# mayataka/idocp

Hardware: AMD Instinct MI355X
Metric: SQP iterations/sec (whole node) (higher is better)
Workload: dtype f64; 1 GPU; ANYmal OCPSolver N=100 T=5.05 FP64, trotting contact sequence (1 lift + 9 impulse events, 120 stages incl. impulse / aux / lift stages, switching constraints; BASELINE.json configs[2]); batch=1024 independent OCP instances per GPU, replicas across GPUs; horizon=100, batch_per_gpu=1024, parallelism=replicas x1

## Files before the change

### idocp_amd/csrc/ocp_capi.hip

```cpp
#include <hip/hip_runtime.h>

#include <cmath>
#include <cstdlib>
#include <cstring>
#include <limits>
#include <string>
#include <vector>

#include "dev_lie.hpp"
#include "host_util.hpp"
#include "idocp_hip.h"
#include "model_shapes.hpp"
#include "ocp_launch.hpp"

using namespace idocp_dev;
using idocp_host::set_last_error;
using idocp_host::isQuadruped;

#define HIP_TRY(expr)                                                                         \
  do {                                                                                        \
    hipError_t e_ = (expr);                                                                   \
    if (e_ != hipSuccess) {                                                                   \
      set_last_error(std::string(#expr) + ": " + hipGetErrorString(e_));                      \
      (void)hipGetLastError();  \
// ... 1532 lines not shown
    }
    const int ck = nd.kind == 1 ? P.impulse_cone_kind : P.cone_kind;
    for (int c = 0; c < DQ::NC; ++c) {
      if (!nd.active[c]) continue;
      double J[3];
      for (int r = 0; r < coneRows(ck); ++r) if (coneRow(ck, P.mu, r, s + LQ::S_F + 3 * c, J) > 0) return false;
    }
    return true;
  };
  for (int b = 0; b < h->batch; ++b) {
    int bad = -1;
    for (int kind = 0; kind < 4 && bad < 0; ++kind)
      for (int p = 0; p < M && bad < 0; ++p) {
        const OcpNode& nd = h->chain[p];
        if (nd.kind != kind) continue;
        if (!stageOk(nd, &sol[((size_t)b * h->NS + nd.slot) * LQ::SOL])) bad = p;
      }
    feasible[b] = bad < 0 ? 1 : 0;
    if (where) where[b] = bad;
  }
  return IDOCP_OK;
}

int idocp_ocp_dimc(const idocp_ocp_t* h) {
  if (!h) return 0;
  const idocp_constraints_t& c = h->cons;
  return 2 * DQ::NU * ((c.joint_position_limits ? 1 : 0) + (c.joint_velocity_limits ? 1 : 0) + (c.joint_torque_limits ? 1 : 0)) +
         (c.linearized_friction_cone ? 5 * DQ::NC : 0) + (c.friction_cone ? 2 * DQ::NC : 0) +
         DQ::NU * ((c.joint_acceleration_lower_limit ? 1 : 0) + (c.joint_acceleration_upper_limit ? 1 : 0)) + (c.contact_distance ? DQ::NC : 0);
}

int idocp_ocp_get_constraint_data(idocp_ocp_t* h, int instance, double* slack, double* dual) {
  if (!h || instance < 0 || instance >= h->batch) return IDOCP_E_ARG;
  int rc = setDev(h); if (rc) return rc;
  const int N = h->Ngrid, dimc = idocp_ocp_dimc(h);
  std::vector<double> sl((size_t)N * LQ::CON), du((size_t)N * LQ::CON);
  HIP_TRY(hipMemcpyAsync(sl.data(), h->B.slack + (size_t)instance * h->NS * LQ::CON, sl.size() * sizeof(double), hipMemcpyDeviceToHost, h->stream));
  HIP_TRY(hipMemcpyAsync(du.data(), h->B.dual + (size_t)instance * h->NS * LQ::CON, du.size() * sizeof(double), hipMemcpyDeviceToHost, h->stream));
  HIP_TRY(hipStreamSynchronize(h->stream));
  const idocp_constraints_t& c = h->cons;
  const int use[11] = {c.joint_position_limits, c.joint_position_limits, c.joint_velocity_limits, c.joint_velocity_limits, c.joint_torque_limits,
                       c.joint_torque_limits, c.linearized_friction_cone || c.friction_cone, 0, c.joint_acceleration_lower_limit, c.joint_acceleration_upper_limit,
                       c.contact_distance};
  const int cr = coneRows(h->prob.cone_kind);
  for (int i = 0; i < N; ++i) {
    int off = 0;
    for (int comp = 0; comp < 11; ++comp) {
      if (!use[comp]) continue;
      const int n = comp == 10 ? DQ::NC : (comp != 6 ? DQ::NU : cr * DQ::NC);
      const bool valid = (comp < 2 || comp == 10) ? i >= 2 : (comp < 4 ? i >= 1 : true);
      for (int r = 0; r < n; ++r) {
        const int src = comp == 10 ? LQ::C_CD + r : (comp != 6 ? ipmCompRow<LQ>(comp) + r : LQ::C_FRIC + 5 * (r / cr) + r % cr);
        if (slack) slack[(size_t)i * dimc + off + r] = valid ? sl[(size_t)i * LQ::CON + src] : 0.0;
        if (dual) dual[(size_t)i * dimc + off + r] = valid ? du[(size_t)i * LQ::CON + src] : 0.0;
      }
      off += n;
    }
  }
  return IDOCP_OK;
}

int idocp_ocp_get_profile(idocp_ocp_t* h, long long* out, int n) {
  if (!h || !out || n <= 0 || n > 64) return IDOCP_E_ARG;
  int rc = setDev(h); if (rc) return rc;
  HIP_TRY(hipMemcpy(out, h->B.prof, sizeof(long long) * n, hipMemcpyDeviceToHost));
  return IDOCP_OK;
}

int idocp_ocp_set_lqr_stage(idocp_ocp_t* h, int stage, int terminal, const double* Qxx, const double* Qxu, const double* Quu, const double* Fqq6,
                            const double* Fqv6, const double* Fvq, const double* Fvv, const double* Fvu, const double* lx, const double* lu,
                            const double* Fx) {
  if (!h || !Qxx || !lx || stage < 0 || stage > h->Ngrid) return IDOCP_E_ARG;
  if (!terminal && (!Qxu || !Quu || !Fqq6 || !Fqv6 || !Fvq || !Fvv || !Fvu || !lu || !Fx)) return IDOCP_E_ARG;
  int rc = setDev(h); if (rc) return rc;
  const int nv = DQ::NV, nx = DQ::NX, nu = DQ::NU;
  std::vector<double> k(LQ::KKT, 0.0);
  for (int c = 0; c < nx; ++c) for (int r = 0; r <= c; ++r) k[LQ::K_QXX + LQ::xsym(r, c)] = Qxx[c * nx + r];
  std::memcpy(&k[LQ::K_LX], lx, sizeof(double) * nx);
  if (!terminal) {
    std::memcpy(&k[LQ::K_QXU], Qxu, sizeof(double) * nx * nu);
    std::memcpy(&k[LQ::K_QUU], Quu, sizeof(double) * nu * nu);
    std::memcpy(&k[LQ::K_FQQ], Fqq6, sizeof(double) * 36);
    std::memcpy(&k[LQ::K_FQV], Fqv6, sizeof(double) * 36);
    std::memcpy(&k[LQ::K_FVQ], Fvq, sizeof(double) * nv * nv);
    std::memcpy(&k[LQ::K_FVV], Fvv, sizeof(double) * nv * nv);
    std::memcpy(&k[LQ::K_FVU], Fvu, sizeof(double) * nv * nu);
    std::memcpy(&k[LQ::K_LU], lu, sizeof(double) * nu);
    std::memcpy(&k[LQ::K_FX], Fx, sizeof(double) * nx);
  }
  HIP_TRY(hipStreamSynchronize(h->stream));
  for (long b = 0; b < h->batch; ++b)
    HIP_TRY(hipMemcpy(h->B.kkt + ((size_t)b * h->NS + stage) * LQ::KKT, k.data(), k.size() * sizeof(double), hipMemcpyHostToDevice));
  return IDOCP_OK;
}

static int getContactDynamics(idocp_ocp_t* h, int instance, int stage, int dimf, double* MJtJinv, double* MJtJinv_dIDCdqv, double* MJtJinv_IDC);
int idocp_ocp_get_contact_dynamics(idocp_ocp_t* h, int instance, int stage, double* MJtJinv, double* MJtJinv_dIDCdqv, double* MJtJinv_IDC) {
  if (!h || !MJtJinv || !MJtJinv_dIDCdqv || !MJtJinv_IDC || instance < 0 || instance >= h->batch) return IDOCP_E_ARG;
  int dimf = -1;
  for (const OcpNode& nd : h->chain) if (nd.kind == 0 && nd.slot == stage) dimf = nd.dimf;
  if (dimf < 0) { set_last_error("idocp_ocp_get_contact_dynamics: stage " + std::to_string(stage) + " is not a grid stage of the current discretisation"); return IDOCP_E_ARG; }
  return getContactDynamics(h, instance, stage, dimf, MJtJinv, MJtJinv_dIDCdqv, MJtJinv_IDC);
}
int idocp_ocp_get_contact_dynamics_chain(idocp_ocp_t* h, int instance, int position, double* MJtJinv, double* MJtJinv_dIDCdqv, double* MJtJinv_IDC) {
  if (!h || !MJtJinv || !MJtJinv_dIDCdqv || !MJtJinv_IDC || instance < 0 || instance >= h->batch || position < 0 || position >= h->M()) return IDOCP_E_ARG;
  const OcpNode& nd = h->chain[position];
  if (nd.kind == 4) { set_last_error("idocp_ocp_get_contact_dynamics_chain: the terminal stage has no dynamics"); return IDOCP_E_ARG; }
  return getContactDynamics(h, instance, nd.slot, nd.dimf, MJtJinv, MJtJinv_dIDCdqv, MJtJinv_IDC);
}
static int getContactDynamics(idocp_ocp_t* h, int instance, int stage, int dimf, double* MJtJinv, double* MJtJinv_dIDCdqv, double* MJtJinv_IDC) {
  int rc = setDev(h); if (rc) return rc;
  std::vector<double> e(LQ::EXP);
  HIP_TRY(hipMemcpyAsync(e.data(), h->B.exp + ((size_t)instance * h->NS + stage) * LQ::EXP, e.size() * sizeof(double), hipMemcpyDeviceToHost, h->stream));
  HIP_TRY(hipStreamSynchronize(h->stream));
  const int n = DQ::NV + dimf;
  for (int c = 0; c < n; ++c) for (int r = 0; r < n; ++r) MJtJinv[r + n * c] = r >= c ? e[LQ::E_MJ + r * (r + 1) / 2 + c] : e[LQ::E_MJ + c * (c + 1) / 2 + r];
  for (int c = 0; c < DQ::NX; ++c) for (int r = 0; r < n; ++r) MJtJinv_dIDCdqv[r + n * c] = e[LQ::E_MJD + r + DQ::NVF * c];
  for (int r = 0; r < n; ++r) MJtJinv_IDC[r] = e[LQ::E_MJIDC + r];
  return dimf;
}

int idocp_ocp_get_lqr_stage(idocp_ocp_t* h, int instance, int stage, double* Qxx, double* Qxu, double* Quu, double* A, double* Bm,
                            double* lx, double* lu, double* Fx) {
  if (!h || instance < 0 || instance >= h->batch || stage < 0 || stage >= h->Ngrid) return IDOCP_E_ARG;
  int rc = setDev(h); if (rc) return rc;
  const int nv = DQ::NV, nx = DQ::NX, nu = DQ::NU;
  std::vector<double> k(LQ::KKT);
  HIP_TRY(hipMemcpyAsync(k.data(), h->B.kkt + ((size_t)instance * h->NS + stage) * LQ::KKT, k.size() * sizeof(double), hipMemcpyDeviceToHost, h->stream));
  HIP_TRY(hipStreamSynchronize(h->stream));
  for (int c = 0; c < nx; ++c) for (int r = 0; r < nx; ++r) Qxx[c * nx + r] = k[LQ::K_QXX + LQ::xsym(r, c)];
  std::memcpy(Qxu, &k[LQ::K_QXU], sizeof(double) * nx * nu);
  std::memcpy(Quu, &k[LQ::K_QUU], sizeof(double) * nu * nu);
  std::memset(A, 0, sizeof(double) * nx * nx);
  std::memset(Bm, 0, sizeof(double) * nx * nu);
  double dt = h->T / h->N;
  for (const OcpNode& nd : h->chain) if (nd.slot == stage) dt = nd.dtq;
  for (int c = 0; c < nv; ++c) for (int r = 0; r < nv; ++r) {
    double fqq = (r == c) ? 1.0 : 0.0, fqv = (r == c) ? dt : 0.0;
    if (r < 6 && c < 6) { fqq = k[LQ::K_FQQ + r + 6 * c]; fqv = k[LQ::K_FQV + r + 6 * c]; }
    else if (r < 6 || c < 6) { fqq = 0.0; fqv = 0.0; }
    A[r + nx * c] = fqq; A[r + nx * (nv + c)] = fqv;
    A[(nv + r) + nx * c] = k[LQ::K_FVQ + r + nv * c]; A[(nv + r) + nx * (nv + c)] = k[LQ::K_FVV + r + nv * c];
  }
  for (int j = 0; j < nu; ++j) for (int r = 0; r < nv; ++r) Bm[(nv + r) + nx * j] = k[LQ::K_FVU + r + nv * j];
  std::memcpy(lx, &k[LQ::K_LX], sizeof(double) * nx);
  std::memcpy(lu, &k[LQ::K_LU], sizeof(double) * nu);
  std::memcpy(Fx, &k[LQ::K_FX], sizeof(double) * nx);
  return IDOCP_OK;
}

int idocp_parnmpc_create(const idocp_model_t* model, const idocp_cost_t* cost, const idocp_constraints_t* constraints, double T,
                         int N, int batch, int device, idocp_ocp_t** out) {
  return createOcpImpl(model, cost, constraints, T, N, 0, batch, device, true, out);
}

int idocp_parnmpc_create_hybrid(const idocp_model_t* model, const idocp_cost_t* cost, const idocp_constraints_t* constraints, double T,
                                int N, int max_num_impulse, int batch, int device, idocp_ocp_t** out) {
  return createOcpImpl(model, cost, constraints, T, N, max_num_impulse, batch, device, true, out);
}

int idocp_parnmpc_init_backward_correction(idocp_ocp_t* h, double t) {
  if (!h || !h->parnmpc) return IDOCP_E_ARG;
  int rc = setDev(h); if (rc) return rc;
  if ((rc = discretize(h, t))) return rc;
  OcpLaunch<DQ>::parnmpcPhase(4, h->B, h->batch, h->M(), h->has_terminal, h->d_q0, h->d_v0, h->stream);
  HIP_TRY(hipGetLastError());
  HIP_TRY(hipStreamSynchronize(h->stream));
  return IDOCP_OK;
}

int idocp_parnmpc_launch_phase(idocp_ocp_t* h, int phase, const double* d_q, const double* d_v) {
  if (!h || !h->parnmpc || phase < 0 || phase > 9 || !d_q || !d_v) return IDOCP_E_ARG;
  int rc = setDev(h); if (rc) return rc;
  if (h->seq_dirty || h->disc_time != h->disc_time) { if ((rc = discretize(h, h->disc_time == h->disc_time ? h->disc_time : 0.0))) return rc; }
  const int M = h->M();
  switch (phase) {
    case 0: OcpLaunch<DQ>::rnea(h->B, h->batch, M, h->n_impulse, h->stream); break;
    case 1:
      if (h->has_switch) OcpLaunch<DQ>::switching(h->B, h->batch, M, h->stream);
      OcpLaunch<DQ>::condenseBackwardEuler(h->B, h->batch, M, d_q, d_v, false, h->stream);
      OcpLaunch<DQ>::parnmpcImpulseCondense(h->B, h->batch, h->n_impulse, false, d_q, d_v, h->stream);
      break;
    case 2:
      OcpLaunch<DQ>::parnmpcInverse(h->B, h->batch, M, h->stream);
      OcpLaunch<DQ>::parnmpcEventInverse(h->B, h->batch, h->n_general, h->stream);
      break;
    case 3: case 4: case 5: case 6: OcpLaunch<DQ>::parnmpcPhase(phase - 3, h->B, h->batch, M, h->has_terminal, d_q, d_v, h->stream); break;
    case 7: OcpLaunch<DQ>::single(4, h->B, h->batch, M, h->stream); break;
    case 8: OcpLaunch<DQ>::single(5, h->B, h->batch, M, h->stream); break;
    default: OcpLaunch<DQ>::single(6, h->B, h->batch, M, h->stream); break;
  }
  HIP_TRY(hipGetLastError());
  return IDOCP_OK;
}

int idocp_parnmpc_update_solution_device(idocp_ocp_t* h, double t, const double* d_q, const double* d_v) {
  if (!h || !h->parnmpc || !d_q || !d_v) return IDOCP_E_ARG;
  if (!h->contact_status_set) { set_last_error("idocp_parnmpc_update_solution: call setContactStatusUniformly first"); return IDOCP_E_ARG; }
  int rc = setDev(h); if (rc) return rc;
  if ((rc = discretize(h, t))) return rc;
  HIP_TRY(hipMemsetAsync(h->B.status, 0, sizeof(int) * h->batch, h->stream));
  for (int phase = 0; phase <= 9; ++phase) if ((rc = idocp_parnmpc_launch_phase(h, phase, d_q, d_v))) return rc;
  return IDOCP_OK;
}

int idocp_parnmpc_compute_direction(idocp_ocp_t* h, double t, const double* q, const double* v) {
  if (!h || !h->parnmpc || !q || !v) return IDOCP_E_ARG;
  if (!h->contact_status_set) { set_last_error("idocp_parnmpc_update_solution: call setContactStatusUniformly first"); return IDOCP_E_ARG; }
  int rc = setDev(h); if (rc) return rc;
  HIP_TRY(hipMemcpyAsync(h->d_q0, q, sizeof(double) * h->batch * DQ::NQ, hipMemcpyHostToDevice, h->stream));
  HIP_TRY(hipMemcpyAsync(h->d_v0, v, sizeof(double) * h->batch * DQ::NV, hipMemcpyHostToDevice, h->stream));
  if ((rc = discretize(h, t))) return rc;
  HIP_TRY(hipMemsetAsync(h->B.status, 0, sizeof(int) * h->batch, h->stream));
  for (int phase = 0; phase <= 8; ++phase) if ((rc = idocp_parnmpc_launch_phase(h, phase, h->d_q0, h->d_v0))) return rc;
  HIP_TRY(hipStreamSynchronize(h->stream));
  return IDOCP_OK;
}

int idocp_parnmpc_update_solution(idocp_ocp_t* h, double t, const double* q, const double* v, int line_search) {
  if (!h || !h->parnmpc || !q || !v) return IDOCP_E_ARG;
  int rc = setDev(h); if (rc) return rc;
  if (line_search) {
    if (!h->contact_status_set) { set_last_error("idocp_parnmpc_update_solution: call setContactStatusUniformly first"); return IDOCP_E_ARG; }
    if ((rc = discretize(h, t))) return rc;
    if ((rc = parnmpcLineSearchSupported(h))) return rc;
// ... 233 lines not shown
```

### idocp_amd/csrc/ocp_condense_kernel.hip

```cpp
#include <hip/hip_runtime.h>

#include <cstdlib>

#include "dev_dense.hpp"
#include "dev_lie.hpp"
#include "dev_rnea_tangent.hpp"
#include "ocp_device.hpp"
#include "ocp_launch.hpp"

namespace idocp_dev {

#ifdef IDOCP_K5_TILES16
#define K5_TILE_PAIR mfmaTilePairTN
#else
#define K5_TILE_PAIR mfmaTilePairTN4
#endif

__device__ __forceinline__ double ocpLimit(const OcpProblem* __restrict__ P, int comp, int r) {
  switch (comp) {
    case 0: return P->q_min[r];
    case 1: return P->q_max[r];
    case 2: return -P->v_max[r];
    case 3: return P->v_max[r];
    case 4: return -P->u_max[r];
// ... 673 lines not shown
        X = &sm[S::MJD + SVF * 16 * ib]; xr = NX - 16 * ib; Y = &sm[S::QAFU + SVF * 16 * jb]; yc = NV - 16 * jb; r0 = 16 * ib; c0 = 16 * jb;
      } else {
        const int ib = j - 12;
        X = &sm[S::MJ + SVF * 16 * ib]; xr = NV - 16 * ib; Y = &sm[S::QAFU + SVF * 6]; yc = NU; r0 = 16 * ib; c0 = 0;
      }
    };
    auto finish = [&](int j, const mfma_d4& acc, int r0, int c0) {
      const int r = r0 + (lane & 15), g4 = lane >> 4;
      if (j < 6) {
        double b6[4];
        const double dg = sm[S::HQD + (r < NX ? r : NX - 1)];
        static_assert(S::HVD == S::HQD + NV, "one diagonal vector");
#pragma unroll
        for (int q = 0; q < 4; ++q) { const int c = c0 + g4 + 4 * q; b6[q] = sm[S::QB6 + (r < 6 ? r : 5) + 6 * (c < 6 ? c : 5)]; }
#pragma unroll
        for (int q = 0; q < 4; ++q) {
          const int c = c0 + g4 + 4 * q;
          const double base = (r < 6 && c < 6) ? b6[q] : (r == c ? dg : 0.0);
          if (r <= c && c < NX) kk[L::K_QXX + L::xsym(r, c)] = base - acc[q];
        }
      } else if (j < 12) {
#pragma unroll
        for (int q = 0; q < 4; ++q) {
          const int c = c0 + g4 + 4 * q;
          double* dst = c < 6 ? ee + (L::E_QXUP + r + NX * c) : kk + (L::K_QXU + r + NX * (c - 6));
          if (r < NX && c < NV) *dst = -acc[q];
        }
      } else {
        double hd[4];
#pragma unroll
        for (int q = 0; q < 4; ++q) { const int c = c0 + g4 + 4 * q; hd[q] = sm[S::HUD + (c < NU ? c : NU - 1)]; }
#pragma unroll
        for (int q = 0; q < 4; ++q) {
          const int c = c0 + g4 + 4 * q;
          double* dst = r < 6 ? ee + (L::E_QUUP + r + 6 * c) : kk + (L::K_QUU + (r - 6) + NU * c);
          const double v = acc[q] + ((r >= 6 && r - 6 == c) ? hd[q] : 0.0);
          if (r < NV && c < NU) *dst = v;
        }
      }
    };
    auto pair = [&](auto jc) {
      constexpr int j = decltype(jc)::value;
      const double *X0, *Y0, *X1, *Y1;
      int xr0, yc0, r00, c00, xr1, yc1, r01, c01;
      operands(j, X0, xr0, Y0, yc0, r00, c00);
      operands(j + 1, X1, xr1, Y1, yc1, r01, c01);
      mfma_d4 a0, a1;
      K5_TILE_PAIR<RVF>(X0, xr0, Y0, yc0, X1, xr1, Y1, yc1, SVF, SVF, dimvf, lane, a0, a1);
      finish(j, a0, r00, c00);
      finish(j + 1, a1, r01, c01);
    };
    static_assert(nt == 256 && NJOB == 14, "four wavefronts: jobs 2 w, 2 w + 1 and 2 w + 8, 2 w + 9");
    switch (__builtin_amdgcn_readfirstlane(wave)) {
      case 0: pair(std::integral_constant<int, 0>{}); pair(std::integral_constant<int, 8>{}); break;
      case 1: pair(std::integral_constant<int, 2>{}); pair(std::integral_constant<int, 10>{}); break;
      case 2: pair(std::integral_constant<int, 4>{}); pair(std::integral_constant<int, 12>{}); break;
      default: pair(std::integral_constant<int, 6>{}); break;
    }
  }
  STAMP(14);
  {
    const int part = tid & 3, g = tid >> 2;
    const int q4 = (dimvf + 3) >> 2, k0 = part * q4, k1 = (k0 + q4 < dimvf) ? k0 + q4 : dimvf;
    double acc = 0.0;
    if (g < NX) { const double* col = &sm[S::MJD + SVF * g]; for (int k = k0; k < k1; ++k) acc += col[k] * sm[S::LAF + k]; }
    else if (g < NX + NV) { const double* row = &sm[S::MJ + (g - NX)]; for (int k = k0; k < k1; ++k) acc += row[SVF * k] * sm[S::LAF + k]; }
    acc += __shfl_xor(acc, 1);
    acc += __shfl_xor(acc, 2);
    if (part == 0) {
      if (g < NV) sm[S::LQ + g] -= acc;
      else if (g < NX) sm[S::LV + g - NV] -= acc;
      else if (g < NX + NV) {
        const int r = g - NX;
        if (r < 6) sm[S::LUP + r] += hu * acc; else sm[S::LU + r - 6] += hu * acc;
        sm[S::FV + r] -= dt * mjidc[r];
      }
    }
  }
  static_assert(4 * (NX + NV) <= nt, "a quad per row of the vector updates");
  blockLdsBarrier();

  STAMP(9);
  typedef double wd2 __attribute__((ext_vector_type(2)));
  static_assert(NV % 2 == 0 && SVF % 2 == 0 && S::MJD % 2 == 0 && L::K_FVQ % 2 == 0 && L::K_FVV % 2 == 0 && L::KKT % 2 == 0, "16-byte stores of Fvq / Fvv");
  for (int e = tid; e < NV * NV / 2; e += nt) {
    const int c = e / (NV / 2), r = 2 * (e - c * (NV / 2));
    const wd2 mq = *reinterpret_cast<const wd2*>(&sm[S::MJD + r + SVF * c]), mvv = *reinterpret_cast<const wd2*>(&sm[S::MJD + r + SVF * (NV + c)]);
    const double one = BWD ? -1.0 : 1.0;
    wd2 fq, fv;
    fq.x = -dt * mq.x; fq.y = -dt * mq.y;
    fv.x = -dt * mvv.x + (r == c ? one : 0.0); fv.y = -dt * mvv.y + (r + 1 == c ? one : 0.0);
    *reinterpret_cast<wd2*>(&kk[L::K_FVQ + r + NV * c]) = fq;
    *reinterpret_cast<wd2*>(&kk[L::K_FVV + r + NV * c]) = fv;
  }
  for (int e = tid; e < NV * NU; e += nt) { const int c = e / NV, r = e - c * NV; kk[L::K_FVU + e] = hu * dt * sm[S::MJ + r + SVF * (6 + c)]; }
  if (tid < NV) {
    kk[L::K_LX + tid] = sm[S::LQ + tid]; kk[L::K_LX + NV + tid] = sm[S::LV + tid];
    kk[L::K_FX + tid] = sm[S::FQ + tid]; kk[L::K_FX + NV + tid] = sm[S::FV + tid];
  }
  if (tid < NU) kk[L::K_LU + tid] = sm[S::LU + tid];
  for (int t = tid; t < RVF * (RVF + 1) / 2; t += nt) {
    const int pr = t / (RVF + 1), idx = t - pr * (RVF + 1);
    const bool lo = idx <= pr;
    const int r = lo ? pr : RVF - 1 - pr, c = lo ? idx : idx - pr - 1;
    ee[L::E_MJ + r * (r + 1) / 2 + c] = sm[S::MJ + r + SVF * c];
  }
  static_assert(RVF % 2 == 0 && NVF % 2 == 0 && L::E_MJD % 2 == 0 && L::EXP % 2 == 0, "16-byte stores of MJtJinv_dIDCdqv");
  for (int e = tid; e < (RVF / 2) * NX; e += nt) {
    const int c = e / (RVF / 2), r = 2 * (e - c * (RVF / 2));
    *reinterpret_cast<wd2*>(&ee[L::E_MJD + r + NVF * c]) = *reinterpret_cast<const wd2*>(&sm[S::MJD + r + SVF * c]);
  }
  if (tid < NV) ee[L::E_QAA + tid] = sm[S::QAA + tid];
  for (int e = tid; e < SF * SF; e += nt) { const int c = e / SF, r = e - c * SF; ee[L::E_QFF + r + NF * c] = sm[S::QFF + e]; }
  if (tid < RVF) { ee[L::E_MJIDC + tid] = mjidc[tid]; ee[L::E_LAF + tid] = sm[S::LAF + tid]; }
  if (tid < 6) ee[L::E_LUP + tid] = sm[S::LUP + tid];
  if (sw_dimi > 0) {
    const int dimi = sw_dimi;
    double* __restrict__ W = B.swc + rec * L::SWC;
    for (int e = tid; e < dimi * NX; e += nt) {
      const int c = e / dimi, j = e - c * dimi;
      double acc = 0.0;
      for (int m2 = 0; m2 < NV; ++m2) acc += W[L::W_PHIA + j + NF * m2] * sm[S::MJD + m2 + SVF * c];
      W[L::W_PHIX + j + NF * c] -= acc;
    }
    for (int e = tid; e < dimi * NU; e += nt) {
      const int c = e / dimi, j = e - c * dimi;
      double acc = 0.0;
      for (int m2 = 0; m2 < NV; ++m2) acc += W[L::W_PHIA + j + NF * m2] * sm[S::MJ + m2 + SVF * (6 + c)];
      W[L::W_PHIU + j + NF * c] = acc;
    }
    if (tid < dimi) {
      double acc = 0.0;
      for (int m2 = 0; m2 < NV; ++m2) acc += W[L::W_PHIA + tid + NF * m2] * mjidc[m2];
      W[L::W_P + tid] -= acc;
    }
  }
  STAMP(10);
  if (tid == 0 && !s_ok && B.status[b] == 0) B.status[b] = 1 + pos;
  };
  stage((long)blockIdx.x);
#undef STAMP
#undef STAMPW
}


template <typename D>
__global__ __launch_bounds__(64) void parnmpc_lie_kernel(OcpBuffers B, const double* __restrict__ q0) {
  using L = OcpLayout<D>;
  constexpr int NQ = D::NQ;
  const OcpProblem* __restrict__ P = B.prob;
  const int M = B.M;
  const long unit = (long)blockIdx.x * 64 + threadIdx.x;
  if (unit >= (long)P->batch * (M - 1)) return;
  const long b = unit / (M - 1);
  const int pos = (int)(unit - b * (M - 1));
  const OcpNode* __restrict__ nd = B.nodes + pos;
  const int task = blockIdx.y;
  const long rec = b * B.NS + nd->slot;
  const double* __restrict__ s = B.sol + rec * L::SOL;
  const double* __restrict__ q = s + L::S_Q;
  double* __restrict__ zz = B.lie + rec * L::LIE;
  double R[9], p[3], Ja[36], Jb[36], d6[6];
  if (task == 0) {
    lieRelative(B.q_ref + (long)pos * NQ, q, R, p);
    lieLog6(R, p, d6);
    lieJlog6(R, p, Ja);
    for (int k = 0; k < 36; ++k) zz[L::Z_JQ + k] = Ja[k];
    for (int k = 0; k < 6; ++k) zz[L::Z_QDIFF + k] = d6[k];
  } else if (task == 1) {
    lieRelative(B.sol + (b * B.NS + nd->next) * L::SOL + L::S_Q, q, R, p);
    lieJlog6(R, p, Ja);
    for (int k = 0; k < 36; ++k) zz[L::Z_FQQ + k] = Ja[k];
  } else {
    const double* __restrict__ q_prev = (nd->prev < 0) ? (q0 + b * NQ) : (B.sol + (b * B.NS + nd->prev) * L::SOL + L::S_Q);
    lieRelative(q, q_prev, R, p);
    lieLog6(R, p, d6);
    for (int k = 0; k < 6; ++k) zz[L::Z_FQ6 + k] = d6[k];
    lieJlog6(R, p, Ja);
    lieDDiffArg0(R, p, Ja, Jb);
    for (int k = 0; k < 36; ++k) zz[L::Z_FQQP + k] = Jb[k];
    lieBlockInverse(Ja, Jb);
    for (int k = 0; k < 36; ++k) zz[L::Z_FQQI + k] = Jb[k];
  }
}

template <typename D>
static void launchCondense(const OcpBuffers& B, long batch, int M, int dimf, const double* q0, hipStream_t st, bool residual, int part = 0) {
  const size_t smem = CondenseSmem<D>::TOTAL * sizeof(double);
  static bool configured = false;
  if (!configured) {
    (void)hipFuncSetAttribute((const void*)ocp_condense_kernel<D, false, -1>, hipFuncAttributeMaxDynamicSharedMemorySize, (int)smem);
    (void)hipFuncSetAttribute((const void*)ocp_condense_kernel<D, false, -1, false, false, true>, hipFuncAttributeMaxDynamicSharedMemorySize, (int)smem);
    (void)hipFuncSetAttribute((const void*)ocp_condense_kernel<D, false, D::NF>, hipFuncAttributeMaxDynamicSharedMemorySize, (int)smem);
// ... 113 lines not shown
```

### idocp_amd/csrc/ocp_device.hpp

```cpp
#ifndef IDOCP_OCP_DEVICE_HPP_
#define IDOCP_OCP_DEVICE_HPP_

#include "unocp_device.hpp"

namespace idocp_dev {

template <int NL_, int LJ_>
struct LeggedDims {
  static constexpr int NL = NL_, LJ = LJ_;
  static constexpr int NJ = 1 + NL * LJ, NV = 6 + NL * LJ, NQ = NV + 1, NU = NL * LJ, NC = NL, NF = 3 * NC;
  static constexpr int NX = 2 * NV, NVF = NV + NF;
};

template <typename D>
struct OcpLayout {
  static constexpr int NV = D::NV, NQ = D::NQ, NU = D::NU, NF = D::NF, NX = D::NX, NVF = D::NVF, NC = D::NC;
  static constexpr int S_LMD = 0, S_GMM = NV, S_Q = 2 * NV, S_V = S_Q + NQ, S_A = S_V + NV, S_U = S_A + NV, S_BETA = S_U + NU,
                       S_F = S_BETA + NV, S_MU = S_F + NF, S_NUP = S_MU + NF, S_XI = S_NUP + 6;
  static constexpr int SOL = roundUp16(S_XI + NF);
  static constexpr int D_LMD = 0, D_GMM = NV, D_Q = 2 * NV, D_V = 3 * NV, D_A = 4 * NV, D_U = 5 * NV, D_BETA = D_U + NU,
                       D_F = D_BETA + NV, D_MU = D_F + NF, D_NUP = D_MU + NF, D_XI = D_NUP + 6,
                       D_T = D_XI + NF, D_W = D_T + NVF;
  static constexpr int DIR = roundUp16(D_W + NVF);
  static constexpr int C_FRIC = 6 * NU, C_ACC = C_FRIC + 5 * NC, C_CD = C_ACC + 2 * NU, NCON = C_CD + NC;
  static constexpr int CON = roundUp16(NCON);
  static constexpr int L_DIDC = 0, L_M = NVF * NX, L_J = L_M + NV * NV, L_IDC = L_J + NF * NV;
  static constexpr int LIN = roundUp16(L_IDC + NVF);
  static constexpr int X_TRI = (NX * (NX + 1) / 2 + 1) / 2 * 2;
  __host__ __device__ static constexpr int xsym(int r, int c) { return r <= c ? c * (c + 1) / 2 + r : r * (r + 1) / 2 + c; }
  static constexpr int K_QXX = 0, K_QXU = X_TRI, K_QUU = K_QXU + NX * NU, K_FQQ = K_QUU + NU * NU, K_FQV = K_FQQ + 36,
                       K_FVQ = K_FQV + 36, K_FVV = K_FVQ + NV * NV, K_FVU = K_FVV + NV * NV, K_LX = K_FVU + NV * NU,
                       K_LU = K_LX + NX, K_FX = K_LU + NU;
  static constexpr int KKT = roundUp16(K_FX + NX);
  static constexpr int MJ_TRI = (NVF * (NVF + 1) / 2 + 1) / 2 * 2;
  static constexpr int E_MJ = 0, E_MJD = MJ_TRI, E_QAA = E_MJD + NVF * NX, E_QFF = E_QAA + NV,
                       E_MJIDC = E_QFF + NF * NF, E_LAF = E_MJIDC + NVF, E_LUP = E_LAF + NVF, E_QUUP = E_LUP + 6,
                       E_QXUP = E_QUUP + 6 * NU, E_FQQPI = E_QXUP + NX * 6;
  static constexpr int EXP = roundUp16(E_FQQPI + 36);
  static constexpr int P_TRI = (NV * (NV + 1) / 2 + 1) / 2 * 2;
  __host__ __device__ static constexpr int psym(int r, int c) { return r <= c ? c * (c + 1) / 2 + r : r * (r + 1) / 2 + c; }
  static constexpr int R_PQQ = 0, R_PQV = P_TRI, R_PVV = R_PQV + NV * NV, R_SQ = R_PVV + P_TRI, R_SV = R_SQ + NV;
  static constexpr int RIC = roundUp16(R_SV + NV);
  static constexpr int Z_JQ = 0, Z_QDIFF = 36, Z_FQQ = 44, Z_FQ6 = 80, Z_FQQI = 88, Z_FQQP = 124, Z_FQQPI = 160;
  static constexpr int LIE = roundUp16(196);
  static constexpr int NJL = NV - 6, NJ_DYN = 42, NF_DYN = 18, NB_DYN = 16;
  static constexpr int O_JOINT = 0, O_FEET = NJL * NJ_DYN, O_BASE = O_FEET + NC * NF_DYN, O_BN = O_BASE + NB_DYN,
                       O_IDC = O_BN + (NC + 1) * 6;
  static constexpr int NOM = roundUp16(O_IDC + NVF);
  static_assert(NVF % 2 == 0, "the nominal record is copied in 16-byte pieces");
  static constexpr int X_CDJ = 0, X_Z = NC * NV, X_LQ = X_Z + NC, X_W = X_LQ + NV, X_ERR = X_W + NC, X_VIOL = X_ERR + 1;
  static constexpr int NT = 1 + IDOCP_MAX_EXTRA_TASKS;
  static constexpr int X_TJ = X_VIOL + 1, X_TW = X_TJ + NT * 6 * NV, X_COST = X_TW + NT * 6;
  static constexpr int EXT = roundUp16(X_COST + 1);
  static constexpr int G_K = 0, G_k = NU * NX;
  static constexpr int GAIN = roundUp16(G_k + NU);
  static constexpr int W_P = 0, W_PHIX = NF, W_PHIA = W_PHIX + NF * NX, W_PHIU = W_PHIA + NF * NV, W_M = W_PHIU + NF * NU,
                       W_m = W_M + NF * NX;
  static constexpr int SWC = roundUp16(W_m + NF);
  static constexpr int N_LMD = 0, N_GMM = NV, N_U = 2 * NV, N_Q = N_U + NU, N_V = N_Q + NQ, N_XI = N_V + NV;
  static constexpr int SNEW = roundUp16(N_XI + NF);
  static constexpr int NK = 2 * NX + NU, I_C0 = 0, I_C1 = NK * NX;
  static constexpr int NKG = 2 * NX + NU + NF, I_C1G = NKG * NX;
  static constexpr int KINV = roundUp16(2 * NKG * NX);
  static constexpr int AUX = roundUp16(NX * NX);
  static constexpr int XRES = roundUp16(NX);
};

struct OcpNode {
  int slot, next, prev;
  int kind;
  int level;
  int has_u;
  int dimf, active[IDOCP_MAX_CONTACTS], row_of[IDOCP_MAX_CONTACTS];
  double dt;
  double dtq;
  double vref_on;
  double contact_point[IDOCP_MAX_CONTACTS][3];
  int sw_dimi, sw_active[IDOCP_MAX_CONTACTS], sw_row[IDOCP_MAX_CONTACTS];
  double sw_dt1, sw_dt2, sw_point[IDOCP_MAX_CONTACTS][3];
};

struct ParnmpcShape {
  bool general, impulse;
  int ni, nw, nk, ld, c1;
};
template <typename L>
__host__ __device__ inline ParnmpcShape parnmpcShape(const OcpNode& nd) {
  ParnmpcShape s;
  s.impulse = nd.kind == 1;
  const bool aux = nd.kind == 2 && nd.sw_dimi > 0;
  s.general = s.impulse || aux;
  s.ni = s.impulse ? nd.dimf : (aux ? nd.sw_dimi : 0);
  s.nw = s.impulse ? nd.dimf : L::NU;
  s.nk = 2 * L::NX + s.ni + s.nw;
  s.ld = s.general ? L::NKG : L::NK;
  s.c1 = s.general ? L::I_C1G : L::I_C1;
  return s;
}

__host__ __device__ inline int coneRows(int kind) { return kind == 1 ? 2 : 5; }
__host__ __device__ inline double coneRow(int kind, double mu, int r, const double* f, double* J) {
  if (kind == 1) {
    if (r == 0) { J[0] = 0.0; J[1] = 0.0; J[2] = -1.0; return -f[2]; }
    J[0] = 2.0 * f[0]; J[1] = 2.0 * f[1]; J[2] = -2.0 * mu * mu * f[2];
    return f[0] * f[0] + f[1] * f[1] - mu * mu * f[2] * f[2];
  }
  const double m2 = mu * 0.70710678118654752440;
  J[0] = (r == 1) ? 1.0 : (r == 2 ? -1.0 : 0.0);
  J[1] = (r == 3) ? 1.0 : (r == 4 ? -1.0 : 0.0);
  J[2] = (r == 0) ? -1.0 : -m2;
  return J[0] * f[0] + J[1] * f[1] + J[2] * f[2];
}

struct OcpProblem;
template <typename L>
__host__ __device__ inline int ipmCompRow(int comp) { return comp < 6 ? comp * L::NU : L::C_ACC + (comp - 8) * L::NU; }

struct OcpProblem {
  int N, batch;
  int M, NS, E;
  int stage_offset;
// ... 74 lines not shown
```

### idocp_amd/csrc/ocp_expand_kernel.hip

```cpp
#include <hip/hip_runtime.h>

#include <cstdlib>

#include "dev_lie.hpp"
#include "dev_dense.hpp"
#include "ocp_device.hpp"
#include "ocp_launch.hpp"

namespace idocp_dev {

__device__ __forceinline__ double ocpLimit2(const OcpProblem* __restrict__ P, int comp, int r) {
  switch (comp) {
    case 0: return P->q_min[r];
    case 1: return P->q_max[r];
    case 2: return -P->v_max[r];
    case 3: return P->v_max[r];
    case 4: return -P->u_max[r];
    case 8: return P->a_min[r];
    case 9: return P->a_max[r];
    default: return P->u_max[r];
  }
}
__device__ __forceinline__ bool ocpRowValid2(const OcpProblem* __restrict__ P, int comp, int level, bool impulse) {
  if (impulse) return comp == 6 && P->use_impulse_friction_cone != 0;
// ... 13 lines not shown
__device__ __forceinline__ bool ipmRow(const OcpProblem* __restrict__ P, const OcpNode* __restrict__ nd, int row, const double* __restrict__ s,
                                       const double* dq, const double* dv, const double* du, const double* df_slot, const double* da,
                                       const double* __restrict__ xx, double* g, double* dg) {
  using L = OcpLayout<D>;
  constexpr int NU = D::NU;
  if (row >= L::C_CD) {
    const int c = row - L::C_CD;
    if (!xx || !P->use_contact_distance || nd->kind == 1 || nd->level < 2 || nd->active[c]) return false;
    *g = -xx[L::X_Z + c];
    double acc = 0.0;
    for (int t = 0; t < D::NV; ++t) acc += xx[L::X_CDJ + c * D::NV + t] * dq[t];
    *dg = -acc;
    return true;
  }
  if (row >= L::C_ACC) {
    const int c = 8 + (row - L::C_ACC) / NU, j = (row - L::C_ACC) % NU;
    if (!ocpRowValid2(P, c, nd->level, nd->kind == 1)) return false;
    const double sgn = (c & 1) ? 1.0 : -1.0;
    *g = sgn * (s[L::S_A + 6 + j] - ocpLimit2(P, c, j));
    *dg = sgn * da[6 + j];
    return true;
  }
  if (row < L::C_FRIC) {
    const int c = row / NU, j = row - c * NU;
    if (!ocpRowValid2(P, c, nd->level, nd->kind == 1)) return false;
    const double sgn = (c & 1) ? 1.0 : -1.0;
    const double x = (c < 2) ? s[L::S_Q + 7 + j] : ((c < 4) ? s[L::S_V + 6 + j] : s[L::S_U + j]);
    const double dx = (c < 2) ? dq[6 + j] : ((c < 4) ? dv[6 + j] : du[j]);
    *g = sgn * (x - ocpLimit2(P, c, j));
    *dg = sgn * dx;
    return true;
  }
  const int fr = row - L::C_FRIC, c = fr / 5, r = fr - 5 * c;
  const int ck = nd->kind == 1 ? P->impulse_cone_kind : P->cone_kind;
  if (r >= coneRows(ck) || !ocpRowValid2(P, 6, nd->level, nd->kind == 1) || !nd->active[c]) return false;
  double J[3];
  const double f[3] = {s[L::S_F + 3 * c], s[L::S_F + 3 * c + 1], s[L::S_F + 3 * c + 2]};
  *g = coneRow(ck, P->mu, r, f, J);
  *dg = J[0] * df_slot[3 * c] + J[1] * df_slot[3 * c + 1] + J[2] * df_slot[3 * c + 2];
  return true;
}
template <typename D>
__device__ __forceinline__ bool ipmIdleConeRow(const OcpProblem* __restrict__ P, const OcpNode* __restrict__ nd, int row) {
  using L = OcpLayout<D>;
  if (row >= L::C_CD) return P->use_contact_distance && nd->kind != 1 && nd->level >= 2 && nd->active[row - L::C_CD];
  if (row < L::C_FRIC || row >= L::C_ACC || !ocpRowValid2(P, 6, nd->level, nd->kind == 1)) return false;
  const int r = (row - L::C_FRIC) % 5;
  return r < coneRows(nd->kind == 1 ? P->impulse_cone_kind : P->cone_kind);
}

typedef double ex_d2 __attribute__((ext_vector_type(2)));
template <int N2>
__device__ __forceinline__ void wideLoad(ex_d2 (&r)[(N2 + 63) / 64], const double* __restrict__ src, int lane) {
  const ex_d2* __restrict__ p = reinterpret_cast<const ex_d2*>(src);
#pragma unroll
  for (int t = 0; t < (N2 + 63) / 64; ++t) { const int e = lane + 64 * t; r[t] = p[e < N2 ? e : N2 - 1]; }
}
template <int N2>
__device__ __forceinline__ void wideLoadN(ex_d2 (&r)[(N2 + 63) / 64], const double* __restrict__ src, int lane, int n2) {
  const ex_d2* __restrict__ p = reinterpret_cast<const ex_d2*>(src);
#pragma unroll
  for (int t = 0; t < (N2 + 63) / 64; ++t) { const int e = lane + 64 * t; r[t] = p[e < n2 ? e : n2 - 1]; }
}
template <int N2, int LD2>
__device__ __forceinline__ void wideLoadRows(ex_d2 (&r)[(N2 + 63) / 64], const double* __restrict__ src, int lane, int h, int inv, int n2) {
  const ex_d2* __restrict__ p = reinterpret_cast<const ex_d2*>(src);
#pragma unroll
  for (int t = 0; t < (N2 + 63) / 64; ++t) {
    int e = lane + 64 * t;
    e = e < n2 ? e : n2 - 1;
    const int c = (e * inv) >> 16;
    r[t] = p[c * LD2 + (e - c * h)];
  }
}
template <int N2, int LD2>
__device__ __forceinline__ void wideStoreLdsRows(double* dst, const ex_d2 (&r)[(N2 + 63) / 64], int lane, int h, int inv, int n2) {
#pragma unroll
  for (int t = 0; t < (N2 + 63) / 64; ++t) {
    const int e = lane + 64 * t;
    const int c = (e * inv) >> 16;
    if (e < n2) reinterpret_cast<ex_d2*>(dst)[c * LD2 + (e - c * h)] = r[t];
  }
}
template <int N2>
__device__ __forceinline__ void wideStoreLds(double* dst, const ex_d2 (&r)[(N2 + 63) / 64], int lane) {
#pragma unroll
  for (int t = 0; t < (N2 + 63) / 64; ++t) { const int e = lane + 64 * t; if (e < N2) reinterpret_cast<ex_d2*>(dst)[e] = r[t]; }
}

template <typename D>
__global__ __launch_bounds__(64) void ocp_expand_primal_kernel(OcpBuffers B) {
  using L = OcpLayout<D>;
  constexpr int NV = D::NV, NX = D::NX, NU = D::NU, NF = D::NF, NVF = D::NVF, NC = D::NC;
  constexpr int RL = L::R_SV + NV, MJDL = NVF * NX, MJUL = L::MJ_TRI;
  static_assert(RL % 2 == 0 && MJDL % 2 == 0 && MJUL % 2 == 0 && L::E_MJD % 2 == 0 && L::EXP % 2 == 0 && L::RIC % 2 == 0, "16-byte loads");
  constexpr int PML = RL > MJDL ? RL : MJDL;
  __shared__ __attribute__((aligned(16))) double pm[PML], mju[MJUL], sr[L::SOL];
  double* pb = pm;
  double* mjd = pm;
  __shared__ double dx[NX], du[NU], dfs[NF], das[NV];
  const OcpProblem* __restrict__ P = B.prob;
  const int M = B.M;
  const int lane = threadIdx.x;
  const long unit = blockIdx.x;
  const long b = unit / M;
  const int pos = (int)(unit - b * M);
  const OcpNode* __restrict__ nd = B.nodes + pos;
  const bool terminal = (pos == M - 1);
  const long rec = b * B.NS + nd->slot;
  double* __restrict__ dd = B.dir + rec * L::DIR;
  if (P->backward_euler && terminal) return;
  const bool costate = !P->backward_euler;
  const bool bimp = P->backward_euler && nd->kind == 1;
  const bool expand = !terminal && !bimp;
  ex_d2 pw[(RL / 2 + 63) / 64], mw[(MJDL / 2 + 63) / 64], uw[(MJUL / 2 + 63) / 64];
  if (costate) wideLoad<RL / 2>(pw, B.ric + rec * L::RIC, lane);
  const int rows_ld = NV + nd->dimf, h_ld = (rows_ld + 1) >> 1, inv_ld = 65535 / h_ld + 1, nmjd2 = h_ld * NX, ntri2 = (rows_ld * (rows_ld + 1) / 2 + 1) >> 1;
  static_assert(NVF % 2 == 0 && (NVF / 2) * NX == MJDL / 2, "pieces per column of MJtJinv_dIDCdqv");
  if (expand) {
    wideLoadRows<MJDL / 2, NVF / 2>(mw, B.exp + rec * L::EXP + L::E_MJD, lane, h_ld, inv_ld, nmjd2);
    wideLoadN<MJUL / 2>(uw, B.exp + rec * L::EXP + L::E_MJ, lane, ntri2);
  }
  static_assert(L::SOL % 2 == 0 && L::NCON <= 128, "two IPM rows per lane");
  ex_d2 sw[(L::SOL / 2 + 63) / 64];
  double sl_r[2] = {1.0, 1.0}, dl_r[2] = {1.0, 1.0}, mjidc_r = 0.0;
  if (!terminal) {
    wideLoad<L::SOL / 2>(sw, B.sol + rec * L::SOL, lane);
#pragma unroll
    for (int t = 0; t < 2; ++t) {
      const int row = lane + 64 * t;
      if (row < L::NCON) { sl_r[t] = B.slack[rec * L::CON + row]; dl_r[t] = B.dual[rec * L::CON + row]; }
    }
    if (lane < NVF) mjidc_r = B.exp[rec * L::EXP + L::E_MJIDC + lane];
  }
  if (lane < NV) { dx[lane] = dd[L::D_Q + lane]; dx[NV + lane] = dd[L::D_V + lane]; }
  if (lane < NU && !terminal) du[lane] = dd[L::D_U + lane];
  if (lane < NF) dfs[lane] = 0.0;
  if (costate) wideStoreLds<RL / 2>(pb, pw, lane);
  if (expand) wideStoreLds<MJUL / 2>(mju, uw, lane);
  if (!terminal) wideStoreLds<L::SOL / 2>(sr, sw, lane);
  waveLdsSync();
  if (lane < NX && costate) {
    const bool isv = lane >= NV;
    const int r = isv ? lane - NV : lane;
    double acc = -pb[(isv ? L::R_SV : L::R_SQ) + r];
    if (!isv) {
#pragma unroll
      for (int c = 0; c < NV; ++c) acc += pb[L::R_PQQ + L::psym(r, c)] * dx[c] + pb[L::R_PQV + r + NV * c] * dx[NV + c];
    } else {
#pragma unroll
      for (int c = 0; c < NV; ++c) acc += pb[L::R_PQV + c + NV * r] * dx[c] + pb[L::R_PVV + L::psym(r, c)] * dx[NV + c];
    }
    dd[(isv ? L::D_GMM : L::D_LMD) + r] = acc;
  }
  if (terminal) return;
  waveLdsSync();
  if (expand) wideStoreLdsRows<MJDL / 2, NVF / 2>(mjd, mw, lane, h_ld, inv_ld, nmjd2);
  waveLdsSync();
  const long su = rec;
  const double* s = sr;
  const int dimf = nd->dimf, dimvf = NV + dimf;
  if (bimp) {
    const double* __restrict__ kk = B.kkt + rec * L::KKT;
    if (lane < NF) dfs[lane] = dd[L::D_F + lane];
    if (lane < NV) {
      double acc = -mjidc_r;
      double t1 = 0.0;
      for (int c = 0; c < NV; ++c) t1 += kk[L::K_FVQ + lane + NV * c] * dx[c];
      acc += t1;
      double t2 = 0.0;
      for (int j = 0; j < dimf; ++j) t2 += kk[L::K_FVU + lane + NV * j] * du[j];
      acc += t2;
      dd[L::D_A + lane] = acc; das[lane] = acc;
    }
  }
  if (!P->backward_euler && nd->sw_dimi > 0 && lane >= 32 && lane < 32 + nd->sw_dimi) {
    const int l = lane - 32;
    const double* __restrict__ W = B.swc + rec * L::SWC;
    double acc = W[L::W_m + l];
    for (int c = 0; c < NX; ++c) acc += W[L::W_M + l + NF * c] * dx[c];
    dd[L::D_XI + l] = acc;
  }
  if (!bimp && lane < dimvf) {
    const int r = lane;
    double acc = -mjidc_r, tt = 0.0, ww = 0.0;
#pragma unroll
    for (int c = 0; c < NX; ++c) tt += mjd[r + NVF * c] * dx[c];
#pragma unroll
    for (int j = 0; j < NU; ++j) { const int c = 6 + j; ww += (r >= c ? mju[r * (r + 1) / 2 + c] : mju[c * (c + 1) / 2 + r]) * du[j]; }
    acc += ww - tt;
    dd[L::D_T + r] = tt; dd[L::D_W + r] = ww;
    if (r < NV) { dd[L::D_A + r] = acc; das[r] = acc; }
    else {
      const int pr = r - NV;
      for (int c = 0; c < NC; ++c) if (nd->active[c] && pr >= nd->row_of[c] && pr < nd->row_of[c] + 3) {
        const int slot = 3 * c + (pr - nd->row_of[c]);
        dfs[slot] = -acc; dd[L::D_F + slot] = -acc;
      }
    }
  }
  waveLdsSync();
  double ps = 1.0, ds = 1.0;
#pragma unroll
  for (int t = 0; t < 2; ++t) {
    const int row = lane + 64 * t;
    double g, dg;
    if (row >= L::NCON || !ipmRow<D>(P, nd, row, s, dx, dx + NV, du, dfs, das, B.ext ? B.ext + rec * L::EXT : nullptr, &g, &dg)) continue;
    const double sl = sl_r[t], dl = dl_r[t];
    const double res = g + sl, duality = sl * dl - P->barrier;
    const double dslack = -dg - res;
    const double ddual = -(dl * dslack + duality) / sl;
    ps = f2b(P->fraction_rate, sl, dslack, ps);
    ds = f2b(P->fraction_rate, dl, ddual, ds);
  }
#pragma unroll
  for (int off = 32; off >= 1; off >>= 1) { ps = fmin(ps, __shfl_xor(ps, off)); ds = fmin(ds, __shfl_xor(ds, off)); }
  if (lane == 0) { B.step_stage[su * 2] = ps; B.step_stage[su * 2 + 1] = ds; }
}

template <typename D>
__global__ __launch_bounds__(128, 1) void ocp_forward_expand_kernel(OcpBuffers B, const double* __restrict__ q0, const double* __restrict__ v0) {
  using L = OcpLayout<D>;
  constexpr int NV = D::NV, NQ = D::NQ, NX = D::NX, NU = D::NU, NF = D::NF, NVF = D::NVF, NC = D::NC;
  constexpr int GL = L::GAIN, RL = L::R_SV + NV, MJDL = NVF * NX, MJUL = L::MJ_TRI;
  static_assert(GL % 2 == 0 && RL % 2 == 0 && MJDL % 2 == 0 && MJUL % 2 == 0 && L::SOL % 2 == 0 && L::GAIN % 2 == 0 && L::RIC % 2 == 0 && L::EXP % 2 == 0 &&
                L::E_MJD % 2 == 0 && L::KKT % 2 == 0 && L::K_FQQ % 2 == 0 && L::K_FX % 2 == 0 && NVF % 2 == 0, "16-byte loads");
  static_assert(L::K_FQV == L::K_FQQ + 36 && L::NCON <= 128 && NX <= 36 && 36 + NX / 2 <= 64, "Fqq6 | Fqv6 and Fx on one load; two IPM rows per lane");
  static_assert(NC <= 4 && NF <= 15 && NVF + NV <= 64 && L::R_PQQ == 0 && L::R_SV == L::R_SQ + NV, "node word: four contacts; lane maps");
  static_assert(L::C_FRIC >= 64 && L::C_CD >= 64 && L::NCON <= 128, "cone / contact-distance rows are mapped to lane + 64 only");
  constexpr int NG2 = (GL / 2 + 63) / 64, NP2 = (RL / 2 + 63) / 64, NM2 = (MJDL / 2 + 63) / 64, NT2 = (MJUL / 2 + 63) / 64, NS2 = (L::SOL / 2 + 63) / 64;
  constexpr int MAXM = OcpForwardExpandMaxChain;
  constexpr int PF = NX * NX, PSV = PF, PPAD = PF + NX;
  constexpr int DV = NX + NU + NV + NF + 2;
  __shared__ __attribute__((aligned(16))) double gb[GL], pfull[PF + NX + 2], mjd[MJDL], mju[MJUL], sr[L::SOL], fb[72 + NX];
  __shared__ double ring[3][DV];
  __shared__ int n_slot[MAXM], n_word[MAXM];
  __shared__ double n_dt[MAXM], n_dtq[MAXM];
  const int M = B.M;
  const int tid = threadIdx.x, lane = tid & 63;
  const int wave = __builtin_amdgcn_readfirstlane(tid >> 6);
  const long b = blockIdx.x;
  const long base = b * B.NS;
  int use_cone, use_icone, use_cd, ck_stage, ck_imp;
  double cmu, barrier, frate;
  int r_xoff[2], r_doff[2], r_thr[2];
  double r_sgn[2], r_bound[2];
  {
    const OcpProblem* __restrict__ P = B.prob;
    use_cone = P->use_friction_cone; use_icone = P->use_impulse_friction_cone;
    use_cd = P->use_contact_distance; ck_stage = P->cone_kind; ck_imp = P->impulse_cone_kind;
    cmu = P->mu; barrier = P->barrier; frate = P->fraction_rate;
#pragma unroll
    for (int t = 0; t < 2; ++t) {
      const int row = lane + 64 * t;
      r_xoff[t] = 0; r_doff[t] = 0; r_thr[t] = 4; r_sgn[t] = 1.0; r_bound[t] = 0.0;
      if (row < L::C_FRIC) {
        const int c = row / NU, j = row - c * NU;
        r_sgn[t] = (c & 1) ? 1.0 : -1.0;
        r_xoff[t] = (c < 2) ? L::S_Q + 7 + j : ((c < 4) ? L::S_V + 6 + j : L::S_U + j);
        r_doff[t] = (c < 2) ? 6 + j : ((c < 4) ? NV + 6 + j : NX + j);
        r_bound[t] = ocpLimit2(P, c, j);
        r_thr[t] = (c < 2) ? (P->use_q_limits ? 2 : 4) : ((c < 4) ? (P->use_v_limits ? 1 : 4) : (P->use_u_limits ? 0 : 4));
      } else if (row >= L::C_ACC && row < L::C_CD) {
        const int c = 8 + (row - L::C_ACC) / NU, j = (row - L::C_ACC) % NU;
        r_sgn[t] = (c & 1) ? 1.0 : -1.0;
        r_xoff[t] = L::S_A + 6 + j; r_doff[t] = NX + NU + 6 + j;
        r_bound[t] = ocpLimit2(P, c, j);
        r_thr[t] = (c == 8 ? P->use_a_lower : P->use_a_upper) ? 0 : 4;
      }
    }
    const OcpNode* __restrict__ nodes = B.nodes;
    for (int i = tid; i < M; i += 128) {
      const OcpNode* __restrict__ nd = nodes + i;
      int w = (nd->kind & 7) | ((nd->level < 3 ? (nd->level < 0 ? 0 : nd->level) : 3) << 3) | (nd->dimf << 5) | (nd->sw_dimi << 9) | ((nd->has_u ? 1 : 0) << 13);
#pragma unroll
      for (int c = 0; c < NC; ++c) if (nd->active[c]) w |= (1 << (14 + c)) | ((nd->row_of[c] / 3) << (18 + 2 * c));
      n_slot[i] = nd->slot; n_word[i] = w; n_dt[i] = nd->dt; n_dtq[i] = nd->dtq;
    }
  }
  if (wave == 0) {
    double* dx = ring[0];
    const int slot0 = B.nodes[0].slot;
    const double* __restrict__ s0 = B.sol + (base + slot0) * L::SOL;
    if (lane == 0) {
      double R[9], p[3], d6[6];
      lieRelative(s0 + L::S_Q, q0 + b * NQ, R, p);
      lieLog6(R, p, d6);
      const double* __restrict__ Fi = B.exp + (base + slot0) * L::EXP + L::E_FQQPI;
      for (int r = 0; r < 6; ++r) { double acc = 0.0; for (int m = 0; m < 6; ++m) acc += Fi[r + 6 * m] * d6[m]; dx[r] = -acc; }
    }
    if (lane >= 6 && lane < NV) dx[lane] = q0[b * NQ + lane + 1] - s0[L::S_Q + lane + 1];
    if (lane < NV) dx[NV + lane] = v0[b * NV + lane] - s0[L::S_V + lane];
  }
  blockLdsSync();
  if (wave == 0) {
    struct Regs { ex_d2 g[NG2], m[NM2], u[NT2], f; double mjidc; };
    Regs RA, RB;
    const int af_row = lane < NVF ? lane : NVF - 1;
    int tri_off[NU];
#pragma unroll
    for (int j = 0; j < NU; ++j) { const int c = 6 + j; tri_off[j] = af_row >= c ? af_row * (af_row + 1) / 2 + c : c * (c + 1) / 2 + af_row; }
    auto fetch = [&](int i, Regs& R) {
      const long rec = base + n_slot[i];
      wideLoad<GL / 2>(R.g, B.gain + rec * L::GAIN, lane);
      const int rows_ld = NV + ((n_word[i] >> 5) & 15), h_ld = (rows_ld + 1) >> 1, inv_ld = 65535 / h_ld + 1;
      wideLoadRows<MJDL / 2, NVF / 2>(R.m, B.exp + rec * L::EXP + L::E_MJD, lane, h_ld, inv_ld, h_ld * NX);
      wideLoadN<MJUL / 2>(R.u, B.exp + rec * L::EXP + L::E_MJ, lane, (rows_ld * (rows_ld + 1) / 2 + 1) >> 1);
      {
        const ex_d2* __restrict__ kq = reinterpret_cast<const ex_d2*>(B.kkt + rec * L::KKT + L::K_FQQ);
        const ex_d2* __restrict__ kx = reinterpret_cast<const ex_d2*>(B.kkt + rec * L::KKT + L::K_FX);
        R.f = lane < 36 ? kq[lane] : kx[lane - 36 < NX / 2 ? lane - 36 : NX / 2 - 1];
      }
      R.mjidc = B.exp[rec * L::EXP + L::E_MJIDC + af_row];
    };
    if (M > 1) fetch(0, RA);
    if (M > 2) fetch(1, RB);
    auto step = [&](int i, Regs& R) {
      double* const dv = ring[i % 3];
      double* const dx = dv; double* const du = dv + NX; double* const das = dv + NX + NU; double* const dfs = dv + NX + NU + NV;
      double* const dxn = ring[(i + 1) % 3];
      const int word = n_word[i];
      const long rec = base + n_slot[i];
      const int dimf = (word >> 5) & 15, amask = (word >> 14) & 15, rows3 = (word >> 18) & 255;
      const double sdt = n_dt[i], sdtq = n_dtq[i];
      double* __restrict__ dd = B.dir + rec * L::DIR;
      const int dimvf = NV + dimf;
      const int h_ld = (dimvf + 1) >> 1, inv_ld = 65535 / h_ld + 1;
      wideStoreLds<GL / 2>(gb, R.g, lane);
      wideStoreLdsRows<MJDL / 2, NVF / 2>(mjd, R.m, lane, h_ld, inv_ld, h_ld * NX);
      wideStoreLds<MJUL / 2>(mju, R.u, lane);
      if (lane < 36 + NX / 2) reinterpret_cast<ex_d2*>(fb)[lane] = R.f;
      const double mjidc_r = R.mjidc;
      waveLdsSync();
      if (i + 2 < M - 1) fetch(i + 2, R);
      {
        const int j = lane >> 2, part = lane & 3;
        double acc = 0.0;
        if (lane < 4 * NU) {
#pragma unroll
          for (int t = 0; t < NX / 4; ++t) { const int c = (NX / 4) * part + t; acc += gb[L::G_K + j + NU * c] * dx[c]; }
        }
        acc += __shfl_xor(acc, 1);
        acc += __shfl_xor(acc, 2);
        if (lane < 4 * NU && part == 0) { acc += gb[L::G_k + j]; du[j] = acc; dd[L::D_U + j] = acc; }
      }
      double tt = 0.0;
      if (lane < dimvf) {
#pragma unroll
        for (int c = 0; c < NX; ++c) tt += mjd[lane + NVF * c] * dx[c];
      }
      if (lane < NF) dfs[lane] = 0.0;
      if (lane >= 40 && lane < 40 + NV) { const int r = lane - 40; dd[L::D_Q + r] = dx[r]; dd[L::D_V + r] = dx[NV + r]; }
      waveLdsSync();
      if (lane < dimvf) {
        const int r = lane;
        double ww = 0.0;
#pragma unroll
        for (int j = 0; j < NU; ++j) ww += mju[tri_off[j]] * du[j];
        const double acc_af = -mjidc_r + (ww - tt);
        dd[L::D_T + r] = tt; dd[L::D_W + r] = ww;
        if (r < NV) {
          dd[L::D_A + r] = acc_af; das[r] = acc_af;
          dxn[NV + r] = dx[NV + r] + sdt * (ww - tt) + fb[72 + NV + r];
        } else {
          const int pr = r - NV;
#pragma unroll
          for (int c = 0; c < NC; ++c) {
            const int row_of = 3 * ((rows3 >> (2 * c)) & 3);
            if (((amask >> c) & 1) && pr >= row_of && pr < row_of + 3) {
              const int slot = 3 * c + (pr - row_of);
              dfs[slot] = -acc_af; dd[L::D_F + slot] = -acc_af;
            }
          }
        }
      } else if (lane >= 32 && lane < 32 + NV) {
        const int r = lane - 32;
        double dq = fb[72 + r];
        if (r < 6) {
#pragma unroll
          for (int m = 0; m < 6; ++m) dq += fb[r + 6 * m] * dx[m] + fb[36 + r + 6 * m] * dx[NV + m];
        } else {
          dq += dx[r] + sdtq * dx[NV + r];
        }
        dxn[r] = dq;
      }
    };
    static_assert(NVF <= 32, "the dq+ rows sit on the lanes behind the (a, f) rows");
    for (int i = 0; i <= M; i += 2) {
      if (i < M - 1) step(i, RA);
      blockLdsSync();
      if (i + 1 <= M) {
        if (i + 1 < M - 1) step(i + 1, RB);
        blockLdsSync();
      }
    }
    {
      const double* dx = ring[(M - 1) % 3];
      double* __restrict__ dd = B.dir + (base + n_slot[M - 1]) * L::DIR;
      if (lane < NV) { dd[L::D_Q + lane] = dx[lane]; dd[L::D_V + lane] = dx[NV + lane]; }
    }
  } else {
    struct Regs { ex_d2 p[NP2], s[NS2]; double sl[2], dl[2]; };
    Regs RA, RB;
    int p_a[NP2][2], p_b[NP2][2];
#pragma unroll
    for (int t = 0; t < NP2; ++t) {
#pragma unroll
      for (int h = 0; h < 2; ++h) {
        const int k = 2 * (lane + 64 * t) + h;
        int a = PPAD + h, bb = PPAD + h;
        if (k < L::R_PQV || (k >= L::R_PVV && k < L::R_SQ)) {
          const bool vv = k >= L::R_PVV;
// ... 521 lines not shown
```

### idocp_amd/csrc/ocp_riccati_kernel.hip

```cpp
#include <hip/hip_runtime.h>
#include <cstdlib>
#include <type_traits>

#include "dev_dense.hpp"
#include "dev_lie.hpp"
#include "ocp_device.hpp"
#include "ocp_launch.hpp"

namespace idocp_dev {

typedef double rd2 __attribute__((ext_vector_type(2)));

template <typename D>
struct RiccatiSmem {
  static constexpr int NV = D::NV, NX = D::NX, NU = D::NU, NF = D::NF;
  static constexpr int LDW = NX + 2;
  static constexpr int PQQ = 0, PQV = PQQ + NV * NV, PVV = PQV + NV * NV, SQ = PVV + NV * NV, SV = SQ + NV,
                       STAGE = SV + NV + 4,
                       STAGE_LEN = OcpLayout<D>::KKT - OcpLayout<D>::K_QXU,
                       WT = STAGE + STAGE_LEN, GK = WT + LDW * NX,
                       KM = WT + LDW * (NX + NU), KV = KM + NU * NX,
                       GW = KV + 16, SQN = GW + NU * NU, SVN = SQN + NV, INVD = SVN + NV + 4, TOTAL = INVD + NU + 4;
  static_assert(NU * NX <= NU * LDW, "GK aliases B^T P");
  static constexpr int DG = WT, SS = DG + NF * NU, DTM = SS + NF * NF, SDG = DTM + NU * NX, MV = SDG + NF * NU, SCORR = MV + NF,
                       MMX = GK;
  static_assert(SCORR + NX <= GK && NF * NX <= NU * LDW, "hybrid aliases");
  static_assert(TOTAL * 8 + 64 <= 40960, "four instances per CU");
};

__device__ __forceinline__ void upperTile3(int t, int& ib, int& jb) {
  if (t < 3) { ib = 0; jb = t; } else if (t < 5) { ib = 1; jb = t - 2; } else { ib = 2; jb = 2; }
}

constexpr int tileBegin(int ntiles, int w, int nw) { return (ntiles * w + nw - 1) / nw; }
constexpr bool tilesUseMod3(int tb, int te, int v) { for (int t = tb; t < te; ++t) if (t % 3 == v) return true; return false; }
constexpr bool tilesUseDiv3(int tb, int te, int v) { for (int t = tb; t < te; ++t) if (t / 3 == v) return true; return false; }
constexpr int upperIb(int t) { return t < 3 ? 0 : (t < 5 ? 1 : 2); }
constexpr int upperJb(int t) { return t < 3 ? t : (t < 5 ? t - 2 : 2); }
constexpr bool tilesUseUpperIb(int tb, int te, int v) { for (int t = tb; t < te; ++t) if (upperIb(t) == v) return true; return false; }
constexpr bool tilesUseUpperJb(int tb, int te, int v) { for (int t = tb; t < te; ++t) if (upperJb(t) == v) return true; return false; }

template <int K>
__device__ __forceinline__ void mfmaLoadOp(double (&o)[(K + 3) / 4], const double* p, int stride, int lane) {
  const int g = lane >> 4;
#pragma unroll
  for (int s = 0; s < (K + 3) / 4; ++s) {
    const int k = 4 * s + g;
    if (4 * s + 3 < K) o[s] = p[stride * k];
    else { const double v = p[stride * (k < K ? k : K - 1)]; o[s] = k < K ? v : 0.0; }
  }
}

template <typename D, bool WIDE, int TB, int TE, typename Mid>
__device__ __forceinline__ void riccatiPhase1(const double* Pqq, const double* Pqv, const double* Pvv, const double* Fall, const double* Fqq6,
                                              const double* Fqv6, double dt, double* Wt, int lane, Mid mid) {
  constexpr int NV = D::NV, NX = D::NX, KS = (NV + 3) / 4, LDW = RiccatiSmem<D>::LDW, NTL = TE - TB;
  if constexpr (NTL > 0) {
    const int li = lane & 15, g = lane >> 4;
    double xo[3][KS], yo[3][KS];
#pragma unroll
    for (int v = 0; v < 3; ++v) {
      if (tilesUseMod3(TB, TE, v)) {
        const int c = 16 * v + li, cc = c < NX ? c : NX - 1;
        mfmaLoadOp<NV>(xo[v], cc < NV ? Pqv + cc : Pvv + NV * (cc - NV), cc < NV ? NV : 1, lane);
      }
      if (tilesUseDiv3(TB, TE, v)) mfmaLoadOp<NV>(yo[v], Fall + NV * (16 * v + li), 1, lane);
    }
    auto structured = [&](int j, int q) -> double {
      const int cb = (TB + j) % 3, ib = (TB + j) / 3;
      const int c = 16 * cb + li, cc = c < NX ? c : NX - 1;
      const double* pq = cc < NV ? Pqq + NV * cc : Pqv + NV * (cc - NV);
      const int lo = 16 * ib + 4 * q, r = lo + g;
      if (lo >= NX) return 0.0;
      const int lo6 = lo < NV ? lo : lo - NV;
      const bool isv = r >= NV;
      const int rr6 = isv ? r - NV : r;
      const bool any6 = lo6 < 6 || (lo < NV && lo + 3 >= NV), all6 = lo6 + 3 < 6 && !(lo < NV && lo + 3 >= NV);
      double dot6 = 0.0;
      if (any6) {
        const double* F6 = (isv ? Fqv6 : Fqq6) + 6 * (rr6 < 6 ? rr6 : 0);
#pragma unroll
        for (int m = 0; m < 6; ++m) dot6 += F6[m] * pq[m];
      }
      if (all6) return dot6;
      const double direct = (isv ? dt : 1.0) * pq[rr6 < NV ? rr6 : 0];
      return (any6 && rr6 < 6) ? dot6 : direct;
    };
    constexpr bool EARLY = false;
    double extra[EARLY ? NTL : 1][4];
    if constexpr (EARLY) {
#pragma unroll
      for (int j = 0; j < NTL; ++j)
#pragma unroll
        for (int q = 0; q < 4; ++q) extra[j][q] = structured(j, q);
    }
    mfma_d4 acc[NTL];
#pragma unroll
    for (int j = 0; j < NTL; ++j) acc[j] = mfma_d4{0.0, 0.0, 0.0, 0.0};
#pragma unroll
    for (int s = 0; s < KS; ++s)
#pragma unroll
      for (int j = 0; j < NTL; ++j) acc[j] = __builtin_amdgcn_mfma_f64_16x16x4f64(yo[(TB + j) / 3][s], xo[(TB + j) % 3][s], acc[j], 0, 0, 0);
    __builtin_amdgcn_sched_barrier(0);
    mid();
    __builtin_amdgcn_sched_barrier(0);
#pragma unroll
    for (int j = 0; j < NTL; ++j) {
      __builtin_amdgcn_sched_barrier(0);
      const int cb = (TB + j) % 3, ib = (TB + j) / 3;
      const int c = 16 * cb + li;
#pragma unroll
      for (int q = 0; q < 4; ++q) {
        const int r = 16 * ib + 4 * q + g;
        double sx;
        if constexpr (EARLY) sx = extra[j][q]; else sx = structured(j, q);
        if (c < NX) Wt[c + LDW * r] = acc[j][q] + sx;
      }
    }
  } else {
    mid();
  }
}

template <typename D, bool WIDE, int TB, int TE, int T2W>
__device__ __forceinline__ void riccatiPhase2(const double* Wt, const double* Fall, const double* Fqq6, const double* Fqv6, double dt,
                                              const double (&qxx)[T2W][4], double* Pqq, double* Pqv, double* Pvv, double* Qxu, double* Quu,
                                              int lane) {
  constexpr int NV = D::NV, NX = D::NX, NU = D::NU, KS = (NV + 3) / 4, LDW = RiccatiSmem<D>::LDW, NTL = TE - TB;
  static_assert(NTL <= T2W, "Qxx registers");
  if constexpr (NTL > 0) {
    const int li = lane & 15, g = lane >> 4;
    double xo[3][KS], yo[3][KS];
#pragma unroll
// ... 114 lines not shown
          const int rb = r >= NV, cb = c >= NV, rr = r - NV * rb, cc = c - NV * cb;
          double* blk = Pqq + NV * NV * (rb + cb);
          const double val = blk[rr + NV * cc] - sign * acc[j][q];
          blk[rr + NV * cc] = val;
          blk[(rb == cb) ? cc + NV * rr : rr + NV * cc] = val;
        }
      }
    }
  }
}

#define RICCATI_TILES_CASE8(FN, NTILES, W, ...)                                                                                        \
  case W: if constexpr (tileBegin(NTILES, W, 8) < tileBegin(NTILES, W + 1, 8)) FN<D, false, tileBegin(NTILES, W, 8), tileBegin(NTILES, W + 1, 8)>(__VA_ARGS__); break;
#define RICCATI_TILES(FN, NTILES, ...)                                                                                                 \
  do {                                                                                                                                 \
    if constexpr (NW == 1) { FN<D, true, 0, NTILES>(__VA_ARGS__); }                                                                          \
    else if constexpr (NW == 2) {                                                                                                      \
      if (wave == 0) FN<D, false, tileBegin(NTILES, 0, 2), tileBegin(NTILES, 1, 2)>(__VA_ARGS__);                                            \
      else FN<D, false, tileBegin(NTILES, 1, 2), tileBegin(NTILES, 2, 2)>(__VA_ARGS__);                                                      \
    } else if constexpr (NW == 8) {                                                                                                    \
      switch (wave) {                                                                                                                  \
        RICCATI_TILES_CASE8(FN, NTILES, 0, __VA_ARGS__) RICCATI_TILES_CASE8(FN, NTILES, 1, __VA_ARGS__)                                \
        RICCATI_TILES_CASE8(FN, NTILES, 2, __VA_ARGS__) RICCATI_TILES_CASE8(FN, NTILES, 3, __VA_ARGS__)                                \
        RICCATI_TILES_CASE8(FN, NTILES, 4, __VA_ARGS__) RICCATI_TILES_CASE8(FN, NTILES, 5, __VA_ARGS__)                                \
        RICCATI_TILES_CASE8(FN, NTILES, 6, __VA_ARGS__) RICCATI_TILES_CASE8(FN, NTILES, 7, __VA_ARGS__)                                \
        default: break;                                                                                                                \
      }                                                                                                                                \
    } else {                                                                                                                           \
      if (wave == 0) FN<D, false, tileBegin(NTILES, 0, 4), tileBegin(NTILES, 1, 4)>(__VA_ARGS__);                                            \
      else if (wave == 1) FN<D, false, tileBegin(NTILES, 1, 4), tileBegin(NTILES, 2, 4)>(__VA_ARGS__);                                       \
      else if (wave == 2) FN<D, false, tileBegin(NTILES, 2, 4), tileBegin(NTILES, 3, 4)>(__VA_ARGS__);                                       \
      else FN<D, false, tileBegin(NTILES, 3, 4), tileBegin(NTILES, 4, 4)>(__VA_ARGS__);                                                      \
    }                                                                                                                                  \
  } while (0)

template <int NW> __device__ __forceinline__ void blockSync() {
  if constexpr (NW == 1) { __builtin_amdgcn_fence(__ATOMIC_SEQ_CST, "wavefront"); __builtin_amdgcn_wave_barrier(); }
  else blockLdsSync();
}

template <typename D, int NT, bool HYBRID>
__global__ __launch_bounds__(NT, (NT == 64 || NT == 512) ? 1 : 2) void ocp_riccati_backward_kernel(OcpBuffers B) {
  using L = OcpLayout<D>;
  using S = RiccatiSmem<D>;
  constexpr int NV = D::NV, NX = D::NX, NU = D::NU, NN = NV * NV, NF = D::NF, LDW = S::LDW, NW = NT / 64;
  static_assert(NX + NU == 48 && NX <= 48, "3 x 3 tiles of 16");
  extern __shared__ __attribute__((aligned(16))) double sm[];
  __shared__ int s_ok;
  const OcpProblem* __restrict__ P = B.prob;
  const int M = B.M;
  const OcpNode* __restrict__ nodes = B.nodes;
  const int tid = threadIdx.x;
  constexpr int nt = NT;
  const int wave = tid >> 6, lane = tid & 63, li = lane & 15, g = lane >> 4;
  const long b = blockIdx.x;
  const long base = b * B.NS;
  double* Pqq = &sm[S::PQQ];
  double* Pqv = &sm[S::PQV];
  double* Pvv = &sm[S::PVV];
  double* Wt = &sm[S::WT];
  double* st = &sm[S::STAGE];
  constexpr int KO = L::K_QXU, SL = S::STAGE_LEN;
  if (tid == 0) s_ok = 1;
  const bool p32 = P->ric_fp32 != 0;
  auto st32 = [&](double x) { return p32 ? (double)(float)x : x; };
  {
    const double* __restrict__ kk = B.kkt + (base + nodes[M - 1].slot) * L::KKT;
    double* __restrict__ rr = B.ric + (base + nodes[M - 1].slot) * L::RIC;
    for (int e = tid; e < NN; e += nt) {
      const int c = e / NV, r = e - c * NV;
      const double pqq = st32(kk[L::K_QXX + L::xsym(r, c)]), pvv = st32(kk[L::K_QXX + L::xsym(NV + r, NV + c)]);
      Pqq[e] = pqq; Pqv[e] = 0.0; Pvv[e] = pvv;
      rr[L::R_PQV + e] = 0.0;
      if (r <= c) { rr[L::R_PQQ + L::psym(r, c)] = pqq; rr[L::R_PVV + L::psym(r, c)] = pvv; }
    }
    if (tid < NV) {
      const double sq = st32(-kk[L::K_LX + tid]), sv = st32(-kk[L::K_LX + NV + tid]);
      sm[S::SQ + tid] = sq; sm[S::SV + tid] = sv;
      rr[L::R_SQ + tid] = sq; rr[L::R_SV + tid] = sv;
    }
  }
  {
    const double* __restrict__ kk = B.kkt + (base + nodes[M - 2].slot) * L::KKT;
    for (int e = tid; e < SL; e += nt) st[e] = kk[KO + e];
  }
  blockSync<NW>();
  for (int i = M - 2; i >= 0; --i) {
    const OcpNode* __restrict__ nd = nodes + i;
    const double dt = nd->dtq;
    const long rec = base + nd->slot;
    const int dimi = HYBRID ? nd->sw_dimi : 0;
    const bool stamp = tid == 0 && b == (gridDim.x > 7 ? 7 : 0) && i == M / 2 && B.prof != nullptr;
#define RSTAMP(k) do { if (stamp) B.prof[16 + k] = wall_clock64(); } while (0)
    RSTAMP(0);
    constexpr int PF = (SL / 2 + NT - 1) / NT, T1 = 9, T2 = 6, T2W = (T2 + NW - 1) / NW;
    static_assert(SL % 2 == 0 && KO % 2 == 0 && S::STAGE % 2 == 0 && L::KKT % 2 == 0, "16-byte loads of the stage record");
    rd2 pre[PF];
    double qxx[T2W][4];
    auto loadQxx = [&]() {
      const double* __restrict__ kc = B.kkt + rec * L::KKT;
      const int t2b = tileBegin(T2, wave, NW), t2e = tileBegin(T2, wave + 1, NW);
#pragma unroll
      for (int jj = 0; jj < T2W; ++jj) {
        const int t = t2b + jj;
        int ib, jb;
        upperTile3(t < t2e ? t : 0, ib, jb);
        const int r = 16 * ib + li;
#pragma unroll
        for (int q = 0; q < 4; ++q) {
          const int c = 16 * jb + g + 4 * q;
          qxx[jj][q] = (t < t2e && r <= c && c < NX) ? kc[L::K_QXX + L::xsym(r, c)] : 0.0;
        }
      }
    };
    double* Qxu = st + (L::K_QXU - KO);
    double* Quu = st + (L::K_QUU - KO);
    const double* Fqq6 = st + (L::K_FQQ - KO);
    const double* Fqv6 = st + (L::K_FQV - KO);
    const double* Fall = st + (L::K_FVQ - KO);
    static_assert(L::K_FVV == L::K_FVQ + NV * NV && L::K_FVU == L::K_FVV + NV * NV, "[Fvq Fvv Fvu] contiguous");
    const double* Fvq = st + (L::K_FVQ - KO);
    const double* Fvv = st + (L::K_FVV - KO);
    const double* Fvu = st + (L::K_FVU - KO);
    const double* lx = st + (L::K_LX - KO);
    double* lu = st + (L::K_LU - KO);
    const double* Fx = st + (L::K_FX - KO);
    RSTAMP(1);
    RICCATI_TILES(riccatiPhase1, T1, Pqq, Pqv, Pvv, Fall, Fqq6, Fqv6, dt, Wt, lane, loadQxx);
    blockSync<NW>();
    RSTAMP(2);
    RICCATI_TILES(riccatiPhase2, T2, Wt, Fall, Fqq6, Fqv6, dt, qxx, Pqq, Pqv, Pvv, Qxu, Quu, lane);
    RSTAMP(11);
    if (tid >= NT - 64 && lane < 4 * NU) {
      const int j = lane >> 2, part = lane & 3;
      const int c0 = (part >> 1) * (NX / 2) + (part & 1) * 10, nc2 = (part & 1) ? 4 : 5;
      static_assert(NX == 36 && LDW % 2 == 0, "column split of the lu rows");
      const rd2* wj = reinterpret_cast<const rd2*>(Wt + LDW * (NX + j) + c0);
      const rd2* fx = reinterpret_cast<const rd2*>(Fx + c0);
      double acc = 0.0;
#pragma unroll
      for (int c = 0; c < 5; ++c) if (c < nc2) { const rd2 w = wj[c], f = fx[c]; acc += w.x * f.x + w.y * f.y; }
#pragma unroll
      for (int t = 0; t < (NV + 3) / 4; ++t) { const int m = part + 4 * t; if (m < NV) acc -= Fvu[m + NV * j] * sm[S::SV + m]; }
      acc += __shfl_xor(acc, 1);
      acc += __shfl_xor(acc, 2);
      if (part == 0) lu[j] += acc;
    }
    auto sPart1 = [&](int row) {
      const bool isv = row >= NV;
      const int r = isv ? row - NV : row;
      const double* F6 = isv ? Fqv6 : Fqq6;
      const rd2* Fm = reinterpret_cast<const rd2*>((isv ? Fvv : Fvq) + NV * r);
      const rd2* wr = reinterpret_cast<const rd2*>(Wt + LDW * row);
      const rd2* svp = reinterpret_cast<const rd2*>(&sm[S::SV]);
      const rd2* fx = reinterpret_cast<const rd2*>(Fx);
      static_assert(NV % 2 == 0 && S::SV % 2 == 0 && (L::K_FX - KO) % 2 == 0 && (L::K_FVQ - KO) % 2 == 0, "16-byte reads of the vector terms");
      double acc;
      if (r < 6) {
        acc = 0.0;
#pragma unroll
        for (int m = 0; m < 6; ++m) acc += F6[m + 6 * r] * sm[S::SQ + m];
      } else {
        acc = isv ? dt * sm[S::SQ + r] : sm[S::SQ + r];
      }
      double a2 = 0.0, a3 = 0.0;
#pragma unroll
      for (int m = 0; m < NV / 2; ++m) { const rd2 f = Fm[m], sv2 = svp[m]; acc += f.x * sv2.x + f.y * sv2.y; }
#pragma unroll
      for (int c = 0; c < NX / 2; c += 2) {
        const rd2 w0 = wr[c], f0 = fx[c], w1 = wr[c + 1], f1 = fx[c + 1];
        a2 += w0.x * f0.x + w0.y * f0.y;
        a3 += w1.x * f1.x + w1.y * f1.y;
      }
      sm[(isv ? S::SVN : S::SQN) + r] = acc - (a2 + a3) - lx[row];
    };
    if (NW == 1 && tid < NX) sPart1(tid);
    RSTAMP(12);
    blockSync<NW>();
    RSTAMP(3);
    if (i > 0) {
      const rd2* __restrict__ kn = reinterpret_cast<const rd2*>(B.kkt + (base + nodes[i - 1].slot) * L::KKT + KO);
#pragma unroll
      for (int t = 0; t < PF; ++t) { const int e = tid + NT * t; pre[t] = kn[e < SL / 2 ? e : SL / 2 - 1]; }
    }
    RSTAMP(9);
    if (NW > 1 && tid >= 64 && tid < 64 + NX) sPart1(tid - 64);
    const bool constrained = HYBRID && dimi > 0;
    if (tid < 64) {
      double x[NU];
      if (!constrained) {
#pragma unroll
        for (int m = 0; m < NU; ++m) x[m] = (tid < NX) ? Qxu[tid + NX * m] : lu[m];
      } else {
#pragma unroll
        for (int m = 0; m < NU; ++m) x[m] = (m == tid) ? 1.0 : 0.0;
      }
      choleskySolveRows<NU>(Quu, NU, tid, &s_ok, x);
      if (!constrained) {
        if (tid <= NX) {
#pragma unroll
          for (int m = 0; m < NU; ++m) { if (tid < NX) sm[S::KM + m + NU * tid] = -x[m]; else sm[S::KV + m] = -x[m]; }
        }
      } else if (tid < NU) {
#pragma unroll
        for (int m = 0; m < NU; ++m) sm[S::GW + m + NU * tid] = x[m];
      }
    }
    blockSync<NW>();
    RSTAMP(10);
    if (HYBRID && dimi > 0) {
      const double* __restrict__ W = B.swc + rec * L::SWC;
      const double* __restrict__ Phiu = W + L::W_PHIU;
      for (int e = tid; e < dimi * NU; e += nt) {
        const int c = e / dimi, j = e - c * dimi;
        double acc = 0.0;
        for (int m = 0; m < NU; ++m) acc += Phiu[j + NF * m] * sm[S::GW + m + NU * c];
        sm[S::DG + j + NF * c] = acc;
      }
      blockSync<NW>();
      for (int e = tid; e < dimi * dimi; e += nt) {
        const int c = e / dimi, j = e - c * dimi;
        double acc = 0.0;
        for (int m = 0; m < NU; ++m) acc += sm[S::DG + j + NF * m] * Phiu[c + NF * m];
        sm[S::SS + j + NF * c] = acc;
      }
      blockSync<NW>();
      if (tid < 64) {
        static_assert(NU + NX + 1 <= 64, "one lane per right-hand side");
        const double* __restrict__ Wc = B.swc + rec * L::SWC;
        double x[NF];
#pragma unroll
        for (int j = 0; j < NF; ++j) {
          double val = 0.0;
          if (j < dimi) val = tid < NU ? sm[S::DG + j + NF * tid] : (tid < NU + NX ? Wc[L::W_PHIX + j + NF * (tid - NU)] : (tid == NU + NX ? Wc[L::W_P + j] : 0.0));
          x[j] = val;
        }
        choleskySolveRows<NF>(&sm[S::SS], NF, tid, &s_ok, x, dimi);
#pragma unroll
        for (int j = 0; j < NF; ++j) {
          if (j < dimi) {
            if (tid < NU) sm[S::SDG + j + NF * tid] = x[j];
            else if (tid < NU + NX) sm[S::MMX + j + NF * (tid - NU)] = x[j];
            else if (tid == NU + NX) sm[S::MV + j] = x[j];
          }
        }
      }
      blockSync<NW>();
      for (int e = tid; e < NU * NU; e += nt) {
        const int c = e / NU, r = e - c * NU;
        double acc = 0.0;
        for (int l = 0; l < dimi; ++l) acc += sm[S::SDG + l + NF * r] * sm[S::DG + l + NF * c];
        sm[S::GW + e] -= acc;
      }
      blockSync<NW>();
    }
    if (constrained) {
      const double* __restrict__ Phix = B.swc + rec * L::SWC + L::W_PHIX;
      const double* __restrict__ Pv = B.swc + rec * L::SWC + L::W_P;
      for (int e = tid; e < NU * NX; e += nt) {
        const int c = e / NU, j = e - c * NU;
        double acc = 0.0;
#pragma unroll
        for (int m = 0; m < NU; ++m) acc += sm[S::GW + j + NU * m] * Qxu[c + NX * m];
        for (int l = 0; l < dimi; ++l) acc += sm[S::SDG + l + NF * j] * Phix[l + NF * c];
        sm[S::KM + e] = -acc;
      }
// ... 19 lines not shown
        const int l = tid;
        double acc = sm[S::MV + l];
        for (int m = 0; m < NU; ++m) acc -= sm[S::SDG + l + NF * m] * lu[m];
        sm[S::MV + l] = acc;
        W[L::W_m + l] = acc;
      }
    }
    blockSync<NW>();
    if (HYBRID && dimi > 0) {
      const double* __restrict__ W = B.swc + rec * L::SWC;
      for (int e = tid; e < NU * NX; e += nt) {
        const int c = e / NU, m = e - c * NU;
        double acc = 0.0;
        for (int l = 0; l < dimi; ++l) acc += W[L::W_PHIU + l + NF * m] * sm[S::MMX + l + NF * c];
        sm[S::DTM + m + NU * c] = acc;
      }
      if (tid < NX) {
        double acc = 0.0;
        for (int l = 0; l < dimi; ++l) acc += W[L::W_PHIX + l + NF * tid] * sm[S::MV + l];
        sm[S::SCORR + tid] = acc;
      }
      blockSync<NW>();
    }
    RSTAMP(4);
    if (constrained) {
      RICCATI_TILES(riccatiPhase4, 3, Quu, &sm[S::KM], &sm[S::GK], lane);
      blockSync<NW>();
    }
    RSTAMP(5);
    if (tid >= NT - NV) {
      const int r = tid - (NT - NV);
      double sq = sm[S::SQN + r], sv = sm[S::SVN + r];
#pragma unroll
      for (int j = 0; j < NU; ++j) { sq -= Qxu[r + NX * j] * sm[S::KV + j]; sv -= Qxu[(NV + r) + NX * j] * sm[S::KV + j]; }
      sm[S::SQN + r] = sq; sm[S::SVN + r] = sv;
    }
    {
      const double* Y = constrained ? &sm[S::GK] : Qxu;
      const int ycs = constrained ? NU : 1, yks = constrained ? 1 : NX;
      const double sign = constrained ? 1.0 : -1.0;
      RICCATI_TILES(riccatiPhase5, T2, &sm[S::KM], Y, ycs, yks, sign, Pqq, Pqv, Pvv, lane);
    }
    blockSync<NW>();
    RSTAMP(6);
    RSTAMP(7);
    double* __restrict__ rr = B.ric + rec * L::RIC;
    double* __restrict__ gg = B.gain + rec * L::GAIN;
    static_assert(S::PQV % 2 == 0 && L::R_PQV % 2 == 0 && NN % 2 == 0 && L::RIC % 2 == 0, "Pqv is one contiguous copy");
    if (HYBRID && dimi > 0) {
      for (int e = tid; e < NN; e += nt) {
        const int c = e / NV, r = e - c * NV;
        double aqq = 0.0, aqv = 0.0, avv = 0.0;
        for (int j = 0; j < NU; ++j) {
          const double kqr = sm[S::KM + j + NU * r], kqc = sm[S::KM + j + NU * c], kvr = sm[S::KM + j + NU * (NV + r)], kvc = sm[S::KM + j + NU * (NV + c)];
          const double dqr = sm[S::DTM + j + NU * r], dqc = sm[S::DTM + j + NU * c], dvr = sm[S::DTM + j + NU * (NV + r)], dvc = sm[S::DTM + j + NU * (NV + c)];
          aqq += kqr * dqc + kqc * dqr;
          aqv += kqr * dvc + kvc * dqr;
          avv += kvr * dvc + kvc * dvr;
        }
        const double pqq = st32(Pqq[e] - aqq), pqv = st32(Pqv[e] - aqv), pvv = st32(Pvv[e] - avv);
        Pqq[e] = pqq; Pqv[e] = pqv; Pvv[e] = pvv;
        rr[L::R_PQV + e] = pqv;
        if (r <= c) { rr[L::R_PQQ + L::psym(r, c)] = pqq; rr[L::R_PVV + L::psym(r, c)] = pvv; }
      }
    } else {
      if (p32) { for (int e = tid; e < 3 * NN; e += nt) Pqq[e] = (double)(float)Pqq[e]; blockSync<NW>(); }
      for (int e = tid; e < NN / 2; e += nt) reinterpret_cast<rd2*>(rr + L::R_PQV)[e] = reinterpret_cast<const rd2*>(Pqv)[e];
      for (int e = tid; e < NN; e += nt) {
        const int c = e / NV, r = e - c * NV;
        if (r <= c) { rr[L::R_PQQ + L::psym(r, c)] = Pqq[e]; rr[L::R_PVV + L::psym(r, c)] = Pvv[e]; }
      }
    }
    if (tid < NV) {
      double sq = sm[S::SQN + tid], sv = sm[S::SVN + tid];
      if (HYBRID && dimi > 0) { sq -= sm[S::SCORR + tid]; sv -= sm[S::SCORR + NV + tid]; }
      sq = st32(sq); sv = st32(sv);
      sm[S::SQ + tid] = sq; sm[S::SV + tid] = sv;
      rr[L::R_SQ + tid] = sq; rr[L::R_SV + tid] = sv;
    }
    static_assert(S::KM % 2 == 0 && L::G_K == 0 && (NU * NX) % 2 == 0 && L::GAIN % 2 == 0, "K is one contiguous copy");
    for (int e = tid; e < NU * NX / 2; e += nt) reinterpret_cast<rd2*>(gg)[e] = reinterpret_cast<const rd2*>(&sm[S::KM])[e];
    if (tid < NU) gg[L::G_k + tid] = sm[S::KV + tid];
    if (i > 0) {
#pragma unroll
      for (int t = 0; t < PF; ++t) { const int e = tid + NT * t; if (e < SL / 2) reinterpret_cast<rd2*>(st)[e] = pre[t]; }
    }
    blockSync<NW>();
    RSTAMP(8);
#undef RSTAMP
  }
  if (tid == 0 && !s_ok && B.status[b] == 0) B.status[b] = 1;
}

template <typename D>
struct RiccatiSlots {
  static_assert(D::NV == 18 && D::NU == 12, "slot table of a 6 + 12 dof floating base");
  __host__ __device__ static constexpr int nat(int s) {
    return s < 12 ? 6 + s : s < 16 ? s - 12 : s < 28 ? 24 + (s - 16) : s < 32 ? 18 + (s - 28) : s < 34 ? 4 + (s - 32) : s < 36 ? 22 + (s - 34) : s;
  }
  __host__ __device__ static constexpr int slot(int n) {
    return n < 4 ? 12 + n : n < 6 ? 32 + (n - 4) : n < 18 ? n - 6 : n < 22 ? 28 + (n - 18) : n < 24 ? 34 + (n - 22) : n < 36 ? 16 + (n - 24) : n;
  }
};

template <typename D>
struct RiccatiRegSmem {
  static constexpr int NV = D::NV, NX = D::NX, NU = D::NU, NF = D::NF;
  static constexpr int LDH = 48;
  static constexpr int LDP = 49;
  static constexpr int HT = 0,
                       KT = HT + NU * LDH,
                       RED = KT + NU * LDH,
                       VF = RED + 192, VT = VF + 48, LUH = VT + 48, KV = LUH + 16,
                       VS = KV + 16,
                       PM = VS + 48,
                       PLAIN = PM + 48 * LDP;
  static constexpr int QXU = PM, QUU = QXU + NX * NU, LU = QUU + NU * NU, KM = LU + 16, KVN = KM + NU * NX, GW = KVN + 16,
                       DG = GW + NU * NU, SS = DG + NF * NU, DTM = SS + NF * NF, SDG = DTM + NU * NX, MV = SDG + NF * NU,
                       SCORR = MV + 16, MMX = SCORR + 48,
                       GK = MMX,
                       WL = MMX + NF * NX,
                       WL_P = WL, WL_PHIX = WL + NF, WL_PHIU = WL_PHIX + NF * NX, HYB = WL_PHIU + NF * NU;
  static_assert(NF * NX == NU * NX, "GK aliases MMX");
  static constexpr int NTBL = OcpLayout<D>::R_SV + NV;
  static constexpr size_t BYTES = (HYB > PLAIN ? HYB : PLAIN) * sizeof(double);
  static_assert(BYTES + 64 <= 40960, "four instances per CU");
};

template <typename D, bool HYBRID>
__global__ __launch_bounds__(64, 1) void ocp_riccati_backward_reg_kernel(OcpBuffers B) {
  using L = OcpLayout<D>;
  using S = RiccatiRegSmem<D>;
  using SL = RiccatiSlots<D>;
  constexpr int NV = D::NV, NX = D::NX, NU = D::NU, NF = D::NF, LDH = S::LDH, LDP = S::LDP;
  static_assert(NX + NU == 48 && L::R_PQV == L::R_PQQ + L::P_TRI && L::R_PVV == L::R_PQV + NV * NV && L::R_SQ == L::R_PVV + L::P_TRI &&
                L::R_SV == L::R_SQ + NV && L::R_PQQ == 0, "ric record: Pqq | Pqv | Pvv | sq | sv");
  static_assert(L::K_FVV == L::K_FVQ + NV * NV && L::K_FVU == L::K_FVV + NV * NV, "[Fvq Fvv Fvu] contiguous");
  extern __shared__ __attribute__((aligned(16))) double sm[];
  __shared__ int s_ok;
  const OcpProblem* __restrict__ P = B.prob;
  const int M = B.M;
  const OcpNode* __restrict__ nodes = B.nodes;
  const int lane = threadIdx.x, li = lane & 15, g = lane >> 4;
  const long b = blockIdx.x;
  const long base = b * B.NS;
  const bool p32 = __builtin_amdgcn_readfirstlane(P->ric_fp32) != 0;
  auto st32 = [&](double x) { return p32 ? (double)(float)x : x; };
  auto slotOf = [&](int pos) { return (long)__builtin_amdgcn_readfirstlane(nodes[pos].slot); };
  if (lane == 0) s_ok = 1;
  constexpr int DC[6] = {0, 1, 1, 1, 1, 2}, DS[6] = {3, 0, 1, 2, 3, 0};
  constexpr int TA[6] = {2, 2, 2, 0, 0, 1}, TB[6] = {0, 1, 2, 0, 1, 1};
  constexpr int ZERO_AT = L::K_FX + NX;
  static_assert(ZERO_AT < L::KKT, "a pad double behind Fx");
  int cOff[6][3];
#pragma unroll
  for (int d = 0; d < 6; ++d) {
    const int rs = 16 * DC[d] + 4 * DS[d] + g;
    const int rn = SL::nat(rs);
#pragma unroll
    for (int bb = 0; bb < 3; ++bb) {
      const int cn = SL::nat(16 * bb + li);
      int off;
      if (rn < NV) off = cn < 6 ? L::K_FQQ + rn + 6 * cn : ((cn >= NV && cn < NV + 6) ? L::K_FQV + rn + 6 * (cn - NV) : ZERO_AT);
      else off = L::K_FVQ + (rn - NV) + NV * cn;
      cOff[d][bb] = off;
    }
  }
  int qOff[6][4];
#pragma unroll
  for (int t = 0; t < 6; ++t)
#pragma unroll
    for (int q = 0; q < 4; ++q) {
      const int ni = SL::nat(16 * TA[t] + 4 * q + g), nj = SL::nat(16 * TB[t] + li);
      qOff[t][q] = (ni < NX && nj < NX) ? L::K_QXX + L::xsym(ni, nj)
                 : (ni < NX ? L::K_QXU + ni + NX * (nj - NX) : (nj < NX ? L::K_QXU + nj + NX * (ni - NX) : L::K_QUU + (ni - NX) + NU * (nj - NX)));
    }
  unsigned cqPk[21];
  {
    static_assert(8 * (L::KKT) < 65536 && 8 * (S::PM + 48 * LDP) < 65536, "16-bit byte offsets");
#pragma unroll
    for (int e = 0; e < 21; ++e) {
      const int e0 = 2 * e, e1 = 2 * e + 1;
      const int o0 = e0 < 18 ? cOff[e0 / 3][e0 % 3] : qOff[(e0 - 18) / 4][(e0 - 18) % 4];
      const int o1 = e1 < 18 ? cOff[e1 / 3][e1 % 3] : qOff[(e1 - 18) / 4][(e1 - 18) % 4];
      cqPk[e] = (unsigned)(8 * o0) | ((unsigned)(8 * o1) << 16);
    }
  }
  const int myNat = SL::nat(lane < 48 ? lane : 47);
  const int lzOff = myNat < NX ? L::K_LX + myNat : L::K_LU + (myNat - NX);
  constexpr int N2 = S::NTBL / 2, NP = (N2 + 63) / 64;
  static_assert(S::NTBL % 2 == 0 && L::R_SQ % 2 == 0, "pairs");
  int pmOff[NP][2];
#pragma unroll
  for (int t = 0; t < NP; ++t)
#pragma unroll
    for (int hh = 0; hh < 2; ++hh) {
      const int e2 = lane + 64 * t < N2 ? lane + 64 * t : N2 - 1;
      const int e = 2 * e2 + hh;
      int off;
      if (e >= L::R_SQ) {
        off = S::VS + SL::slot(e - L::R_SQ);
      } else {
        int r = 0, c = 0;
        if (e < L::R_PQV) { int cc = 0; while ((cc + 1) * (cc + 2) / 2 <= e && cc < NV - 1) ++cc; c = cc; r = e - cc * (cc + 1) / 2; if (r > c) r = c; }
        else if (e < L::R_PVV) { const int k = e - L::R_PQV; c = k / NV; r = k - c * NV; c += NV; }
        else { const int k = e - L::R_PVV; int cc = 0; while ((cc + 1) * (cc + 2) / 2 <= k && cc < NV - 1) ++cc; c = cc; r = k - cc * (cc + 1) / 2; if (r > c) r = c; r += NV; c += NV; }
        int i = SL::slot(r), j = SL::slot(c);
        const int bi = i >> 4, bj = j >> 4;
        const bool keep = bi == bj ? i <= j : ((bi == 0 && bj == 1) || bi == 2);
        if (!keep) { const int tt = i; i = j; j = tt; }
        off = S::PM + LDP * i + j;
      }
      pmOff[t][hh] = off;
    }
  unsigned pmPk[NP];
#pragma unroll
  for (int t = 0; t < NP; ++t) pmPk[t] = (unsigned)(8 * pmOff[t][0]) | ((unsigned)(8 * pmOff[t][1]) << 16);
  constexpr int G2 = (NU * NX + NU) / 2, NG = (G2 + 63) / 64;
  static_assert(L::G_K == 0 && L::G_k == NU * NX && NU % 2 == 0 && 2 * G2 <= L::GAIN, "gain record: K | k");
  unsigned gnPk[NG];
#pragma unroll
  for (int t = 0; t < NG; ++t) {
    const int e2 = lane + 64 * t < G2 ? lane + 64 * t : G2 - 1, e = 2 * e2;
    const int o0 = e < NU * NX ? S::KT + LDH * (e % NU) + SL::slot(e / NU) : S::KV + (e - NU * NX);
    const int o1 = e < NU * NX ? o0 + LDH : o0 + 1;
    gnPk[t] = (unsigned)(8 * o0) | ((unsigned)(8 * o1) << 16);
  }
  auto ldsAt = [&](const double* b0, unsigned byteoff) { return *reinterpret_cast<const double*>(reinterpret_cast<const char*>(b0) + byteoff); };
  typedef mfma_d4 tile_t;
  tile_t Pt[3][3];
  double s_reg = 0.0;
  auto tilesToPM = [&](const tile_t (&T)[6]) {
#pragma unroll
    for (int t = 0; t < 6; ++t)
#pragma unroll
      for (int q = 0; q < 4; ++q) sm[S::PM + LDP * (16 * TA[t] + 4 * q + g) + 16 * TB[t] + li] = T[t][q];
  };
  rd2 pv[NP];
  auto readP = [&]() {
#pragma unroll
    for (int t = 0; t < NP; ++t) {
      unsigned pk = pmPk[t];
      asm volatile("" : "+v"(pk));
      pv[t].x = ldsAt(sm, pk & 0xffffu); pv[t].y = ldsAt(sm, pk >> 16);
    }
  };
  auto writeP = [&](double* __restrict__ rr) {
#pragma unroll
    for (int t = 0; t < NP; ++t) { const int e2 = lane + 64 * t < N2 ? lane + 64 * t : N2 - 1; reinterpret_cast<rd2*>(rr)[e2] = pv[t]; }
  };
  auto writeGain = [&](double* __restrict__ gg) {
    rd2 gv[NG];
#pragma unroll
    for (int t = 0; t < NG; ++t) {
      unsigned pk = gnPk[t];
      asm volatile("" : "+v"(pk));
      gv[t].x = ldsAt(sm, pk & 0xffffu); gv[t].y = ldsAt(sm, pk >> 16);
    }
#pragma unroll
    for (int t = 0; t < NG; ++t) { const int e2 = lane + 64 * t < G2 ? lane + 64 * t : G2 - 1; reinterpret_cast<rd2*>(gg)[e2] = gv[t]; }
  };
  auto mirrorP = [&](const tile_t (&T)[6]) {
    const bool c4 = li < 4;
#pragma unroll
    for (int q = 0; q < 4; ++q) {
      const bool r0 = (q == 0);
      Pt[2][0][q] = r0 ? T[0][q] : 0.0;
      Pt[2][1][q] = r0 ? T[1][q] : 0.0;
      Pt[0][1][q] = T[4][q];
      Pt[1][0][q] = sm[S::PM + LDP * li + 16 + 4 * q + g];
      const double m02 = sm[S::PM + LDP * (32 + (c4 ? li : 0)) + 4 * q + g];
      const double m12 = sm[S::PM + LDP * (32 + (c4 ? li : 0)) + 16 + 4 * q + g];
      Pt[0][2][q] = c4 ? m02 : 0.0;
      Pt[1][2][q] = c4 ? m12 : 0.0;
      const int ir = 4 * q + g;
      const double d0 = sm[S::PM + LDP * li + ir], d1 = sm[S::PM + LDP * (16 + li) + 16 + ir], d2 = sm[S::PM + LDP * (32 + li) + 32 + ir];
      Pt[0][0][q] = ir <= li ? T[3][q] : d0;
      Pt[1][1][q] = ir <= li ? T[5][q] : d1;
      Pt[2][2][q] = (r0 && c4) ? (ir <= li ? T[2][q] : d2) : 0.0;
    }
  };
  {
    const double* __restrict__ kk = B.kkt + (base + slotOf(M - 1)) * L::KKT;
    double* __restrict__ rr = B.ric + (base + slotOf(M - 1)) * L::RIC;
    tile_t T[6];
#pragma unroll
    for (int t = 0; t < 6; ++t)
#pragma unroll
      for (int q = 0; q < 4; ++q) {
        const int ni = SL::nat(16 * TA[t] + 4 * q + g), nj = SL::nat(16 * TB[t] + li);
        const bool in = ni < NX && nj < NX && ((ni < NV) == (nj < NV));
        const double v = kk[in ? L::K_QXX + L::xsym(ni, nj) : 0];
        T[t][q] = in ? st32(v) : 0.0;
      }
    if (lane < NX) s_reg = st32(-kk[L::K_LX + myNat]);
    if (lane < 48) sm[S::VS + lane] = s_reg;
    tilesToPM(T);
    waveLdsSync();
    mirrorP(T);
    readP();
    writeP(rr);
    waveLdsSync();
  }
  constexpr int SL2 = (ZERO_AT + 2) / 2, PF = (SL2 + 63) / 64;
  static_assert(ZERO_AT % 2 == 0 && 2 * SL2 <= L::KKT && 2 * SL2 <= 48 * LDP && S::PM % 2 == 0 && L::KKT % 2 == 0, "the staged record fits the record and the PM block");
  rd2 pre[PF];
  auto prefetch = [&](const double* __restrict__ kk) {
    const rd2* __restrict__ k2 = reinterpret_cast<const rd2*>(kk);
#pragma unroll
    for (int t = 0; t < PF; ++t) { const int e = lane + 64 * t; pre[t] = k2[e < SL2 ? e : SL2 - 1]; }
  };
  double Cd[6][3], lz = 0.0, fx = 0.0;
  tile_t Qc[6];
  auto stageIn = [&]() {
#pragma unroll
    for (int t = 0; t < PF; ++t) { const int e = lane + 64 * t; if (64 * t + 63 < SL2 || e < SL2) reinterpret_cast<rd2*>(&sm[S::PM])[e] = pre[t]; }
    waveLdsSync();
    const double* kk = &sm[S::PM];
#pragma unroll
    for (int e = 0; e < 9; ++e) {
      unsigned pk = cqPk[e];
      asm volatile("" : "+v"(pk));
      const int e0 = 2 * e, e1 = 2 * e + 1;
      Cd[e0 / 3][e0 % 3] = ldsAt(kk, pk & 0xffffu);
      Cd[e1 / 3][e1 % 3] = ldsAt(kk, pk >> 16);
    }
    lz = kk[lzOff];
    fx = kk[L::K_FX + (myNat < NX ? myNat : 0)];
    waveLdsSync();
  };
  auto gatherQ = [&]() {
    const double* kk = &sm[S::PM];
#pragma unroll
    for (int e = 9; e < 21; ++e) {
      unsigned pk = cqPk[e];
      asm volatile("" : "+v"(pk));
      const int e0 = 2 * e - 18, e1 = 2 * e - 17;
      Qc[e0 / 4][e0 % 4] = ldsAt(kk, pk & 0xffffu);
      Qc[e1 / 4][e1 % 4] = ldsAt(kk, pk >> 16);
    }
  };
  if (M > 1) { prefetch(B.kkt + (base + slotOf(M - 2)) * L::KKT); stageIn(); }
  int n_slot = M > 1 ? nodes[M - 2].slot : 0, n_dimi = (HYBRID && M > 1) ? nodes[M - 2].sw_dimi : 0;
  double n_dt = M > 1 ? nodes[M - 2].dtq : 0.0;
  for (int i = M - 2; i >= 0; --i) {
    const double dt = n_dt;
    const long rec = base + __builtin_amdgcn_readfirstlane(n_slot);
    const int dimi = HYBRID ? __builtin_amdgcn_readfirstlane(n_dimi) : 0;
    if (i > 0) { n_slot = nodes[i - 1].slot; n_dt = nodes[i - 1].dtq; if (HYBRID) n_dimi = nodes[i - 1].sw_dimi; }
    const bool constrained = HYBRID && dimi > 0;
#ifdef IDOCP_S3_STAMPS
    const bool stamp = lane == 0 && b == (gridDim.x > 7 ? 7 : 0) && i == M / 2 && B.prof != nullptr;
#define RSTAMP(k) do { if (stamp) B.prof[16 + k] = wall_clock64(); } while (0)
    const bool cstamp = lane == 0 && b == (gridDim.x > 7 ? 7 : 0) && constrained && B.prof != nullptr;
#define CSTAMP(k) do { if (cstamp) B.prof[32 + k] = wall_clock64(); } while (0)
#else
#define RSTAMP(k) do { } while (0)
#define CSTAMP(k) do { } while (0)
#endif
    RSTAMP(0);
    double* __restrict__ rr = B.ric + rec * L::RIC;
    double* __restrict__ gg = B.gain + rec * L::GAIN;
    tile_t Wt[3][3];
#pragma unroll
    for (int a = 0; a < 3; ++a)
#pragma unroll
      for (int bb = 0; bb < 3; ++bb) Wt[a][bb] = tile_t{0.0, 0.0, 0.0, 0.0};
#ifndef IDOCP_S3_MFMA4
#define IDOCP_S3_MFMA4 1
#endif
    auto quadToRow = [&](double v) -> double {
      int lo = __double2loint(v), hi = __double2hiint(v);
      lo = __builtin_amdgcn_update_dpp(lo, lo, 0x114, 0xF, 0x2, false);
      hi = __builtin_amdgcn_update_dpp(hi, hi, 0x114, 0xF, 0x2, false);
      lo = __builtin_amdgcn_update_dpp(lo, lo, 0x118, 0xF, 0xC, false);
      hi = __builtin_amdgcn_update_dpp(hi, hi, 0x118, 0xF, 0xC, false);
      return __hiloint2double(hi, lo);
    };
    auto phase1 = [&](auto dtag) {
      constexpr int d = decltype(dtag)::value;
#pragma unroll
      for (int a = 0; a < (IDOCP_S3_MFMA4 ? 2 : 3); ++a)
#pragma unroll
        for (int bb = 0; bb < 3; ++bb) Wt[a][bb] = __builtin_amdgcn_mfma_f64_16x16x4f64(Pt[DC[d]][a][DS[d]], Cd[d][bb], Wt[a][bb], 0, 0, 0);
      if (IDOCP_S3_MFMA4) {
        const double p4 = quadToRow(Pt[DC[d]][2][DS[d]]);
#pragma unroll
        for (int bb = 0; bb < 3; ++bb) Wt[2][bb][0] = __builtin_amdgcn_mfma_f64_4x4x4f64(p4, Cd[d][bb], Wt[2][bb][0], 0, 0, 0);
      }
    };
    if (lane < 48) sm[S::VF + lane] = lane < NX ? fx : 0.0;
    waveLdsSync();
    double lzh = 0.0;
    {
      double part[3] = {0.0, 0.0, 0.0};
      double fr[9];
#pragma unroll
      for (int a = 0; a < 3; ++a)
#pragma unroll
        for (int q = 0; q < (a < 2 ? 4 : 1); ++q) fr[4 * a + q] = sm[S::VF + 16 * a + 4 * q + g];
      phase1(std::integral_constant<int, 0>{});
#pragma unroll
      for (int a = 0; a < 3; ++a)
#pragma unroll
        for (int q = 0; q < (a < 2 ? 4 : 1); ++q)
#pragma unroll
          for (int bb = 0; bb < 3; ++bb) part[bb] += Pt[a][bb][q] * fr[4 * a + q];
#pragma unroll
      for (int bb = 0; bb < 3; ++bb) sm[S::RED + 64 * bb + lane] = part[bb];
      waveLdsSync();
      const int rb = S::RED + 64 * (lane < 48 ? (lane >> 4) : 0) + li;
      const double r0 = sm[rb], r1 = sm[rb + 16], r2 = sm[rb + 32], r3 = sm[rb + 48];
      phase1(std::integral_constant<int, 1>{});
      const double y = (r0 + r1) + (r2 + r3);
      const double t = lane < NX ? y - s_reg : 0.0;
      waveLdsSync();
      if (lane < 48) sm[S::VT + lane] = t;
      waveLdsSync();
      double tv[6];
#pragma unroll
      for (int d = 0; d < 6; ++d) tv[d] = sm[S::VT + 16 * DC[d] + 4 * DS[d] + g];
      const double ts = sm[S::VT + (lane < 12 ? lane : (lane >= 16 && lane < 28 ? lane - 16 : 0))];
      phase1(std::integral_constant<int, 2>{});
#pragma unroll
      for (int bb = 0; bb < 3; ++bb) part[bb] = 0.0;
#pragma unroll
      for (int d = 0; d < 6; ++d)
#pragma unroll
        for (int bb = 0; bb < 3; ++bb) part[bb] += Cd[d][bb] * tv[d];
#pragma unroll
      for (int bb = 0; bb < 3; ++bb) sm[S::RED + 64 * bb + lane] = part[bb];
      waveLdsSync();
// ... 232 lines not shown
          double acc = 0.0;
          for (int l = 0; l < dimi_; ++l) acc += Phix[l + NF * lane] * sm[S::MV + l];
          sm[S::SCORR + lane] = acc;
        }
        waveLdsSync();
      };
      if (dimi == 6) switchingRows(std::integral_constant<int, 6>{}); else switchingRows(std::integral_constant<int, 0>{});
      CSTAMP(6);
      riccatiPhase4<D, true, 0, 3>(Quu, &sm[S::KM], &sm[S::GK], lane);
      waveLdsSync();
      RSTAMP(10);
      for (int e = lane; e < NU * NX / 2; e += 64) reinterpret_cast<rd2*>(gg)[e] = reinterpret_cast<const rd2*>(&sm[S::KM])[e];
      if (lane < NU) gg[L::G_k + lane] = sm[S::KVN + lane];
      static_assert(S::KM % 2 == 0 && L::G_K == 0 && (NU * NX) % 2 == 0, "K is one contiguous copy");
      if (lane < NX) {
        double hk = 0.0;
#pragma unroll
        for (int m = 0; m < NU; ++m) hk += Qxu[myNat + NX * m] * sm[S::KVN + m];
        s_reg = st32(-lzh - hk - sm[S::SCORR + myNat]);
      }
      RSTAMP(4);
      CSTAMP(7);
      double Gr[3][3], Dr[3][3];
#pragma unroll
      for (int a = 0; a < 3; ++a)
#pragma unroll
        for (int s = 0; s < 3; ++s) {
          const int c = 16 * a + li, cn = NU * SL::nat(c < NX ? c : 0) + 4 * s + g;
          const double kv = sm[S::KM + cn], gv = sm[S::GK + cn], dv = sm[S::DTM + cn];
          Kr[a][s] = c < NX ? -kv : 0.0;
          Gr[a][s] = c < NX ? gv + dv : 0.0;
          Dr[a][s] = c < NX ? dv : 0.0;
        }
#pragma unroll
      for (int t = 0; t < 6; ++t) {
        Pn[t] = Qh[t];
        if (TA[t] == 2) { Pn[t][1] = 0.0; Pn[t][2] = 0.0; Pn[t][3] = 0.0; }
      }
#pragma unroll
      for (int s = 0; s < 3; ++s)
#pragma unroll
        for (int t = 0; t < 6; ++t) {
          Pn[t] = __builtin_amdgcn_mfma_f64_16x16x4f64(Kr[TA[t]][s], Gr[TB[t]][s], Pn[t], 0, 0, 0);
          Pn[t] = __builtin_amdgcn_mfma_f64_16x16x4f64(Dr[TA[t]][s], Kr[TB[t]][s], Pn[t], 0, 0, 0);
        }
    }
    RSTAMP(5);
    CSTAMP(8);
    if (p32) {
#pragma unroll
      for (int t = 0; t < 6; ++t)
#pragma unroll
        for (int q = 0; q < 4; ++q) Pn[t][q] = (double)(float)Pn[t][q];
    }
    waveLdsSync();
    if (lane < 48) sm[S::VS + lane] = s_reg;
    tilesToPM(Pn);
    waveLdsSync();
    mirrorP(Pn);
    readP();
    waveLdsSync();
    RSTAMP(7);
    if (i > 0) stageIn();
    writeP(rr);
    RSTAMP(8);
    CSTAMP(15);
#undef RSTAMP
#undef CSTAMP
  }
  if (lane == 0 && !s_ok && B.status[b] == 0) B.status[b] = 1;
}

template <typename D>
__global__ __launch_bounds__(64) void ocp_riccati_forward_kernel(OcpBuffers B, const double* __restrict__ q0,
                                                                const double* __restrict__ v0) {
  using L = OcpLayout<D>;
  constexpr int NV = D::NV, NQ = D::NQ, NX = D::NX, NU = D::NU;
  typedef double d2 __attribute__((ext_vector_type(2)));
  constexpr int FO = L::K_FQQ, FL = L::K_FX + NX - L::K_FQQ, GL = L::GAIN;
  static_assert(FO % 2 == 0 && FL % 2 == 0 && GL % 2 == 0 && L::KKT % 2 == 0, "16-byte loads");
  constexpr int F2 = FL / 2, G2 = GL / 2, NF2 = (F2 + 63) / 64, NG2 = (G2 + 63) / 64;
  __shared__ __attribute__((aligned(16))) double fb[FL], gb[GL];
  __shared__ double dx[NX], du[NU], dxn[NX];
  constexpr int MAXM = 1024;
  __shared__ int s_slot[MAXM];
  __shared__ double s_dtq[MAXM];
  const OcpProblem* __restrict__ P = B.prob;
  const int M = B.M;
  const OcpNode* __restrict__ nodes = B.nodes;
  const int lane = threadIdx.x;
  const long b = blockIdx.x;
  const long base = b * B.NS;
  const bool tab = M <= MAXM;
  if (tab) {
    for (int i = lane; i < M; i += 64) { s_slot[i] = nodes[i].slot; s_dtq[i] = nodes[i].dtq; }
    waveLdsSync();
  }
  auto slotOf = [&](int i) -> int { return tab ? s_slot[i] : nodes[i].slot; };
  d2 frA[NF2], grA[NG2], frB[NF2], grB[NG2];
  auto fetch = [&](int i, d2 (&fr)[NF2], d2 (&gr)[NG2]) {
    const long rec = base + slotOf(i);
    const d2* __restrict__ fp = reinterpret_cast<const d2*>(B.kkt + rec * L::KKT + FO);
    const d2* __restrict__ gp = reinterpret_cast<const d2*>(B.gain + rec * L::GAIN);
#pragma unroll
    for (int t = 0; t < NF2; ++t) { const int e = lane + 64 * t; fr[t] = fp[e < F2 ? e : F2 - 1]; }
#pragma unroll
    for (int t = 0; t < NG2; ++t) { const int e = lane + 64 * t; gr[t] = gp[e < G2 ? e : G2 - 1]; }
  };
  if (M > 1) fetch(0, frA, grA);
  if (M > 2) fetch(1, frB, grB);
  const double* __restrict__ s0 = B.sol + (base + slotOf(0)) * L::SOL;
  if (lane == 0) {
    double R[9], p[3], d6[6];
    lieRelative(s0 + L::S_Q, q0 + b * NQ, R, p);
    lieLog6(R, p, d6);
    const double* __restrict__ Fi = B.exp + (base + slotOf(0)) * L::EXP + L::E_FQQPI;
    for (int r = 0; r < 6; ++r) { double acc = 0.0; for (int m = 0; m < 6; ++m) acc += Fi[r + 6 * m] * d6[m]; dx[r] = -acc; }
  }
  if (lane >= 6 && lane < NV) dx[lane] = q0[b * NQ + lane + 1] - s0[L::S_Q + lane + 1];
  if (lane < NV) dx[NV + lane] = v0[b * NV + lane] - s0[L::S_V + lane];
  const double* Fqq6 = fb + (L::K_FQQ - FO);
  const double* Fqv6 = fb + (L::K_FQV - FO);
  const double* Fvq = fb + (L::K_FVQ - FO);
  const double* Fvv = fb + (L::K_FVV - FO);
  const double* Fvu = fb + (L::K_FVU - FO);
  const double* Fx = fb + (L::K_FX - FO);
  auto step = [&](int i, d2 (&fr)[NF2], d2 (&gr)[NG2]) {
    const long rec = base + slotOf(i);
    const double dt = tab ? s_dtq[i] : nodes[i].dtq;
    double* __restrict__ dd = B.dir + rec * L::DIR;
#pragma unroll
    for (int t = 0; t < NF2; ++t) { const int e = lane + 64 * t; if (e < F2) reinterpret_cast<d2*>(fb)[e] = fr[t]; }
#pragma unroll
    for (int t = 0; t < NG2; ++t) { const int e = lane + 64 * t; if (e < G2) reinterpret_cast<d2*>(gb)[e] = gr[t]; }
    waveLdsSync();
    if (i + 2 < M - 1) fetch(i + 2, fr, gr);
    {
      const int j = lane >> 2, part = lane & 3;
      double acc = 0.0;
      if (lane < 4 * NU) {
#pragma unroll
        for (int t = 0; t < NX / 4; ++t) { const int c = (NX / 4) * part + t; acc += gb[L::G_K + j + NU * c] * dx[c]; }
      }
      acc += __shfl_xor(acc, 1);
      acc += __shfl_xor(acc, 2);
      if (lane < 4 * NU && part == 0) { acc += gb[L::G_k + j]; du[j] = acc; dd[L::D_U + j] = acc; }
    }
    if (lane < NV) { dd[L::D_Q + lane] = dx[lane]; dd[L::D_V + lane] = dx[NV + lane]; }
    waveLdsSync();
    {
      double acc = 0.0;
      if (lane < 2 * NV) {
        const int r = lane >> 1, half = lane & 1;
        const double* Fm = half ? Fvv : Fvq;
        const double* xs = half ? dx + NV : dx;
#pragma unroll
        for (int c = 0; c < NV; ++c) acc += Fm[r + NV * c] * xs[c];
#pragma unroll
        for (int j = 0; j < NU / 2; ++j) acc += Fvu[r + NV * ((NU / 2) * half + j)] * du[(NU / 2) * half + j];
      }
      acc += __shfl_xor(acc, 1);
      if (lane < 2 * NV && (lane & 1) == 0) dxn[NV + (lane >> 1)] = acc + Fx[NV + (lane >> 1)];
      if (lane >= 2 * NV && lane < 3 * NV) {
        const int r = lane - 2 * NV;
        double dq = Fx[r];
        if (r < 6) {
#pragma unroll
          for (int m = 0; m < 6; ++m) dq += Fqq6[r + 6 * m] * dx[m] + Fqv6[r + 6 * m] * dx[NV + m];
        } else {
          dq += dx[r] + dt * dx[NV + r];
        }
        dxn[r] = dq;
      }
    }
    waveLdsSync();
    if (lane < NX) dx[lane] = dxn[lane];
    waveLdsSync();
  };
  for (int i = 0; i < M - 1; i += 2) {
    step(i, frA, grA);
    if (i + 1 < M - 1) step(i + 1, frB, grB);
  }
  double* __restrict__ dd = B.dir + (base + slotOf(M - 1)) * L::DIR;
  if (lane < NV) { dd[L::D_Q + lane] = dx[lane]; dd[L::D_V + lane] = dx[NV + lane]; }
}

template <typename D>
void OcpLaunch<D>::riccatiBackward(const OcpBuffers& B, long batch, int M, bool hybrid, hipStream_t st, bool wide) {
  (void)M;
  const size_t smem = RiccatiSmem<D>::TOTAL * sizeof(double), smem_h = smem;
  static bool configured = false;
  if (!configured) {
    (void)hipFuncSetAttribute((const void*)ocp_riccati_backward_kernel<D, 256, false>, hipFuncAttributeMaxDynamicSharedMemorySize, (int)smem);
    (void)hipFuncSetAttribute((const void*)ocp_riccati_backward_kernel<D, 128, false>, hipFuncAttributeMaxDynamicSharedMemorySize, (int)smem);
    (void)hipFuncSetAttribute((const void*)ocp_riccati_backward_kernel<D, 64, false>, hipFuncAttributeMaxDynamicSharedMemorySize, (int)smem);
    (void)hipFuncSetAttribute((const void*)ocp_riccati_backward_kernel<D, 128, true>, hipFuncAttributeMaxDynamicSharedMemorySize, (int)smem_h);
    (void)hipFuncSetAttribute((const void*)ocp_riccati_backward_kernel<D, 256, true>, hipFuncAttributeMaxDynamicSharedMemorySize, (int)smem_h);
    (void)hipFuncSetAttribute((const void*)ocp_riccati_backward_kernel<D, 64, true>, hipFuncAttributeMaxDynamicSharedMemorySize, (int)smem_h);
    (void)hipFuncSetAttribute((const void*)ocp_riccati_backward_kernel<D, 512, true>, hipFuncAttributeMaxDynamicSharedMemorySize, (int)smem_h);
    (void)hipFuncSetAttribute((const void*)ocp_riccati_backward_kernel<D, 512, false>, hipFuncAttributeMaxDynamicSharedMemorySize, (int)smem);
    configured = true;
  }
  static const int nt_env = getenv("IDOCP_RICCATI_NT") ? atoi(getenv("IDOCP_RICCATI_NT")) : 0;
  static const int reg_env = getenv("IDOCP_RICCATI_REG") ? atoi(getenv("IDOCP_RICCATI_REG")) : 1;
  if (nt_env == 512 || (nt_env == 0 && wide)) {
    if (hybrid) hipLaunchKernelGGL((ocp_riccati_backward_kernel<D, 512, true>), dim3((unsigned)batch), dim3(512), smem_h, st, B);
    else hipLaunchKernelGGL((ocp_riccati_backward_kernel<D, 512, false>), dim3((unsigned)batch), dim3(512), smem, st, B);
    return;
  }
  if (reg_env && nt_env == 0) {
    const size_t rs = RiccatiRegSmem<D>::BYTES;
    static bool reg_configured = false;
    if (!reg_configured) {
      (void)hipFuncSetAttribute((const void*)ocp_riccati_backward_reg_kernel<D, false>, hipFuncAttributeMaxDynamicSharedMemorySize, (int)rs);
      (void)hipFuncSetAttribute((const void*)ocp_riccati_backward_reg_kernel<D, true>, hipFuncAttributeMaxDynamicSharedMemorySize, (int)rs);
      reg_configured = true;
    }
    if (hybrid) hipLaunchKernelGGL((ocp_riccati_backward_reg_kernel<D, true>), dim3((unsigned)batch), dim3(64), rs, st, B);
    else hipLaunchKernelGGL((ocp_riccati_backward_reg_kernel<D, false>), dim3((unsigned)batch), dim3(64), rs, st, B);
    return;
  }
  if (hybrid) {
    if (nt_env == 64 || (nt_env == 0 && batch >= 1024)) hipLaunchKernelGGL((ocp_riccati_backward_kernel<D, 64, true>), dim3((unsigned)batch), dim3(64), smem_h, st, B);
    else if (nt_env == 256 || (nt_env == 0 && batch < 512)) hipLaunchKernelGGL((ocp_riccati_backward_kernel<D, 256, true>), dim3((unsigned)batch), dim3(256), smem_h, st, B);
    else hipLaunchKernelGGL((ocp_riccati_backward_kernel<D, 128, true>), dim3((unsigned)batch), dim3(128), smem_h, st, B);
    return;
  }
  if (nt_env == 128) hipLaunchKernelGGL((ocp_riccati_backward_kernel<D, 128, false>), dim3((unsigned)batch), dim3(128), smem, st, B);
  else if (nt_env == 256) hipLaunchKernelGGL((ocp_riccati_backward_kernel<D, 256, false>), dim3((unsigned)batch), dim3(256), smem, st, B);
  else if (nt_env == 64) hipLaunchKernelGGL((ocp_riccati_backward_kernel<D, 64, false>), dim3((unsigned)batch), dim3(64), smem, st, B);
  else if (batch >= 512) hipLaunchKernelGGL((ocp_riccati_backward_kernel<D, 128, false>), dim3((unsigned)batch), dim3(128), smem, st, B);
  else hipLaunchKernelGGL((ocp_riccati_backward_kernel<D, 256, false>), dim3((unsigned)batch), dim3(256), smem, st, B);
}
template <typename D>
void OcpLaunch<D>::riccatiForward(const OcpBuffers& B, long batch, int M, const double* q0, const double* v0, hipStream_t st) {
  (void)M;
  hipLaunchKernelGGL((ocp_riccati_forward_kernel<D>), dim3((unsigned)batch), dim3(64), 0, st, B, q0, v0);
}

template void OcpLaunch<LeggedDims<4, 3>>::riccatiBackward(const OcpBuffers&, long, int, bool, hipStream_t, bool);
// ... 4 lines not shown
```

### idocp_amd/csrc/parnmpc_event_kernels.hip

```cpp
#include <hip/hip_runtime.h>

#include <cstdlib>

#include "dev_dense.hpp"
#include "dev_lie.hpp"
#include "ocp_device.hpp"
#include "ocp_launch.hpp"

namespace idocp_dev {

namespace {


}

template <typename D, bool RESIDUAL, bool MERIT = false>
__global__ __launch_bounds__(256) void parnmpc_impulse_condense_kernel(OcpBuffers B, const double* __restrict__ q0, const double* __restrict__ v0) {
  using L = OcpLayout<D>;
  constexpr int NV = D::NV, NQ = D::NQ, NX = D::NX, NF = D::NF, NVF = D::NVF, NU = D::NU, NC = D::NC;
  __shared__ double Mi[NV * NV], Fvq[NV * NV], Fvf[NV * NF], Vq[NF * NV], Vv[NF * NV], dIq[NV * NV];
  __shared__ double lq[NV], lv[NV], ldv[NV], lf[NF], Fq[NV], Fv[NV], ImD[NV], Vr[NF], MiI[NV], qdd[NV], mu_p[NF], f_p[NF], err[256];
  __shared__ double Qff[NF * NF], Jq6[36], Fqq6[36], FqqI[36], FqqP[36], Fq6[6];
  __shared__ int s_ok;
  const OcpProblem* __restrict__ P = B.prob;
// ... 119 lines not shown
    if (tid < ni) e += lf[tid] * lf[tid] + Vr[tid] * Vr[tid];
    err[tid] = e;
    blockLdsSync();
    if (tid == 0) { double acc = 0.0; for (int t = 0; t < 256; ++t) acc += err[t]; B.err_stage[rec] = acc; }
    return;
  }
  double* __restrict__ kk = B.kkt + rec * L::KKT;
  double* __restrict__ ee = B.exp + rec * L::EXP;
  double* __restrict__ W = B.swc + rec * L::SWC;
  if (tid < 36) {
    const int c = tid / 6, r = tid - 6 * c;
    double acc = 0.0;
    for (int m = 0; m < 6; ++m) acc += FqqI[r + 6 * m] * FqqP[m + 6 * c];
    kk[L::K_FQQ + tid] = acc;
    kk[L::K_FQV + tid] = 0.0;
    ee[L::E_FQQPI + tid] = FqqI[tid];
  } else if (tid >= 64 && tid < 70) {
    const int r = tid - 64;
    double acc = 0.0;
    for (int m = 0; m < 6; ++m) acc += FqqI[r + 6 * m] * Fq6[m];
    Fq[r] = acc;
  }
  blockLdsSync();
  if (tid < 64) spdInverseRows<NV>(Mi, NV, NV, tid, &s_ok);
  blockLdsSync();
  for (int e = tid; e < NV * NV; e += 256) {
    const int c = e / NV, r = e - c * NV;
    double acc = 0.0;
    for (int m = 0; m < NV; ++m) acc += Mi[r + NV * m] * dIq[m + NV * c];
    Fvq[e] = -acc;
  }
  for (int e = tid; e < NV * ni; e += 256) {
    const int j = e / NV, r = e - j * NV;
    double acc = 0.0;
    for (int m = 0; m < NV; ++m) acc += Mi[r + NV * m] * Vv[j + NF * m];
    Fvf[r + NV * j] = acc;
  }
  if (tid >= 192 && tid < 192 + NV) {
    const int r = tid - 192;
    double acc = 0.0;
    for (int m = 0; m < NV; ++m) acc += Mi[r + NV * m] * ImD[m];
    MiI[r] = acc;
  }
  blockLdsSync();
  if (tid < NV) ldv[tid] -= P->dvi_weight[tid] * MiI[tid];
  blockLdsSync();
  for (int e = tid; e < NX * NX; e += 256) {
    const int c = e / NX, r = e - c * NX;
    double v = 0.0;
    if (r < NV && c < NV) {
      if (r < 6 && c < 6) { for (int m2 = 0; m2 < 6; ++m2) v += Jq6[m2 + 6 * r] * P->qi_weight[m2] * Jq6[m2 + 6 * c]; }
      else if (r == c) v = P->qi_weight[r];
      double acc = 0.0;
      for (int m = 0; m < NV; ++m) acc += Fvq[m + NV * r] * (P->dvi_weight[m] * Fvq[m + NV * c]);
      v += acc;
      if (B.ext) {
        const double* __restrict__ xx = B.ext + rec * L::EXT;
        for (int k = 0; k < 6 * L::NT; ++k) v += xx[L::X_TW + k] * xx[L::X_TJ + k * NV + r] * xx[L::X_TJ + k * NV + c];
      }
    } else if (r == c) {
      v = P->vi_weight[r - NV];
    }
    if (r <= c) kk[L::K_QXX + L::xsym(r, c)] = v;
  }
  for (int e = tid; e < NX * NU; e += 256) {
    const int j = e / NX, r = e - j * NX;
    double v = 0.0;
    if (r < NV && j < ni) for (int m = 0; m < NV; ++m) v += Fvq[m + NV * r] * (P->dvi_weight[m] * Fvf[m + NV * j]);
    kk[L::K_QXU + e] = v;
  }
  for (int e = tid; e < NU * NU; e += 256) {
    const int c = e / NU, r = e - c * NU;
    double v = 0.0;
    if (r < ni && c < ni) {
      v = Qff[r + NF * c];
      double acc = 0.0;
      for (int m = 0; m < NV; ++m) acc += Fvf[m + NV * r] * (P->dvi_weight[m] * Fvf[m + NV * c]);
      v += acc;
    } else if (r == c) v = 1.0;
    kk[L::K_QUU + e] = v;
  }
  for (int e = tid; e < NV * NV; e += 256) {
    const int c = e / NV, r = e - c * NV;
    kk[L::K_FVQ + e] = Fvq[e];
    kk[L::K_FVV + e] = (r == c) ? -1.0 : 0.0;
    if (r >= c) ee[L::E_MJ + r * (r + 1) / 2 + c] = Mi[e];
  }
  for (int e = tid; e < NV * NU; e += 256) {
    const int j = e / NV;
    kk[L::K_FVU + e] = j < ni ? Fvf[e] : 0.0;
  }
  if (tid < NV) {
    const int r = tid;
    double aq = 0.0;
    for (int m = 0; m < NV; ++m) aq += Fvq[m + NV * r] * ldv[m];
    kk[L::K_LX + r] = lq[r] + aq;
    kk[L::K_LX + NV + r] = lv[r];
    kk[L::K_FX + r] = Fq[r];
    kk[L::K_FX + NV + r] = Fv[r] - MiI[r];
    ee[L::E_MJIDC + r] = MiI[r];
    ee[L::E_LAF + r] = ldv[r];
    ee[L::E_QAA + r] = P->dvi_weight[r];
  }
  if (tid >= 64 && tid < 64 + NU) {
    const int j = tid - 64;
    double v = 0.0;
    if (j < ni) { v = lf[j]; double af = 0.0; for (int m = 0; m < NV; ++m) af += Fvf[m + NV * j] * ldv[m]; v += af; }
    kk[L::K_LU + j] = v;
  }
  if (tid >= 128 && tid < 128 + NF) W[L::W_P + tid - 128] = (tid - 128 < ni) ? Vr[tid - 128] : 0.0;
  for (int e = tid; e < NF * NX; e += 256) {
    const int c = e / NF, j = e - c * NF;
    W[L::W_PHIX + e] = j < ni ? (c < NV ? Vq[j + NF * c] : Vv[j + NF * (c - NV)]) : 0.0;
  }
  if (tid == 0 && !s_ok && B.status[b] == 0) B.status[b] = 2000 + pos;
}

template <typename D>
struct KktInvEventSmem {
  static constexpr int NX = D::NX, NU = D::NU, NF = D::NF, NQ_ = NU + NX, NR = NX + NF;
  static_assert(NQ_ == NR && NR % 3 == 0 && (NR / 3) * (NR / 3) <= 256, "square 48 x 48 tiles, one per thread");
  static constexpr int A = 0, B = A + NQ_ * NQ_, PV = B + NR * NQ_,
                       R1 = PV + 2 * (2 * NQ_ + 2), R2 = R1 + NR, T1 = R2 + NQ_, W = T1 + NR, DIR = W + NQ_, TOTAL = DIR + NR + NQ_ + 4;
};

template <typename D>
__global__ __launch_bounds__(256) void parnmpc_kkt_inverse_general_kernel(OcpBuffers B) {
  using L = OcpLayout<D>;
  using S = KktInvEventSmem<D>;
  constexpr int NV = D::NV, NX = D::NX, NU = D::NU, NF = D::NF, NC = D::NC, NQ = S::NQ_, NR = S::NR;
  constexpr int TQ = NQ / 3;
  extern __shared__ __attribute__((aligned(16))) double sm[];
  __shared__ int s_ok;
  const OcpProblem* __restrict__ P = B.prob;
  const int M = B.M;
  const int tid = threadIdx.x, nt = 256;
  const long b = blockIdx.x;
  const int pos = B.general_pos[blockIdx.y];
  const OcpNode* __restrict__ nd = B.nodes + pos;
  const ParnmpcShape sh = parnmpcShape<L>(*nd);
  const int ni = sh.ni, nw = sh.nw, nr = NX + ni, nK = sh.nk;
  const bool impulse = sh.impulse;
  const bool last = P->has_terminal && (pos == M - 2);
  const double dt = nd->dt;
  const long rec = b * B.NS + nd->slot;
  const double* __restrict__ kk = B.kkt + rec * L::KKT;
  const double* __restrict__ Wc = B.swc + rec * L::SWC;
  const double* __restrict__ aux = B.aux + (b * B.NS + nd->next) * L::AUX;
  double* __restrict__ ki = B.kinv + rec * L::KINV;
  if (tid == 0) s_ok = 1;
  double qinv[3][3];
  const int ti = tid % TQ, tj = tid / TQ;
#pragma unroll
  for (int tr = 0; tr < 3; ++tr)
#pragma unroll
    for (int tc = 0; tc < 3; ++tc) {
      const int r = 3 * ti + tr, c = 3 * tj + tc;
      double v;
      if (r < NU && c < NU) v = (r < nw && c < nw) ? kk[L::K_QUU + r + NU * c] : (r == c ? 1.0 : 0.0);
      else if (r < NU) v = r < nw ? kk[L::K_QXU + (c - NU) + NX * r] : 0.0;
      else if (c < NU) v = c < nw ? kk[L::K_QXU + (r - NU) + NX * c] : 0.0;
      else {
        int rr = r - NU, cc = c - NU;
        const double ax = last ? 0.0 : aux[rr + NX * cc];
        if (rr > cc) { const int t = rr; rr = cc; cc = t; }
        v = kk[L::K_QXX + L::xsym(rr, cc)] + ax;
      }
      qinv[tr][tc] = v;
    }
  for (int e = tid; e < NR * NQ; e += nt) {
    const int c = e / NR, r = e - c * NR;
    double v = 0.0;
    if (r < NV) {
      if (c >= NU && c < NU + NV) { const int cq = c - NU; v = (r < 6 && cq < 6) ? kk[L::K_FQQ + r + 6 * cq] : ((r >= 6 && r == cq) ? -1.0 : 0.0); }
      else if (c >= NU + NV && !impulse) { const int cv = c - NU - NV; v = (r < 6 && cv < 6) ? kk[L::K_FQV + r + 6 * cv] : ((r >= 6 && r == cv) ? dt : 0.0); }
    } else if (r < NX) {
      const int rv = r - NV;
      if (c < NU) v = c < nw ? kk[L::K_FVU + rv + NV * c] : 0.0;
      else if (c < NU + NV) v = kk[L::K_FVQ + rv + NV * (c - NU)];
      else v = kk[L::K_FVV + rv + NV * (c - NU - NV)];
    } else if (r < nr && c >= NU) {
      v = Wc[L::W_PHIX + (r - NX) + NF * (c - NU)];
    }
    sm[S::B + e] = v;
  }
  if (tid < NR) sm[S::R1 + tid] = tid < NX ? kk[L::K_FX + tid] : (tid < nr ? Wc[L::W_P + tid - NX] : 0.0);
  if (tid >= 64 && tid < 64 + NQ) { const int r = tid - 64; sm[S::R2 + r] = r < NU ? (r < nw ? kk[L::K_LU + r] : 0.0) : kk[L::K_LX + r - NU]; }
  blockLdsSync();
  gaussJordanTiles<NQ>(qinv, true, ti, tj, &sm[S::PV], &s_ok);
#pragma unroll
  for (int tr = 0; tr < 3; ++tr)
#pragma unroll
    for (int tc = 0; tc < 3; ++tc) sm[S::A + 3 * ti + tr + NQ * (3 * tj + tc)] = qinv[tr][tc];
  blockLdsSync();
  double acc[3][3] = {{0.0, 0.0, 0.0}, {0.0, 0.0, 0.0}, {0.0, 0.0, 0.0}};
  tileMM<NQ>(acc, [&](int r, int m) { return sm[S::B + 3 * ti + r + NR * m]; },
             [&](int m, int c) { return sm[S::A + m + NQ * (3 * tj + c)]; });
  if (tid < NQ) {
    double w = 0.0;
    for (int m = 0; m < NQ; ++m) w += sm[S::A + tid + NQ * m] * sm[S::R2 + m];
    sm[S::W + tid] = w;
  }
  blockLdsSync();
#pragma unroll
  for (int tr = 0; tr < 3; ++tr)
#pragma unroll
    for (int tc = 0; tc < 3; ++tc) sm[S::A + 3 * ti + tr + NR * (3 * tj + tc)] = acc[tr][tc];
  blockLdsSync();
  double sinv[3][3] = {{0.0, 0.0, 0.0}, {0.0, 0.0, 0.0}, {0.0, 0.0, 0.0}};
  tileMM<NQ>(sinv, [&](int r, int m) { return sm[S::B + 3 * ti + r + NR * m]; },
             [&](int m, int c) { return sm[S::A + 3 * tj + c + NR * m]; });
  if (ti == tj) {
#pragma unroll
    for (int t3 = 0; t3 < 3; ++t3) if (3 * ti + t3 >= nr) sinv[t3][t3] = 1.0;
  }
  gaussJordanTiles<NR>(sinv, true, ti, tj, &sm[S::PV], &s_ok);
#pragma unroll
  for (int tr = 0; tr < 3; ++tr)
#pragma unroll
    for (int tc = 0; tc < 3; ++tc) sm[S::B + 3 * ti + tr + NR * (3 * tj + tc)] = sinv[tr][tc];
  blockLdsSync();
#pragma unroll
  for (int tr = 0; tr < 3; ++tr)
#pragma unroll
    for (int tc = 0; tc < 3; ++tc) acc[tr][tc] = 0.0;
  tileMM<NR>(acc, [&](int r, int m) { return sm[S::B + 3 * ti + r + NR * m]; },
             [&](int m, int c) { return sm[S::A + m + NR * (3 * tj + c)]; });
  if (tid < NR) {
    const int r = tid;
    double t = sm[S::R1 + r];
    for (int m = 0; m < NQ; ++m) t -= sm[S::A + r + NR * m] * sm[S::R2 + m];
    sm[S::T1 + r] = t;
    double d = 0.0;
    for (int m = 0; m < NR; ++m) d -= sm[S::B + r + NR * m] * sm[S::R1 + m];
    sm[S::DIR + r] = d;
  }
  for (int e = tid; e < nr * NX; e += nt) {
    const int c = e / nr, r = e - c * nr;
    ki[L::I_C0 + r + L::NKG * c] = -sm[S::B + r + NR * c];
  }
  blockLdsSync();
#pragma unroll
  for (int tr = 0; tr < 3; ++tr)
#pragma unroll
    for (int tc = 0; tc < 3; ++tc) sm[S::B + 3 * ti + tr + NR * (3 * tj + tc)] = acc[tr][tc];
  blockLdsSync();
  const bool b_on = tj >= NU / 3;
  if (b_on) {
#pragma unroll
    for (int tr = 0; tr < 3; ++tr)
#pragma unroll
      for (int tc = 0; tc < 3; ++tc) acc[tr][tc] = 0.0;
    tileMM<NR>(acc, [&](int r, int m) { return sm[S::B + m + NR * (3 * ti + r)]; },
               [&](int m, int c) { return sm[S::A + m + NR * (3 * tj + c)]; });
  } else if (tid < NR) {
    double d = sm[S::DIR + tid];
    for (int m = 0; m < NQ; ++m) d += sm[S::B + tid + NR * m] * sm[S::R2 + m];
    sm[S::DIR + tid] = d;
  }
  if (tid >= 256 - NQ) {
    const int r = tid - (256 - NQ);
    double d = sm[S::W + r];
    for (int m = 0; m < NR; ++m) d += sm[S::B + m + NR * r] * sm[S::T1 + m];
// ... 83 lines not shown
```

### idocp_amd/csrc/parnmpc_kernels.hip

```cpp
#include <hip/hip_runtime.h>

#include <cstdlib>
#include <type_traits>

#include "dev_dense.hpp"
#include "dev_lie.hpp"
#include "ocp_device.hpp"
#include "ocp_launch.hpp"

namespace idocp_dev {

template <typename D>
struct KktInvSmem {
  static constexpr int NX = D::NX, NU = D::NU, NQ_ = NU + NX;
  static constexpr int A = 0, B = A + NQ_ * NQ_, PV = B + NX * NQ_,
                       R1 = PV + 2 * (2 * NQ_ + 2), R2 = R1 + NX, T1 = R2 + NQ_, W = T1 + NQ_, DIR = W + NQ_, TOTAL = DIR + NX + NQ_ + 4;
  static_assert(NX % 3 == 0 && NQ_ % 3 == 0 && NU % 3 == 0, "3 x 3 tiles");
  static_assert((NQ_ / 3) * (NQ_ / 3) <= 256, "one tile per thread");
  static_assert((NQ_ / 3) * (NX / 3) + NQ_ <= 256 && (NQ_ / 3) * (NX / 3) + NX <= 256, "side jobs next to the NX x NQ tiles");
};

template <typename D>
__global__ __launch_bounds__(256) void parnmpc_kkt_inverse_kernel(OcpBuffers B) {
  using L = OcpLayout<D>;
  using S = KktInvSmem<D>;
  constexpr int NV = D::NV, NQc = D::NQ, NX = D::NX, NU = D::NU, NQ = S::NQ_, NK = L::NK;
  constexpr int TQ = NQ / 3, TX = NX / 3, TU = NU / 3;
  extern __shared__ __attribute__((aligned(16))) double sm[];
  __shared__ int s_ok;
  const OcpProblem* __restrict__ P = B.prob;
  const int M = B.M;
  const int tid = threadIdx.x, nt = 256;
  const long unit = blockIdx.x;
  const long b = unit / (M - 1);
  const int pos = (int)(unit - b * (M - 1));
  const OcpNode* __restrict__ nd = B.nodes + pos;
  if (parnmpcShape<L>(*nd).general) return;
  const bool last = P->has_terminal && (pos == M - 2);
  const double dt = nd->dt;
  const long rec = b * B.NS + nd->slot;
  const double* __restrict__ kk = B.kkt + rec * L::KKT;
  const double* __restrict__ aux = B.aux + (b * B.NS + nd->next) * L::AUX;
  double* __restrict__ ki = B.kinv + rec * L::KINV;
  if (tid == 0) s_ok = 1;
  double qinv[3][3];
  const int qi = tid % TQ, qj = tid / TQ;
  const bool q_on = tid < TQ * TQ;
#pragma unroll
  for (int tr = 0; tr < 3; ++tr)
#pragma unroll
    for (int tc = 0; tc < 3; ++tc) {
      const int r = 3 * qi + tr, c = 3 * qj + tc;
      double v = 0.0;
      if (q_on) {
        if (r < NU && c < NU) v = kk[L::K_QUU + r + NU * c];
        else if (r < NU) v = kk[L::K_QXU + (c - NU) + NX * r];
        else if (c < NU) v = kk[L::K_QXU + (r - NU) + NX * c];
        else {
          int rr = r - NU, cc = c - NU;
          const double ax = last ? 0.0 : aux[rr + NX * cc];
          if (rr > cc) { const int t = rr; rr = cc; cc = t; }
          v = kk[L::K_QXX + L::xsym(rr, cc)] + ax;
        }
      }
      qinv[tr][tc] = v;
    }
  for (int e = tid; e < NX * NQ; e += nt) {
    const int c = e / NX, r = e - c * NX;
    double v = 0.0;
    if (r < NV) {
      if (c >= NU && c < NU + NV) { const int cq = c - NU; v = (r < 6 && cq < 6) ? kk[L::K_FQQ + r + 6 * cq] : ((r >= 6 && r == cq) ? -1.0 : 0.0); }
      else if (c >= NU + NV) { const int cv = c - NU - NV; v = (r < 6 && cv < 6) ? kk[L::K_FQV + r + 6 * cv] : ((r >= 6 && r == cv) ? dt : 0.0); }
    } else {
      const int rv = r - NV;
      if (c < NU) v = kk[L::K_FVU + rv + NV * c];
      else if (c < NU + NV) v = kk[L::K_FVQ + rv + NV * (c - NU)];
      else v = kk[L::K_FVV + rv + NV * (c - NU - NV)];
    }
    sm[S::B + e] = v;
  }
  if (tid < NX) sm[S::R1 + tid] = kk[L::K_FX + tid];
  if (tid >= 64 && tid < 64 + NU) sm[S::R2 + tid - 64] = kk[L::K_LU + tid - 64];
  if (tid >= 128 && tid < 128 + NX) sm[S::R2 + NU + tid - 128] = kk[L::K_LX + tid - 128];
  blockLdsSync();
  gaussJordanTiles<NQ>(qinv, q_on, qi, qj, &sm[S::PV], &s_ok);
  if (q_on) {
#pragma unroll
    for (int tr = 0; tr < 3; ++tr)
#pragma unroll
      for (int tc = 0; tc < 3; ++tc) sm[S::A + 3 * qi + tr + NQ * (3 * qj + tc)] = qinv[tr][tc];
  }
  blockLdsSync();
  const int fi = tid % TX, fj = tid / TX;
  const bool f_on = tid < TX * TQ;
  double acc[3][3] = {{0.0, 0.0, 0.0}, {0.0, 0.0, 0.0}, {0.0, 0.0, 0.0}};
  if (f_on) {
    tileMM<NQ>(acc, [&](int r, int m) { return sm[S::B + 3 * fi + r + NX * m]; },
               [&](int m, int c) { return sm[S::A + m + NQ * (3 * fj + c)]; });
  } else if (tid < TX * TQ + NQ) {
    const int r = tid - TX * TQ;
    double w = 0.0;
    for (int m = 0; m < NQ; ++m) w += sm[S::A + r + NQ * m] * sm[S::R2 + m];
    sm[S::W + r] = w;
  }
  blockLdsSync();
  if (f_on) {
#pragma unroll
    for (int tr = 0; tr < 3; ++tr)
#pragma unroll
      for (int tc = 0; tc < 3; ++tc) sm[S::A + 3 * fi + tr + NX * (3 * fj + tc)] = acc[tr][tc];
  }
  blockLdsSync();
  const bool s_on = tid < TX * TX;
  double sinv[3][3] = {{0.0, 0.0, 0.0}, {0.0, 0.0, 0.0}, {0.0, 0.0, 0.0}};
  if (s_on)
    tileMM<NQ>(sinv, [&](int r, int m) { return sm[S::B + 3 * fi + r + NX * m]; },
               [&](int m, int c) { return sm[S::A + 3 * fj + c + NX * m]; });
  gaussJordanTiles<NX>(sinv, s_on, fi, fj, &sm[S::PV], &s_ok);
  if (s_on) {
#pragma unroll
    for (int tr = 0; tr < 3; ++tr)
#pragma unroll
      for (int tc = 0; tc < 3; ++tc) sm[S::B + 3 * fi + tr + NX * (3 * fj + tc)] = sinv[tr][tc];
  }
  blockLdsSync();
#pragma unroll
  for (int tr = 0; tr < 3; ++tr)
#pragma unroll
    for (int tc = 0; tc < 3; ++tc) acc[tr][tc] = 0.0;
  if (f_on) {
    tileMM<NX>(acc, [&](int r, int m) { return sm[S::B + 3 * fi + r + NX * m]; },
               [&](int m, int c) { return sm[S::A + m + NX * (3 * fj + c)]; });
  } else if (tid < TX * TQ + NX) {
    const int r = tid - TX * TQ;
    double t = sm[S::R1 + r];
    for (int m = 0; m < NQ; ++m) t -= sm[S::A + r + NX * m] * sm[S::R2 + m];
    sm[S::T1 + r] = t;
    double d = 0.0;
    for (int m = 0; m < NX; ++m) d -= sm[S::B + r + NX * m] * sm[S::R1 + m];
    sm[S::DIR + r] = d;
  }
  for (int e = tid; e < NX * NX; e += nt) {
    const int c = e / NX, r = e - c * NX;
    ki[L::I_C0 + r + NK * c] = -sm[S::B + e];
  }
  blockLdsSync();
  if (f_on) {
#pragma unroll
    for (int tr = 0; tr < 3; ++tr)
#pragma unroll
      for (int tc = 0; tc < 3; ++tc) sm[S::B + 3 * fi + tr + NX * (3 * fj + tc)] = acc[tr][tc];
  }
  blockLdsSync();
  const bool b_on = q_on && qj >= TU;
  if (b_on) {
#pragma unroll
    for (int tr = 0; tr < 3; ++tr)
#pragma unroll
      for (int tc = 0; tc < 3; ++tc) acc[tr][tc] = 0.0;
    tileMM<NX>(acc, [&](int r, int m) { return sm[S::B + m + NX * (3 * qi + r)]; },
// ... 537 lines not shown
```

### idocp_amd/csrc/parnmpc_kkt_wave_kernel.hip

```cpp
#include <hip/hip_runtime.h>

#include <type_traits>

#include "dev_dense.hpp"
#include "dev_lie.hpp"
#include "ocp_device.hpp"
#include "ocp_launch.hpp"

namespace idocp_dev {

typedef mfma_d4 wtile;
typedef double v2d __attribute__((ext_vector_type(2)));

template <typename D>
struct KktWaveSmem {
  using L = OcpLayout<D>;
  static constexpr int NX = D::NX, NU = D::NU, NQ_ = NU + NX;
  static_assert(NQ_ == 48 && NX == 36, "three 16 x 16 blocks for (u, q, v); S = 16 + 16 + 4");
  static constexpr int LDT = 18;
  static constexpr int QPART = L::K_QUU + NU * NU;
  static constexpr int FPART = L::K_FX + NX - QPART;
  static constexpr int NBUF = 6 * 256 + 3 * 64;
  static_assert(L::K_QXX == 0 && L::K_QXU < L::K_QUU && L::K_FQQ == QPART && QPART % 2 == 0 && FPART % 2 == 0, "record order");
  static_assert(NX * NX <= NBUF && QPART <= NBUF && FPART <= NBUF && L::NK * 16 <= NBUF, "everything that passes through BUF");
// ... 189 lines not shown
    const v2d lo = reinterpret_cast<const v2d*>(&sm[S::BUF + 256 * slot + o])[0], hi = reinterpret_cast<const v2d*>(&sm[S::BUF + 256 * slot + o])[1];
    return wtile{lo.x, lo.y, hi.x, hi.y};
  };

  wtile Wq[6];
  {
    wtile A[6];
#pragma unroll
    for (int t = 0; t < TA; ++t) { const int e = lane + 64 * t; if (e < NA2) reinterpret_cast<v2d*>(&sm[S::BUF])[e] = last ? v2d{0.0, 0.0} : rvA[t]; }
    waveLdsSync();
    KSTAMP(1);
#pragma unroll
    for (int it = 0; it < 3; ++it)
#pragma unroll
      for (int jt = it; jt < 3; ++jt)
#pragma unroll
        for (int q = 0; q < 4; ++q) {
          const int r = 16 * it + 4 * q + g, c = 16 * jt + li;
          const bool xx = r >= NU && c >= NU;
          const int lo = r < c ? r : c, hi = r < c ? c : r;
          A[U3(it, jt)][q] = sm[xx ? S::BUF + (lo - NU) + NX * (hi - NU) : S::CPAD];
        }
    waveLdsSync();
#pragma unroll
    for (int t = 0; t < TQ; ++t) { const int e = lane + 64 * t; if (e < NQ2) reinterpret_cast<v2d*>(&sm[S::BUF])[e] = rvQ[t]; }
    waveLdsSync();
#pragma unroll
    for (int it = 0; it < 3; ++it)
#pragma unroll
      for (int jt = it; jt < 3; ++jt)
#pragma unroll
        for (int q = 0; q < 4; ++q) {
          const int r = 16 * it + 4 * q + g, c = 16 * jt + li;
          const int lo = r < c ? r : c, hi = r < c ? c : r;
          int ad;
          if (hi < NU) ad = L::K_QUU + lo + NU * hi;
          else if (lo < NU) ad = L::K_QXU + (hi - NU) + NX * lo;
          else { const int rr = lo - NU, cc = hi - NU; ad = L::K_QXX + cc * (cc + 1) / 2 + rr; }
          A[U3(it, jt)][q] += sm[S::BUF + ad];
        }
    waveLdsSync();
    KSTAMP(2);
    cholInv3(A, Wq, std::integral_constant<int, 16>{});
  }
#pragma unroll
  for (int t = 0; t < TF; ++t) { const int e = lane + 64 * t; if (e < NF2) reinterpret_cast<v2d*>(&sm[S::BUF])[e] = rvF[t]; }
  waveLdsSync();
  if (lane < NX) sm[S::R1 + lane] = sm[S::BUF + (L::K_FX - S::QPART) + lane];
  KSTAMP(3);

  auto stageTile = [&](const wtile& Z, int r0, int nrow, int c0, int ncol) {
#pragma unroll
    for (int q = 0; q < 4; ++q) {
      const int c = c0 + 4 * q + g;
      sm[(li < nrow && c >= 0 && c < ncol) ? S::BUF + (r0 + li) + NK * c : S::DUMP] = Z[q];
    }
  };
  auto flushBlock = [&](int first_col, int ncol) {
    waveLdsSync();
    const int n2 = NK * ncol / 2;
    v2d* __restrict__ dst = reinterpret_cast<v2d*>(ki + (long)NK * first_col);
#pragma unroll
    for (int t = 0; t < (NK * 16 / 2 + 63) / 64; ++t) {
      const int e = lane + 64 * t;
      if (64 * t + 63 < n2 || e < n2) dst[e] = reinterpret_cast<const v2d*>(&sm[S::BUF])[e];
    }
    waveLdsSync();
  };
  double pt[3] = {0.0, 0.0, 0.0}, pb[3] = {0.0, 0.0, 0.0};

  auto ftRow = [&](int kt, wtile (&Fr)[3]) {
#pragma unroll
    for (int jt = 0; jt < 3; ++jt)
#pragma unroll
      for (int q = 0; q < 4; ++q) {
        const int z = 16 * kt + 4 * q + g, e = 16 * jt + li;
        int ad = S::CPAD;
        if (e < NV) {
          if (z >= NU && z < NU + NV) { const int cq = z - NU; ad = (e < 6 && cq < 6) ? S::BUF - S::QPART + L::K_FQQ + e + 6 * cq : ((e >= 6 && e == cq) ? S::CPAD + 1 : S::CPAD); }
          else if (z >= NU + NV) { const int cv = z - NU - NV; ad = (e < 6 && cv < 6) ? S::BUF - S::QPART + L::K_FQV + e + 6 * cv : ((e >= 6 && e == cv) ? S::CPAD + 2 : S::CPAD); }
        } else if (e < NX) {
          const int rv_ = e - NV;
          if (z < NU) ad = S::BUF - S::QPART + L::K_FVU + rv_ + NV * z;
          else if (z < NU + NV) ad = S::BUF - S::QPART + L::K_FVQ + rv_ + NV * (z - NU);
          else ad = S::BUF - S::QPART + L::K_FVV + rv_ + NV * (z - NU - NV);
        } else if (e == NX) {
          ad = z < NU ? S::BUF - S::QPART + L::K_LU + z : S::BUF - S::QPART + L::K_LX + (z - NU);
        }
        Fr[jt][q] = sm[ad];
      }
  };
  wtile Sm[6];
  {
    wtile Y[3][3];
#pragma unroll
    for (int it = 0; it < 3; ++it)
#pragma unroll
      for (int jt = 0; jt < 3; ++jt) Y[it][jt] = wzero();
#pragma unroll
    for (int kt = 0; kt < 3; ++kt) {
      wtile Fr[3];
      ftRow(kt, Fr);
#pragma unroll
      for (int it = kt; it < 3; ++it) {
        const wtile Gt = transposeTile(Wq[U3(kt, it)]);
#pragma unroll
        for (int jt = 0; jt < 3; ++jt) pAcc(Y[it][jt], Gt, Fr[jt]);
      }
      __builtin_amdgcn_sched_barrier(0);
    }
    KSTAMP(4);
    if (li == 4) {
#pragma unroll
      for (int it = 0; it < 3; ++it)
#pragma unroll
        for (int q = 0; q < 4; ++q) sm[S::Y2 + 16 * it + 4 * q + g] = Y[it][2][q];
    }
    waveLdsSync();
    {
      double y2v[3][4];
#pragma unroll
      for (int it = 0; it < 3; ++it)
#pragma unroll
        for (int q = 0; q < 4; ++q) y2v[it][q] = sm[S::Y2 + 16 * it + 4 * q + g];
#pragma unroll
      for (int jt = 0; jt < 3; ++jt)
#pragma unroll
        for (int kt = jt; kt < 3; ++kt)
#pragma unroll
          for (int q = 0; q < 4; ++q) pb[jt] += Wq[U3(jt, kt)][q] * y2v[kt][q];
      asm volatile("" : "+v"(pb[0]), "+v"(pb[1]), "+v"(pb[2]));
    }
    __builtin_amdgcn_sched_barrier(0);
#pragma unroll
    for (int it = 0; it < 3; ++it)
#pragma unroll
      for (int jt = it; jt < 3; ++jt) {
        wtile Z = wzero();
#pragma unroll
        for (int kt = jt; kt < 3; ++kt) pAcc(Z, Wq[U3(it, kt)], Wq[U3(jt, kt)]);
        reinterpret_cast<v2d*>(scr + 256 * U3(it, jt))[2 * lane] = v2d{Z[0], Z[1]};
        reinterpret_cast<v2d*>(scr + 256 * U3(it, jt))[2 * lane + 1] = v2d{Z[2], Z[3]};
        __builtin_amdgcn_sched_barrier(0);
      }
    waveLdsSync();
#pragma unroll
    for (int it = 0; it < 3; ++it)
#pragma unroll
      for (int jt = 0; jt < 3; ++jt) {
        wtile Z = wzero();
#pragma unroll
        for (int kt = jt; kt < 3; ++kt) { if (it == 2) pAcc4(Z, Y[kt][it], Wq[U3(jt, kt)]); else pAcc(Z, Y[kt][it], Wq[U3(jt, kt)]); }
        if (it < 2) parkTile(3 * it + jt, Z);
        else sm[S::BUF + 6 * 256 + 64 * jt + lane] = Z[0];
        __builtin_amdgcn_sched_barrier(0);
      }
#pragma unroll
    for (int it = 0; it < 3; ++it)
#pragma unroll
      for (int jt = it; jt < 3; ++jt) {
        Sm[U3(it, jt)] = wzero();
#pragma unroll
        for (int kt = 0; kt < 3; ++kt) { if (it == 2) pAcc4(Sm[U3(it, jt)], Y[kt][it], Y[kt][jt]); else pAcc(Sm[U3(it, jt)], Y[kt][it], Y[kt][jt]); }
      }
  }
  if (li == 4) {
#pragma unroll
    for (int it = 0; it < 3; ++it)
#pragma unroll
      for (int q = 0; q < 4; ++q) {
        const int row = 16 * it + 4 * q + g;
        sm[S::T1 + row] = row < NX ? sm[S::R1 + (row < NX ? row : 0)] - Sm[U3(it, 2)][q] : 0.0;
// ... 313 lines not shown
          A[U3(it, jt)][q] = sm[xx ? S::BUF + (lo - NU) + NX * (hi - NU) : S::CPAD];
        }
    waveLdsSync();
#pragma unroll
    for (int t = 0; t < TQ; ++t) { const int e = lane + 64 * t; if (e < NQ2) reinterpret_cast<v2d*>(&sm[S::BUF])[e] = rvQ[t]; }
    waveLdsSync();
#pragma unroll
    for (int it = 0; it < 3; ++it)
#pragma unroll
      for (int jt = it; jt < 3; ++jt)
#pragma unroll
        for (int q = 0; q < 4; ++q) {
          const int r = 16 * it + 4 * q + g, c = 16 * jt + li;
          const int lo = r < c ? r : c, hi = r < c ? c : r;
          int ad;
          if (hi < NU) ad = (hi < nw) ? S::BUF + L::K_QUU + lo + NU * hi : (lo == hi ? S::CPAD + 3 : S::CPAD);
          else if (lo < NU) ad = lo < nw ? S::BUF + L::K_QXU + (hi - NU) + NX * lo : S::CPAD;
          else { const int rr = lo - NU, cc = hi - NU; ad = S::BUF + L::K_QXX + cc * (cc + 1) / 2 + rr; }
          A[U3(it, jt)][q] += sm[ad];
        }
    waveLdsSync();
    KSTAMP(2);
    cholInv3(A, Wq, std::integral_constant<int, 16>{});
  }
#pragma unroll
  for (int t = 0; t < TF; ++t) { const int e = lane + 64 * t; if (e < NF2) reinterpret_cast<v2d*>(&sm[S::BUF])[e] = rvF[t]; }
  waveLdsSync();
#pragma unroll
  for (int t = 0; t < TP; ++t) { const int e = lane + 64 * t; if (e < NP2) reinterpret_cast<v2d*>(&sm[S::BUF + S::PHIX])[e] = rvP[t]; }
  if (lane < NX) sm[S::R1 + lane] = sm[S::BUF + (L::K_FX - S::QPART) + lane];
  if (lane < NF) sm[S::R1 + NX + lane] = lane < ni ? wp_r : 0.0;
  waveLdsSync();
  KSTAMP(3);

  auto stageTile = [&](const wtile& Z, int r0, int nrow, int c0, int ncol) {
#pragma unroll
    for (int q = 0; q < 4; ++q) {
      const int c = c0 + 4 * q + g;
      sm[(li < nrow && c >= 0 && c < ncol) ? S::BUF + (r0 + li) + NK * c : S::DUMP] = Z[q];
    }
  };
  auto stageVarTile = [&](const wtile& Z, int bz, int c0, int ncol) {
    const int z = 16 * bz + li;
    const int vrow = z < NU ? (z < nw ? nr + z : -1) : nr + nw + (z - NU);
#pragma unroll
    for (int q = 0; q < 4; ++q) {
      const int c = c0 + 4 * q + g;
      if (vrow >= 0 && c >= 0 && c < ncol) sm[S::BUF + vrow + NK * c] = Z[q];
    }
  };
  auto flushBlock = [&](int first_col, int ncol) {
    waveLdsSync();
    const int n2 = NK * ncol / 2;
    v2d* __restrict__ dst = reinterpret_cast<v2d*>(ki + (long)NK * first_col);
#pragma unroll
    for (int t = 0; t < (NK * 16 / 2 + 63) / 64; ++t) {
      const int e = lane + 64 * t;
      if (64 * t + 63 < n2 || e < n2) dst[e] = reinterpret_cast<const v2d*>(&sm[S::BUF])[e];
    }
    waveLdsSync();
  };
  auto reduceRows = [&](const double (&p)[3], double* out) {
#pragma unroll
    for (int jt = 0; jt < 3; ++jt) sm[S::RED + 48 * g + 16 * jt + li] = p[jt];
    waveLdsSync();
    if (lane < 48) out[lane] = (sm[S::RED + lane] + sm[S::RED + 48 + lane]) + (sm[S::RED + 96 + lane] + sm[S::RED + 144 + lane]);
    waveLdsSync();
  };
  double pt[3] = {0.0, 0.0, 0.0}, pb[3] = {0.0, 0.0, 0.0};

  auto ftRow = [&](int kt, wtile (&Fr)[3]) {
#pragma unroll
    for (int jt = 0; jt < 3; ++jt)
#pragma unroll
      for (int q = 0; q < 4; ++q) {
        const int z = 16 * kt + 4 * q + g, e = 16 * jt + li;
        int ad = S::CPAD;
        if (e < NV) {
          if (z >= NU && z < NU + NV) { const int cq = z - NU; ad = (e < 6 && cq < 6) ? S::BUF - S::QPART + L::K_FQQ + e + 6 * cq : ((e >= 6 && e == cq) ? S::CPAD + 1 : S::CPAD); }
          else if (z >= NU + NV && !impulse) { const int cv = z - NU - NV; ad = (e < 6 && cv < 6) ? S::BUF - S::QPART + L::K_FQV + e + 6 * cv : ((e >= 6 && e == cv) ? S::CPAD + 2 : S::CPAD); }
        } else if (e < NX) {
          const int rv_ = e - NV;
          if (z < NU) ad = z < nw ? S::BUF - S::QPART + L::K_FVU + rv_ + NV * z : S::CPAD;
          else if (z < NU + NV) ad = S::BUF - S::QPART + L::K_FVQ + rv_ + NV * (z - NU);
          else ad = S::BUF - S::QPART + L::K_FVV + rv_ + NV * (z - NU - NV);
        } else if (e < nr && z >= NU) {
          ad = S::BUF + S::PHIX + (e - NX) + NF * (z - NU);
        }
        Fr[jt][q] = sm[ad];
      }
  };
  wtile Sm[6];
  {
    wtile Y[3][3];
#pragma unroll
    for (int it = 0; it < 3; ++it)
#pragma unroll
      for (int jt = 0; jt < 3; ++jt) Y[it][jt] = wzero();
    double py[3] = {0.0, 0.0, 0.0};
#pragma unroll
    for (int kt = 0; kt < 3; ++kt) {
      wtile Fr[3];
      ftRow(kt, Fr);
      double r2v[4];
#pragma unroll
      for (int q = 0; q < 4; ++q) {
        const int z = 16 * kt + 4 * q + g;
        r2v[q] = sm[z < NU ? (z < nw ? S::BUF - S::QPART + L::K_LU + z : S::CPAD) : S::BUF - S::QPART + L::K_LX + (z - NU)];
      }
#pragma unroll
      for (int it = kt; it < 3; ++it) {
        const wtile Gt = transposeTile(Wq[U3(kt, it)]);
#pragma unroll
        for (int q = 0; q < 4; ++q) py[it] += Gt[q] * r2v[q];
#pragma unroll
        for (int jt = 0; jt < 3; ++jt) pAcc(Y[it][jt], Gt, Fr[jt]);
      }
      __builtin_amdgcn_sched_barrier(0);
    }
    KSTAMP(4);
    reduceRows(py, &sm[S::Y2]);
    {
      double y2v[3][4];
#pragma unroll
      for (int it = 0; it < 3; ++it)
#pragma unroll
        for (int q = 0; q < 4; ++q) y2v[it][q] = sm[S::Y2 + 16 * it + 4 * q + g];
#pragma unroll
      for (int jt = 0; jt < 3; ++jt)
#pragma unroll
        for (int kt = jt; kt < 3; ++kt)
#pragma unroll
          for (int q = 0; q < 4; ++q) pb[jt] += Wq[U3(jt, kt)][q] * y2v[kt][q];
      double ps[3] = {0.0, 0.0, 0.0};
#pragma unroll
      for (int jt = 0; jt < 3; ++jt)
#pragma unroll
        for (int kt = 0; kt < 3; ++kt)
#pragma unroll
          for (int q = 0; q < 4; ++q) ps[jt] += Y[kt][jt][q] * y2v[kt][q];
      reduceRows(ps, &sm[S::T1]);
      if (lane < 48) sm[S::T1 + lane] = lane < nr ? sm[S::R1 + lane] - sm[S::T1 + lane] : 0.0;
      asm volatile("" : "+v"(pb[0]), "+v"(pb[1]), "+v"(pb[2]));
    }
    __builtin_amdgcn_sched_barrier(0);
#pragma unroll
    for (int it = 0; it < 3; ++it)
#pragma unroll
      for (int jt = it; jt < 3; ++jt) {
        wtile Z = wzero();
#pragma unroll
        for (int kt = jt; kt < 3; ++kt) pAcc(Z, Wq[U3(it, kt)], Wq[U3(jt, kt)]);
        reinterpret_cast<v2d*>(scr + 256 * U3(it, jt))[2 * lane] = v2d{Z[0], Z[1]};
        reinterpret_cast<v2d*>(scr + 256 * U3(it, jt))[2 * lane + 1] = v2d{Z[2], Z[3]};
        __builtin_amdgcn_sched_barrier(0);
      }
    waveLdsSync();
#pragma unroll
    for (int it = 0; it < 3; ++it)
#pragma unroll
      for (int jt = 0; jt < 3; ++jt) {
        wtile Z = wzero();
#pragma unroll
        for (int kt = jt; kt < 3; ++kt) pAcc(Z, Y[kt][it], Wq[U3(jt, kt)]);
        parkTile(3 * it + jt, Z);
        __builtin_amdgcn_sched_barrier(0);
      }
#pragma unroll
    for (int it = 0; it < 3; ++it)
#pragma unroll
      for (int jt = it; jt < 3; ++jt) {
        Sm[U3(it, jt)] = wzero();
// ... 180 lines not shown
```

Measured before the change: 219,000 SQP iterations/s.

## Store raw MJtJinv_dIDCdqv velocity rows once in KKT, rebuild Fvq/Fvv on the fly

The KKT record now stores the velocity rows of MJtJinv_dIDCdqv (X_q, X_v) instead of Fvq/Fvv. The exp record keeps only the contact rows, so the duplicate NV x NX block no longer has to be written and read in two places. Consumers (riccati, expand, forward, parnmpc kernels, host C API) rebuild Fv = -dt*X + identity on the fly through fvRow. This cuts global memory traffic and record size, at the cost of extra per-element arithmetic, a dt lookup per node, and many layout changes across kernels that could introduce errors.

```diff
diff --git a/idocp_amd/csrc/ocp_capi.hip b/idocp_amd/csrc/ocp_capi.hip
--- a/idocp_amd/csrc/ocp_capi.hip
+++ b/idocp_amd/csrc/ocp_capi.hip
@@ -1638,8 +1638,14 @@
     std::memcpy(&k[LQ::K_QUU], Quu, sizeof(double) * nu * nu);
     std::memcpy(&k[LQ::K_FQQ], Fqq6, sizeof(double) * 36);
     std::memcpy(&k[LQ::K_FQV], Fqv6, sizeof(double) * 36);
-    std::memcpy(&k[LQ::K_FVQ], Fvq, sizeof(double) * nv * nv);
-    std::memcpy(&k[LQ::K_FVV], Fvv, sizeof(double) * nv * nv);
+    double dts = 0.0;
+    for (const OcpNode& nd : h->chain) if (nd.slot == stage) dts = nd.dt;
+    if (!(dts > 0.0)) { set_last_error("idocp_ocp_set_lqr_stage: stage " + std::to_string(stage) + " is not a stage of the current discretisation"); return IDOCP_E_ARG; }
+    const double one = h->parnmpc ? -1.0 : 1.0;
+    for (int c = 0; c < nv; ++c) for (int r = 0; r < nv; ++r) {
+      k[LQ::K_MJDQ + r + nv * c] = -Fvq[r + nv * c] / dts;
+      k[LQ::K_MJDV + r + nv * c] = ((r == c ? one : 0.0) - Fvv[r + nv * c]) / dts;
+    }
     std::memcpy(&k[LQ::K_FVU], Fvu, sizeof(double) * nv * nu);
     std::memcpy(&k[LQ::K_LU], lu, sizeof(double) * nu);
     std::memcpy(&k[LQ::K_FX], Fx, sizeof(double) * nx);
@@ -1666,12 +1672,14 @@
 }
 static int getContactDynamics(idocp_ocp_t* h, int instance, int stage, int dimf, double* MJtJinv, double* MJtJinv_dIDCdqv, double* MJtJinv_IDC) {
   int rc = setDev(h); if (rc) return rc;
-  std::vector<double> e(LQ::EXP);
+  std::vector<double> e(LQ::EXP), k(LQ::KKT);
   HIP_TRY(hipMemcpyAsync(e.data(), h->B.exp + ((size_t)instance * h->NS + stage) * LQ::EXP, e.size() * sizeof(double), hipMemcpyDeviceToHost, h->stream));
+  HIP_TRY(hipMemcpyAsync(k.data(), h->B.kkt + ((size_t)instance * h->NS + stage) * LQ::KKT, k.size() * sizeof(double), hipMemcpyDeviceToHost, h->stream));
   HIP_TRY(hipStreamSynchronize(h->stream));
   const int n = DQ::NV + dimf;
   for (int c = 0; c < n; ++c) for (int r = 0; r < n; ++r) MJtJinv[r + n * c] = r >= c ? e[LQ::E_MJ + r * (r + 1) / 2 + c] : e[LQ::E_MJ + c * (c + 1) / 2 + r];
-  for (int c = 0; c < DQ::NX; ++c) for (int r = 0; r < n; ++r) MJtJinv_dIDCdqv[r + n * c] = e[LQ::E_MJD + r + DQ::NVF * c];
+  for (int c = 0; c < DQ::NX; ++c) for (int r = 0; r < n; ++r)
+    MJtJinv_dIDCdqv[r + n * c] = r < DQ::NV ? k[LQ::K_MJDQ + r + DQ::NV * c] : e[LQ::E_MJDC + (r - DQ::NV) + dimf * c];
   for (int r = 0; r < n; ++r) MJtJinv_IDC[r] = e[LQ::E_MJIDC + r];
   return dimf;
 }
@@ -1689,14 +1697,16 @@
   std::memcpy(Quu, &k[LQ::K_QUU], sizeof(double) * nu * nu);
   std::memset(A, 0, sizeof(double) * nx * nx);
   std::memset(Bm, 0, sizeof(double) * nx * nu);
-  double dt = h->T / h->N;
-  for (const OcpNode& nd : h->chain) if (nd.slot == stage) dt = nd.dtq;
+  double dt = h->T / h->N, dts = dt;
+  for (const OcpNode& nd : h->chain) if (nd.slot == stage) { dt = nd.dtq; dts = nd.dt; }
+  const double one = h->parnmpc ? -1.0 : 1.0;
   for (int c = 0; c < nv; ++c) for (int r = 0; r < nv; ++r) {
     double fqq = (r == c) ? 1.0 : 0.0, fqv = (r == c) ? dt : 0.0;
     if (r < 6 && c < 6) { fqq = k[LQ::K_FQQ + r + 6 * c]; fqv = k[LQ::K_FQV + r + 6 * c]; }
     else if (r < 6 || c < 6) { fqq = 0.0; fqv = 0.0; }
     A[r + nx * c] = fqq; A[r + nx * (nv + c)] = fqv;
-    A[(nv + r) + nx * c] = k[LQ::K_FVQ + r + nv * c]; A[(nv + r) + nx * (nv + c)] = k[LQ::K_FVV + r + nv * c];
+    A[(nv + r) + nx * c] = LQ::fvRow(k[LQ::K_MJDQ + r + nv * c], dts, r, c, one);
+    A[(nv + r) + nx * (nv + c)] = LQ::fvRow(k[LQ::K_MJDV + r + nv * c], dts, r, nv + c, one);
   }
   for (int j = 0; j < nu; ++j) for (int r = 0; r < nv; ++r) Bm[(nv + r) + nx * j] = k[LQ::K_FVU + r + nv * j];
   std::memcpy(lx, &k[LQ::K_LX], sizeof(double) * nx);
diff --git a/idocp_amd/csrc/ocp_condense_kernel.hip b/idocp_amd/csrc/ocp_condense_kernel.hip
--- a/idocp_amd/csrc/ocp_condense_kernel.hip
+++ b/idocp_amd/csrc/ocp_condense_kernel.hip
@@ -779,16 +779,10 @@
 
   STAMP(9);
   typedef double wd2 __attribute__((ext_vector_type(2)));
-  static_assert(NV % 2 == 0 && SVF % 2 == 0 && S::MJD % 2 == 0 && L::K_FVQ % 2 == 0 && L::K_FVV % 2 == 0 && L::KKT % 2 == 0, "16-byte stores of Fvq / Fvv");
-  for (int e = tid; e < NV * NV / 2; e += nt) {
+  static_assert(NV % 2 == 0 && SVF % 2 == 0 && S::MJD % 2 == 0 && L::K_MJDQ % 2 == 0 && L::K_MJDV == L::K_MJDQ + NV * NV && L::KKT % 2 == 0, "16-byte stores of the velocity rows");
+  for (int e = tid; e < (NV / 2) * NX; e += nt) {
     const int c = e / (NV / 2), r = 2 * (e - c * (NV / 2));
-    const wd2 mq = *reinterpret_cast<const wd2*>(&sm[S::MJD + r + SVF * c]), mvv = *reinterpret_cast<const wd2*>(&sm[S::MJD + r + SVF * (NV + c)]);
-    const double one = BWD ? -1.0 : 1.0;
-    wd2 fq, fv;
-    fq.x = -dt * mq.x; fq.y = -dt * mq.y;
-    fv.x = -dt * mvv.x + (r == c ? one : 0.0); fv.y = -dt * mvv.y + (r + 1 == c ? one : 0.0);
-    *reinterpret_cast<wd2*>(&kk[L::K_FVQ + r + NV * c]) = fq;
-    *reinterpret_cast<wd2*>(&kk[L::K_FVV + r + NV * c]) = fv;
+    *reinterpret_cast<wd2*>(&kk[L::K_MJDQ + r + NV * c]) = *reinterpret_cast<const wd2*>(&sm[S::MJD + r + SVF * c]);
   }
   for (int e = tid; e < NV * NU; e += nt) { const int c = e / NV, r = e - c * NV; kk[L::K_FVU + e] = hu * dt * sm[S::MJ + r + SVF * (6 + c)]; }
   if (tid < NV) {
@@ -802,10 +796,14 @@
     const int r = lo ? pr : RVF - 1 - pr, c = lo ? idx : idx - pr - 1;
     ee[L::E_MJ + r * (r + 1) / 2 + c] = sm[S::MJ + r + SVF * c];
   }
-  static_assert(RVF % 2 == 0 && NVF % 2 == 0 && L::E_MJD % 2 == 0 && L::EXP % 2 == 0, "16-byte stores of MJtJinv_dIDCdqv");
-  for (int e = tid; e < (RVF / 2) * NX; e += nt) {
-    const int c = e / (RVF / 2), r = 2 * (e - c * (RVF / 2));
-    *reinterpret_cast<wd2*>(&ee[L::E_MJD + r + NVF * c]) = *reinterpret_cast<const wd2*>(&sm[S::MJD + r + SVF * c]);
+  static_assert(L::E_MJDC % 2 == 0 && L::EXP % 2 == 0, "16-byte stores of the contact rows of MJtJinv_dIDCdqv");
+  if constexpr (DIMF > 0 && DIMF % 2 == 0) {
+    for (int e = tid; e < (DIMF / 2) * NX; e += nt) {
+      const int c = e / (DIMF / 2), r = 2 * (e - c * (DIMF / 2));
+      *reinterpret_cast<wd2*>(&ee[L::E_MJDC + r + DIMF * c]) = *reinterpret_cast<const wd2*>(&sm[S::MJD + NV + r + SVF * c]);
+    }
+  } else if constexpr (DIMF != 0) {
+    for (int e = tid; e < dimf * NX; e += nt) { const int c = e / dimfd, r = e - c * dimfd; ee[L::E_MJDC + e] = sm[S::MJD + NV + r + SVF * c]; }
   }
   if (tid < NV) ee[L::E_QAA + tid] = sm[S::QAA + tid];
   for (int e = tid; e < SF * SF; e += nt) { const int c = e / SF, r = e - c * SF; ee[L::E_QFF + r + NF * c] = sm[S::QFF + e]; }
diff --git a/idocp_amd/csrc/ocp_device.hpp b/idocp_amd/csrc/ocp_device.hpp
--- a/idocp_amd/csrc/ocp_device.hpp
+++ b/idocp_amd/csrc/ocp_device.hpp
@@ -29,14 +29,18 @@
   static constexpr int X_TRI = (NX * (NX + 1) / 2 + 1) / 2 * 2;
   __host__ __device__ static constexpr int xsym(int r, int c) { return r <= c ? c * (c + 1) / 2 + r : r * (r + 1) / 2 + c; }
   static constexpr int K_QXX = 0, K_QXU = X_TRI, K_QUU = K_QXU + NX * NU, K_FQQ = K_QUU + NU * NU, K_FQV = K_FQQ + 36,
-                       K_FVQ = K_FQV + 36, K_FVV = K_FVQ + NV * NV, K_FVU = K_FVV + NV * NV, K_LX = K_FVU + NV * NU,
+                       K_MJDQ = K_FQV + 36, K_MJDV = K_MJDQ + NV * NV, K_FVU = K_MJDV + NV * NV, K_LX = K_FVU + NV * NU,
                        K_LU = K_LX + NX, K_FX = K_LU + NU;
   static constexpr int KKT = roundUp16(K_FX + NX);
+  static_assert(K_MJDV == K_MJDQ + NV * NV && K_FVU == K_MJDQ + NV * NX, "[X_q X_v Fvu]: NV rows, NX + NU columns, contiguous");
+  static_assert(K_MJDQ % 2 == 0 && K_FVU % 2 == 0 && K_FX % 2 == 0 && KKT % 2 == 0, "16-byte pieces of the kkt record");
+  __host__ __device__ static constexpr double fvRow(double x, double dt, int r, int c, double one = 1.0) { return -dt * x + (c == NV + r ? one : 0.0); }
   static constexpr int MJ_TRI = (NVF * (NVF + 1) / 2 + 1) / 2 * 2;
-  static constexpr int E_MJ = 0, E_MJD = MJ_TRI, E_QAA = E_MJD + NVF * NX, E_QFF = E_QAA + NV,
+  static constexpr int E_MJ = 0, E_MJDC = MJ_TRI, E_QAA = E_MJDC + NF * NX, E_QFF = E_QAA + NV,
                        E_MJIDC = E_QFF + NF * NF, E_LAF = E_MJIDC + NVF, E_LUP = E_LAF + NVF, E_QUUP = E_LUP + 6,
                        E_QXUP = E_QUUP + 6 * NU, E_FQQPI = E_QXUP + NX * 6;
   static constexpr int EXP = roundUp16(E_FQQPI + 36);
+  static_assert(E_MJDC % 2 == 0 && (NF * NX) % 2 == 0 && EXP % 2 == 0, "16-byte pieces of the exp record");
   static constexpr int P_TRI = (NV * (NV + 1) / 2 + 1) / 2 * 2;
   __host__ __device__ static constexpr int psym(int r, int c) { return r <= c ? c * (c + 1) / 2 + r : r * (r + 1) / 2 + c; }
   static constexpr int R_PQQ = 0, R_PQV = P_TRI, R_PVV = R_PQV + NV * NV, R_SQ = R_PVV + P_TRI, R_SV = R_SQ + NV;
diff --git a/idocp_amd/csrc/ocp_expand_kernel.hip b/idocp_amd/csrc/ocp_expand_kernel.hip
--- a/idocp_amd/csrc/ocp_expand_kernel.hip
+++ b/idocp_amd/csrc/ocp_expand_kernel.hip
@@ -119,6 +119,47 @@
     if (e < n2) reinterpret_cast<ex_d2*>(dst)[c * LD2 + (e - c * h)] = r[t];
   }
 }
+template <typename L>
+struct MjdRegs {
+  static constexpr int TOP2 = L::NV * L::NX / 2, CON2 = L::NF * L::NX / 2, NT = (TOP2 + 63) / 64, NC = (CON2 + 63) / 64, N = NT + NC;
+  static_assert(L::K_MJDQ % 2 == 0 && L::E_MJDC % 2 == 0 && (L::NV * L::NX) % 2 == 0 && L::NX % 2 == 0 && L::NV % 2 == 0 && L::NVF % 2 == 0, "16-byte pieces");
+};
+template <typename L>
+__device__ __forceinline__ void wideLoadMjd(ex_d2 (&r)[MjdRegs<L>::N], const double* __restrict__ kkt_rec, const double* __restrict__ exp_rec, int lane, int dimf) {
+  using M = MjdRegs<L>;
+  const ex_d2* __restrict__ pt = reinterpret_cast<const ex_d2*>(kkt_rec + L::K_MJDQ);
+  const ex_d2* __restrict__ pc = reinterpret_cast<const ex_d2*>(exp_rec + L::E_MJDC);
+  const int n2 = dimf * (L::NX / 2), last = n2 > 0 ? n2 - 1 : 0;
+  asm volatile("" : "+v"(lane));
+#pragma unroll
+  for (int t = 0; t < M::NT; ++t) { const int e = lane + 64 * t; r[t] = pt[e < M::TOP2 ? e : M::TOP2 - 1]; }
+#pragma unroll
+  for (int t = 0; t < M::NC; ++t) { const int e = lane + 64 * t; r[M::NT + t] = pc[e < n2 ? e : last]; }
+}
+template <typename L>
+__device__ __forceinline__ void wideStoreLdsMjd(double* dst, const ex_d2 (&r)[MjdRegs<L>::N], int lane, int dimf) {
+  using M = MjdRegs<L>;
+  constexpr int NV = L::NV, NVF = L::NVF;
+  const int n2 = dimf * (L::NX / 2);
+  const int inv_f = dimf > 0 ? 65535 / dimf + 1 : 0;
+  asm volatile("" : "+v"(lane));
+#pragma unroll
+  for (int t = 0; t < M::NT; ++t) {
+    const int e = lane + 64 * t;
+    const int c = e / (NV / 2);
+    if (64 * t + 63 < M::TOP2 || e < M::TOP2) reinterpret_cast<ex_d2*>(dst)[c * (NVF / 2) + (e - c * (NV / 2))] = r[t];
+  }
+#pragma unroll
+  for (int t = 0; t < M::NC; ++t) {
+    const int e = lane + 64 * t;
+    if (e < n2) {
+      const int k = 2 * e, c0 = (k * inv_f) >> 16, r0 = k - c0 * dimf;
+      const bool wrap = r0 + 1 == dimf;
+      dst[NV + r0 + NVF * c0] = r[M::NT + t].x;
+      dst[NV + (wrap ? 0 : r0 + 1) + NVF * (wrap ? c0 + 1 : c0)] = r[M::NT + t].y;
+    }
+  }
+}
 template <int N2>
 __device__ __forceinline__ void wideStoreLds(double* dst, const ex_d2 (&r)[(N2 + 63) / 64], int lane) {
 #pragma unroll
@@ -130,7 +171,7 @@
   using L = OcpLayout<D>;
   constexpr int NV = D::NV, NX = D::NX, NU = D::NU, NF = D::NF, NVF = D::NVF, NC = D::NC;
   constexpr int RL = L::R_SV + NV, MJDL = NVF * NX, MJUL = L::MJ_TRI;
-  static_assert(RL % 2 == 0 && MJDL % 2 == 0 && MJUL % 2 == 0 && L::E_MJD % 2 == 0 && L::EXP % 2 == 0 && L::RIC % 2 == 0, "16-byte loads");
+  static_assert(RL % 2 == 0 && MJDL % 2 == 0 && MJUL % 2 == 0 && L::E_MJDC % 2 == 0 && L::EXP % 2 == 0 && L::RIC % 2 == 0, "16-byte loads");
   constexpr int PML = RL > MJDL ? RL : MJDL;
   __shared__ __attribute__((aligned(16))) double pm[PML], mju[MJUL], sr[L::SOL];
   double* pb = pm;
@@ -150,12 +191,12 @@
   const bool costate = !P->backward_euler;
   const bool bimp = P->backward_euler && nd->kind == 1;
   const bool expand = !terminal && !bimp;
-  ex_d2 pw[(RL / 2 + 63) / 64], mw[(MJDL / 2 + 63) / 64], uw[(MJUL / 2 + 63) / 64];
+  ex_d2 pw[(RL / 2 + 63) / 64], mw[MjdRegs<L>::N], uw[(MJUL / 2 + 63) / 64];
   if (costate) wideLoad<RL / 2>(pw, B.ric + rec * L::RIC, lane);
-  const int rows_ld = NV + nd->dimf, h_ld = (rows_ld + 1) >> 1, inv_ld = 65535 / h_ld + 1, nmjd2 = h_ld * NX, ntri2 = (rows_ld * (rows_ld + 1) / 2 + 1) >> 1;
+  const int rows_ld = NV + nd->dimf, ntri2 = (rows_ld * (rows_ld + 1) / 2 + 1) >> 1;
   static_assert(NVF % 2 == 0 && (NVF / 2) * NX == MJDL / 2, "pieces per column of MJtJinv_dIDCdqv");
   if (expand) {
-    wideLoadRows<MJDL / 2, NVF / 2>(mw, B.exp + rec * L::EXP + L::E_MJD, lane, h_ld, inv_ld, nmjd2);
+    wideLoadMjd<L>(mw, B.kkt + rec * L::KKT, B.exp + rec * L::EXP, lane, nd->dimf);
     wideLoadN<MJUL / 2>(uw, B.exp + rec * L::EXP + L::E_MJ, lane, ntri2);
   }
   static_assert(L::SOL % 2 == 0 && L::NCON <= 128, "two IPM rows per lane");
@@ -192,7 +233,7 @@
   }
   if (terminal) return;
   waveLdsSync();
-  if (expand) wideStoreLdsRows<MJDL / 2, NVF / 2>(mjd, mw, lane, h_ld, inv_ld, nmjd2);
+  if (expand) wideStoreLdsMjd<L>(mjd, mw, lane, nd->dimf);
   waveLdsSync();
   const long su = rec;
   const double* s = sr;
@@ -203,7 +244,7 @@
     if (lane < NV) {
       double acc = -mjidc_r;
       double t1 = 0.0;
-      for (int c = 0; c < NV; ++c) t1 += kk[L::K_FVQ + lane + NV * c] * dx[c];
+      for (int c = 0; c < NV; ++c) t1 += L::fvRow(kk[L::K_MJDQ + lane + NV * c], nd->dt, lane, c) * dx[c];
       acc += t1;
       double t2 = 0.0;
       for (int j = 0; j < dimf; ++j) t2 += kk[L::K_FVU + lane + NV * j] * du[j];
@@ -261,11 +302,11 @@
   constexpr int NV = D::NV, NQ = D::NQ, NX = D::NX, NU = D::NU, NF = D::NF, NVF = D::NVF, NC = D::NC;
   constexpr int GL = L::GAIN, RL = L::R_SV + NV, MJDL = NVF * NX, MJUL = L::MJ_TRI;
   static_assert(GL % 2 == 0 && RL % 2 == 0 && MJDL % 2 == 0 && MJUL % 2 == 0 && L::SOL % 2 == 0 && L::GAIN % 2 == 0 && L::RIC % 2 == 0 && L::EXP % 2 == 0 &&
-                L::E_MJD % 2 == 0 && L::KKT % 2 == 0 && L::K_FQQ % 2 == 0 && L::K_FX % 2 == 0 && NVF % 2 == 0, "16-byte loads");
+                L::E_MJDC % 2 == 0 && L::KKT % 2 == 0 && L::K_FQQ % 2 == 0 && L::K_FX % 2 == 0 && NVF % 2 == 0, "16-byte loads");
   static_assert(L::K_FQV == L::K_FQQ + 36 && L::NCON <= 128 && NX <= 36 && 36 + NX / 2 <= 64, "Fqq6 | Fqv6 and Fx on one load; two IPM rows per lane");
   static_assert(NC <= 4 && NF <= 15 && NVF + NV <= 64 && L::R_PQQ == 0 && L::R_SV == L::R_SQ + NV, "node word: four contacts; lane maps");
   static_assert(L::C_FRIC >= 64 && L::C_CD >= 64 && L::NCON <= 128, "cone / contact-distance rows are mapped to lane + 64 only");
-  constexpr int NG2 = (GL / 2 + 63) / 64, NP2 = (RL / 2 + 63) / 64, NM2 = (MJDL / 2 + 63) / 64, NT2 = (MJUL / 2 + 63) / 64, NS2 = (L::SOL / 2 + 63) / 64;
+  constexpr int NG2 = (GL / 2 + 63) / 64, NP2 = (RL / 2 + 63) / 64, NM2 = MjdRegs<L>::N, NT2 = (MJUL / 2 + 63) / 64, NS2 = (L::SOL / 2 + 63) / 64;
   constexpr int MAXM = OcpForwardExpandMaxChain;
   constexpr int PF = NX * NX, PSV = PF, PPAD = PF + NX;
   constexpr int DV = NX + NU + NV + NF + 2;
@@ -340,8 +381,8 @@
     auto fetch = [&](int i, Regs& R) {
       const long rec = base + n_slot[i];
       wideLoad<GL / 2>(R.g, B.gain + rec * L::GAIN, lane);
-      const int rows_ld = NV + ((n_word[i] >> 5) & 15), h_ld = (rows_ld + 1) >> 1, inv_ld = 65535 / h_ld + 1;
-      wideLoadRows<MJDL / 2, NVF / 2>(R.m, B.exp + rec * L::EXP + L::E_MJD, lane, h_ld, inv_ld, h_ld * NX);
+      const int rows_ld = NV + ((n_word[i] >> 5) & 15);
+      wideLoadMjd<L>(R.m, B.kkt + rec * L::KKT, B.exp + rec * L::EXP, lane, rows_ld - NV);
       wideLoadN<MJUL / 2>(R.u, B.exp + rec * L::EXP + L::E_MJ, lane, (rows_ld * (rows_ld + 1) / 2 + 1) >> 1);
       {
         const ex_d2* __restrict__ kq = reinterpret_cast<const ex_d2*>(B.kkt + rec * L::KKT + L::K_FQQ);
@@ -362,9 +403,8 @@
       const double sdt = n_dt[i], sdtq = n_dtq[i];
       double* __restrict__ dd = B.dir + rec * L::DIR;
       const int dimvf = NV + dimf;
-      const int h_ld = (dimvf + 1) >> 1, inv_ld = 65535 / h_ld + 1;
       wideStoreLds<GL / 2>(gb, R.g, lane);
-      wideStoreLdsRows<MJDL / 2, NVF / 2>(mjd, R.m, lane, h_ld, inv_ld, h_ld * NX);
+      wideStoreLdsMjd<L>(mjd, R.m, lane, dimf);
       wideStoreLds<MJUL / 2>(mju, R.u, lane);
       if (lane < 36 + NX / 2) reinterpret_cast<ex_d2*>(fb)[lane] = R.f;
       const double mjidc_r = R.mjidc;
diff --git a/idocp_amd/csrc/ocp_riccati_kernel.hip b/idocp_amd/csrc/ocp_riccati_kernel.hip
--- a/idocp_amd/csrc/ocp_riccati_kernel.hip
+++ b/idocp_amd/csrc/ocp_riccati_kernel.hip
@@ -49,6 +49,22 @@
     if (4 * s + 3 < K) o[s] = p[stride * k];
     else { const double v = p[stride * (k < K ? k : K - 1)]; o[s] = k < K ? v : 0.0; }
   }
+}
+
+__device__ __forceinline__ double uniformDouble(double x) {
+  return __hiloint2double(__builtin_amdgcn_readfirstlane(__double2hiint(x)), __builtin_amdgcn_readfirstlane(__double2loint(x)));
+}
+template <typename L>
+__device__ __forceinline__ rd2 fvStagedPiece(rd2 x, int j0, double sdt) {
+  constexpr int NV = L::NV, NX = L::NX;
+  static_assert(NV % 2 == 0 && L::K_MJDQ % 2 == 0 && L::K_FVU == L::K_MJDQ + NV * NX, "pairs of rows inside [X_q X_v]");
+  const int j = j0 - L::K_MJDQ;
+  const bool in = j >= 0 && j < NV * NX;
+  const int jj = in ? j : 0, c = jj / NV, r = jj - c * NV;
+  const double sc = in ? -sdt : 1.0;
+  x.x = sc * x.x + ((in && c == NV + r) ? 1.0 : 0.0);
+  x.y = sc * x.y + ((in && c == NV + r + 1) ? 1.0 : 0.0);
+  return x;
 }
 
 template <typename D, bool WIDE, int TB, int TE, typename Mid>
@@ -329,7 +345,8 @@
   }
   {
     const double* __restrict__ kk = B.kkt + (base + nodes[M - 2].slot) * L::KKT;
-    for (int e = tid; e < SL; e += nt) st[e] = kk[KO + e];
+    const double sdt0 = nodes[M - 2].dt;
+    for (int e = tid; e < SL / 2; e += nt) reinterpret_cast<rd2*>(st)[e] = fvStagedPiece<L>(reinterpret_cast<const rd2*>(kk + KO)[e], KO + 2 * e, sdt0);
   }
   blockSync<NW>();
   for (int i = M - 2; i >= 0; --i) {
@@ -343,6 +360,7 @@
     constexpr int PF = (SL / 2 + NT - 1) / NT, T1 = 9, T2 = 6, T2W = (T2 + NW - 1) / NW;
     static_assert(SL % 2 == 0 && KO % 2 == 0 && S::STAGE % 2 == 0 && L::KKT % 2 == 0, "16-byte loads of the stage record");
     rd2 pre[PF];
+    double sdt_pre = 0.0;
     double qxx[T2W][4];
     auto loadQxx = [&]() {
       const double* __restrict__ kc = B.kkt + rec * L::KKT;
@@ -364,10 +382,10 @@
     double* Quu = st + (L::K_QUU - KO);
     const double* Fqq6 = st + (L::K_FQQ - KO);
     const double* Fqv6 = st + (L::K_FQV - KO);
-    const double* Fall = st + (L::K_FVQ - KO);
-    static_assert(L::K_FVV == L::K_FVQ + NV * NV && L::K_FVU == L::K_FVV + NV * NV, "[Fvq Fvv Fvu] contiguous");
-    const double* Fvq = st + (L::K_FVQ - KO);
-    const double* Fvv = st + (L::K_FVV - KO);
+    const double* Fall = st + (L::K_MJDQ - KO);
+    static_assert(L::K_MJDV == L::K_MJDQ + NV * NV && L::K_FVU == L::K_MJDV + NV * NV, "[Fvq Fvv Fvu] contiguous");
+    const double* Fvq = st + (L::K_MJDQ - KO);
+    const double* Fvv = st + (L::K_MJDV - KO);
     const double* Fvu = st + (L::K_FVU - KO);
     const double* lx = st + (L::K_LX - KO);
     double* lu = st + (L::K_LU - KO);
@@ -401,7 +419,7 @@
       const rd2* wr = reinterpret_cast<const rd2*>(Wt + LDW * row);
       const rd2* svp = reinterpret_cast<const rd2*>(&sm[S::SV]);
       const rd2* fx = reinterpret_cast<const rd2*>(Fx);
-      static_assert(NV % 2 == 0 && S::SV % 2 == 0 && (L::K_FX - KO) % 2 == 0 && (L::K_FVQ - KO) % 2 == 0, "16-byte reads of the vector terms");
+      static_assert(NV % 2 == 0 && S::SV % 2 == 0 && (L::K_FX - KO) % 2 == 0 && (L::K_MJDQ - KO) % 2 == 0, "16-byte reads of the vector terms");
       double acc;
       if (r < 6) {
         acc = 0.0;
@@ -429,6 +447,7 @@
       const rd2* __restrict__ kn = reinterpret_cast<const rd2*>(B.kkt + (base + nodes[i - 1].slot) * L::KKT + KO);
 #pragma unroll
       for (int t = 0; t < PF; ++t) { const int e = tid + NT * t; pre[t] = kn[e < SL / 2 ? e : SL / 2 - 1]; }
+      sdt_pre = nodes[i - 1].dt;
     }
     RSTAMP(9);
     if (NW > 1 && tid >= 64 && tid < 64 + NX) sPart1(tid - 64);
@@ -614,8 +633,11 @@
     for (int e = tid; e < NU * NX / 2; e += nt) reinterpret_cast<rd2*>(gg)[e] = reinterpret_cast<const rd2*>(&sm[S::KM])[e];
     if (tid < NU) gg[L::G_k + tid] = sm[S::KV + tid];
     if (i > 0) {
-#pragma unroll
-      for (int t = 0; t < PF; ++t) { const int e = tid + NT * t; if (e < SL / 2) reinterpret_cast<rd2*>(st)[e] = pre[t]; }
+      const double sdt_u = uniformDouble(sdt_pre);
+      int td = tid;
+      asm volatile("" : "+v"(td));
+#pragma unroll
+      for (int t = 0; t < PF; ++t) { const int e = td + NT * t; if (e < SL / 2) reinterpret_cast<rd2*>(st)[e] = fvStagedPiece<L>(pre[t], KO + 2 * e, sdt_u); }
     }
     blockSync<NW>();
     RSTAMP(8);
@@ -667,7 +689,7 @@
   constexpr int NV = D::NV, NX = D::NX, NU = D::NU, NF = D::NF, LDH = S::LDH, LDP = S::LDP;
   static_assert(NX + NU == 48 && L::R_PQV == L::R_PQQ + L::P_TRI && L::R_PVV == L::R_PQV + NV * NV && L::R_SQ == L::R_PVV + L::P_TRI &&
                 L::R_SV == L::R_SQ + NV && L::R_PQQ == 0, "ric record: Pqq | Pqv | Pvv | sq | sv");
-  static_assert(L::K_FVV == L::K_FVQ + NV * NV && L::K_FVU == L::K_FVV + NV * NV, "[Fvq Fvv Fvu] contiguous");
+  static_assert(L::K_MJDV == L::K_MJDQ + NV * NV && L::K_FVU == L::K_MJDV + NV * NV, "[Fvq Fvv Fvu] contiguous");
   extern __shared__ __attribute__((aligned(16))) double sm[];
   __shared__ int s_ok;
   const OcpProblem* __restrict__ P = B.prob;
@@ -694,7 +716,7 @@
       const int cn = SL::nat(16 * bb + li);
       int off;
       if (rn < NV) off = cn < 6 ? L::K_FQQ + rn + 6 * cn : ((cn >= NV && cn < NV + 6) ? L::K_FQV + rn + 6 * (cn - NV) : ZERO_AT);
-      else off = L::K_FVQ + (rn - NV) + NV * cn;
+      else off = L::K_MJDQ + (rn - NV) + NV * cn;
       cOff[d][bb] = off;
     }
   }
@@ -844,6 +866,7 @@
   };
   double Cd[6][3], lz = 0.0, fx = 0.0;
   tile_t Qc[6];
+  double n_sdt = M > 1 ? nodes[M - 2].dt : 0.0;
   auto stageIn = [&]() {
 #pragma unroll
     for (int t = 0; t < PF; ++t) { const int e = lane + 64 * t; if (64 * t + 63 < SL2 || e < SL2) reinterpret_cast<rd2*>(&sm[S::PM])[e] = pre[t]; }
@@ -859,6 +882,19 @@
     }
     lz = kk[lzOff];
     fx = kk[L::K_FX + (myNat < NX ? myNat : 0)];
+    {
+      const double sdt = uniformDouble(n_sdt);
+      int lj = li, gj = g;
+      asm volatile("" : "+v"(lj), "+v"(gj));
+#pragma unroll
+      for (int d = 1; d < 6; ++d) {
+        const bool vrow = d < 5 || gj >= 2;
+        const double sc = vrow ? -sdt : 1.0, sc2 = (vrow && lj < 4) ? -sdt : 1.0;
+        Cd[d][0] = sc * Cd[d][0];
+        Cd[d][1] = sc * Cd[d][1] + ((d < 5 && lj == 4 * (d - 1) + gj) ? 1.0 : 0.0);
+        Cd[d][2] = sc2 * Cd[d][2] + ((d == 5 && gj >= 2 && lj == gj) ? 1.0 : 0.0);
+      }
+    }
     waveLdsSync();
   };
   auto gatherQ = [&]() {
@@ -879,7 +915,7 @@
     const double dt = n_dt;
     const long rec = base + __builtin_amdgcn_readfirstlane(n_slot);
     const int dimi = HYBRID ? __builtin_amdgcn_readfirstlane(n_dimi) : 0;
-    if (i > 0) { n_slot = nodes[i - 1].slot; n_dt = nodes[i - 1].dtq; if (HYBRID) n_dimi = nodes[i - 1].sw_dimi; }
+    if (i > 0) { n_slot = nodes[i - 1].slot; n_dt = nodes[i - 1].dtq; n_sdt = nodes[i - 1].dt; if (HYBRID) n_dimi = nodes[i - 1].sw_dimi; }
     const bool constrained = HYBRID && dimi > 0;
 #ifdef IDOCP_S3_STAMPS
     const bool stamp = lane == 0 && b == (gridDim.x > 7 ? 7 : 0) && i == M / 2 && B.prof != nullptr;
@@ -1278,9 +1314,9 @@
   constexpr int F2 = FL / 2, G2 = GL / 2, NF2 = (F2 + 63) / 64, NG2 = (G2 + 63) / 64;
   __shared__ __attribute__((aligned(16))) double fb[FL], gb[GL];
   __shared__ double dx[NX], du[NU], dxn[NX];
-  constexpr int MAXM = 1024;
+  constexpr int MAXM = 768;
   __shared__ int s_slot[MAXM];
-  __shared__ double s_dtq[MAXM];
+  __shared__ double s_dtq[MAXM], s_dt[MAXM];
   const OcpProblem* __restrict__ P = B.prob;
   const int M = B.M;
   const OcpNode* __restrict__ nodes = B.nodes;
@@ -1289,7 +1325,7 @@
   const long base = b * B.NS;
   const bool tab = M <= MAXM;
   if (tab) {
-    for (int i = lane; i < M; i += 64) { s_slot[i] = nodes[i].slot; s_dtq[i] = nodes[i].dtq; }
+    for (int i = lane; i < M; i += 64) { s_slot[i] = nodes[i].slot; s_dtq[i] = nodes[i].dtq; s_dt[i] = nodes[i].dt; }
     waveLdsSync();
   }
   auto slotOf = [&](int i) -> int { return tab ? s_slot[i] : nodes[i].slot; };
@@ -1317,13 +1353,13 @@
   if (lane < NV) dx[NV + lane] = v0[b * NV + lane] - s0[L::S_V + lane];
   const double* Fqq6 = fb + (L::K_FQQ - FO);
   const double* Fqv6 = fb + (L::K_FQV - FO);
-  const double* Fvq = fb + (L::K_FVQ - FO);
-  const double* Fvv = fb + (L::K_FVV - FO);
+  const double* Xqv = fb + (L::K_MJDQ - FO);
   const double* Fvu = fb + (L::K_FVU - FO);
   const double* Fx = fb + (L::K_FX - FO);
   auto step = [&](int i, d2 (&fr)[NF2], d2 (&gr)[NG2]) {
     const long rec = base + slotOf(i);
     const double dt = tab ? s_dtq[i] : nodes[i].dtq;
+    const double sdt = tab ? s_dt[i] : nodes[i].dt;
     double* __restrict__ dd = B.dir + rec * L::DIR;
 #pragma unroll
     for (int t = 0; t < NF2; ++t) { const int e = lane + 64 * t; if (e < F2) reinterpret_cast<d2*>(fb)[e] = fr[t]; }
@@ -1348,10 +1384,10 @@
       double acc = 0.0;
       if (lane < 2 * NV) {
         const int r = lane >> 1, half = lane & 1;
-        const double* Fm = half ? Fvv : Fvq;
+        const double* Xm = Xqv + (half ? NV * NV : 0);
         const double* xs = half ? dx + NV : dx;
 #pragma unroll
-        for (int c = 0; c < NV; ++c) acc += Fm[r + NV * c] * xs[c];
+        for (int c = 0; c < NV; ++c) acc += L::fvRow(Xm[r + NV * c], sdt, r, half ? NV + c : c) * xs[c];
 #pragma unroll
         for (int j = 0; j < NU / 2; ++j) acc += Fvu[r + NV * ((NU / 2) * half + j)] * du[(NU / 2) * half + j];
       }
diff --git a/idocp_amd/csrc/parnmpc_event_kernels.hip b/idocp_amd/csrc/parnmpc_event_kernels.hip
--- a/idocp_amd/csrc/parnmpc_event_kernels.hip
+++ b/idocp_amd/csrc/parnmpc_event_kernels.hip
@@ -225,8 +225,8 @@
   }
   for (int e = tid; e < NV * NV; e += 256) {
     const int c = e / NV, r = e - c * NV;
-    kk[L::K_FVQ + e] = Fvq[e];
-    kk[L::K_FVV + e] = (r == c) ? -1.0 : 0.0;
+    kk[L::K_MJDQ + e] = -Fvq[e];
+    kk[L::K_MJDV + e] = 0.0;
     if (r >= c) ee[L::E_MJ + r * (r + 1) / 2 + c] = Mi[e];
   }
   for (int e = tid; e < NV * NU; e += 256) {
@@ -320,8 +320,7 @@
     } else if (r < NX) {
       const int rv = r - NV;
       if (c < NU) v = c < nw ? kk[L::K_FVU + rv + NV * c] : 0.0;
-      else if (c < NU + NV) v = kk[L::K_FVQ + rv + NV * (c - NU)];
-      else v = kk[L::K_FVV + rv + NV * (c - NU - NV)];
+      else v = L::fvRow(kk[L::K_MJDQ + rv + NV * (c - NU)], dt, rv, c - NU, -1.0);
     } else if (r < nr && c >= NU) {
       v = Wc[L::W_PHIX + (r - NX) + NF * (c - NU)];
     }
diff --git a/idocp_amd/csrc/parnmpc_kernels.hip b/idocp_amd/csrc/parnmpc_kernels.hip
--- a/idocp_amd/csrc/parnmpc_kernels.hip
+++ b/idocp_amd/csrc/parnmpc_kernels.hip
@@ -74,8 +74,7 @@
     } else {
       const int rv = r - NV;
       if (c < NU) v = kk[L::K_FVU + rv + NV * c];
-      else if (c < NU + NV) v = kk[L::K_FVQ + rv + NV * (c - NU)];
-      else v = kk[L::K_FVV + rv + NV * (c - NU - NV)];
+      else v = L::fvRow(kk[L::K_MJDQ + rv + NV * (c - NU)], dt, rv, c - NU, -1.0);
     }
     sm[S::B + e] = v;
   }
diff --git a/idocp_amd/csrc/parnmpc_kkt_wave_kernel.hip b/idocp_amd/csrc/parnmpc_kkt_wave_kernel.hip
--- a/idocp_amd/csrc/parnmpc_kkt_wave_kernel.hip
+++ b/idocp_amd/csrc/parnmpc_kkt_wave_kernel.hip
@@ -295,12 +295,12 @@
         } else if (e < NX) {
           const int rv_ = e - NV;
           if (z < NU) ad = S::BUF - S::QPART + L::K_FVU + rv_ + NV * z;
-          else if (z < NU + NV) ad = S::BUF - S::QPART + L::K_FVQ + rv_ + NV * (z - NU);
-          else ad = S::BUF - S::QPART + L::K_FVV + rv_ + NV * (z - NU - NV);
+          else ad = S::BUF - S::QPART + L::K_MJDQ + rv_ + NV * (z - NU);
         } else if (e == NX) {
           ad = z < NU ? S::BUF - S::QPART + L::K_LU + z : S::BUF - S::QPART + L::K_LX + (z - NU);
         }
-        Fr[jt][q] = sm[ad];
+        const double f = sm[ad];
+        Fr[jt][q] = (e >= NV && e < NX && z >= NU) ? L::fvRow(f, dt, e - NV, z - NU, -1.0) : f;
       }
   };
   wtile Sm[6];
@@ -780,12 +780,12 @@
         } else if (e < NX) {
           const int rv_ = e - NV;
           if (z < NU) ad = z < nw ? S::BUF - S::QPART + L::K_FVU + rv_ + NV * z : S::CPAD;
-          else if (z < NU + NV) ad = S::BUF - S::QPART + L::K_FVQ + rv_ + NV * (z - NU);
-          else ad = S::BUF - S::QPART + L::K_FVV + rv_ + NV * (z - NU - NV);
+          else ad = S::BUF - S::QPART + L::K_MJDQ + rv_ + NV * (z - NU);
         } else if (e < nr && z >= NU) {
           ad = S::BUF + S::PHIX + (e - NX) + NF * (z - NU);
         }
-        Fr[jt][q] = sm[ad];
+        const double f = sm[ad];
+        Fr[jt][q] = (e >= NV && e < NX && z >= NU) ? L::fvRow(f, dt, e - NV, z - NU, -1.0) : f;
       }
   };
   wtile Sm[6];
```

Measured after the change: 221,700 SQP iterations/s, median of 6. 1.01x the previous value.
